# OpenMendel/MendelIHT.jl

Hardware: AMD Instinct MI355X
Metric: IHT iterations/sec + Xᵀr GB/s vs HBM roofline, n=500k p=1M k=200 (higher is better)
Workload: dtype f64 (residual as a 54-bit fixed-point number, exact accumulation on the matrix cores, f64 recombination); 1 GPU; iht on synthetic SnpArray n=500000 p=1000000 k=200 Normal/Identity (BASELINE configs[2]); n=500000, p=1000000, k=200, xtv_variant=-1

## Files before the change

### include/mendeliht_hip.h

```cpp
#ifndef MENDELIHT_HIP_H
#define MENDELIHT_HIP_H
#include <stddef.h>
#include <stdint.h>

#ifdef __cplusplus
extern "C" {
#endif

enum {
    MIH_OK = 0,
    MIH_BAD_DIM = 1,
    MIH_BAD_ARG = 2,
    MIH_NOT_CENTERED = 3,
    MIH_NAN_LOGL = 4,
    MIH_INF_LOGL = 5,
    MIH_HIP_ERROR = 6,
    MIH_OOM = 7,
    MIH_NO_DEVICE = 8
};

enum { MIH_NORMAL = 0, MIH_BERNOULLI = 1, MIH_POISSON = 2, MIH_NEGBIN = 3,
       MIH_GAMMA = 4, MIH_INVGAUSS = 5 };
enum { MIH_IDENTITY = 0, MIH_LOGIT = 1, MIH_LOG = 2, MIH_PROBIT = 3, MIH_CLOGLOG = 4, MIH_CAUCHIT = 5,
       MIH_INVERSE = 6, MIH_INVSQUARE = 7, MIH_SQRT = 8 };
enum { MIH_ESTR_NONE = 0, MIH_ESTR_MM = 1, MIH_ESTR_NEWTON = 2 };

typedef struct mih_mat mih_mat;

int mih_device_count(int *count);
int mih_last_error(char *buf, size_t len);
int mih_version(int *major, int *minor);
int mih_abi_sizes(int64_t *sizes, int32_t n);

int mih_snp_create(const uint8_t *bed_cols, int64_t n, int64_t p, int64_t col_stride_bytes,
                   int center, int scale, int impute, int dtype, int device, mih_mat **out);
int mih_snp_create_synthetic(int64_t n, int64_t p, uint64_t seed, double missing_rate,
                             int center, int scale, int impute, int device, mih_mat **out);
int mih_snp_create_synthetic_shard(int64_t n, int64_t p, int64_t col_offset, uint64_t seed,
                                   double missing_rate, int center, int scale, int impute,
                                   int device, mih_mat **out);
int mih_dense_create(const double *x, int64_t n, int64_t p, int device, mih_mat **out);
int mih_dense_create_f32(const float *x, int64_t n, int64_t p, int device, mih_mat **out);
int mih_dense_create_synthetic(int64_t n, int64_t p, uint64_t seed, int device, mih_mat **out);
int mih_dosage_create(const uint16_t *num, int64_t n, int64_t p, int64_t col_stride, int32_t denom, int device, mih_mat **out);
int mih_dosage_create_synthetic(int64_t n, int64_t p, uint64_t seed, int32_t denom, double missing_rate, int device, mih_mat **out);
enum {
    MIH_BGEN_CORRUPT = 1,
    MIH_BGEN_HEADER = 2,
    MIH_BGEN_PLOIDY = 3,
    MIH_BGEN_PHASED = 4,
    MIH_BGEN_BITS = 5,
    MIH_BGEN_SUM = 6,
    MIH_BGEN_DEEP = 10,
    MIH_BGEN_MIXED = 11,
    MIH_BGEN_FINE = 12,
    MIH_BGEN_MALFORMED = 13
};
int mih_dosage_create_bgen(const char *path, int64_t n, int64_t ncols, const int64_t *block_offset, int compression,
                           int threads, int device, mih_mat **out, int32_t *denom_out, int64_t *bad_block, int32_t *bad_what);
int mih_dosage_regrid(mih_mat *h, int32_t denom);
int mih_dosage_export(const mih_mat *h, int64_t col0, int64_t ncols, uint16_t *out);
int mih_mat_destroy(mih_mat *h);
int mih_mat_reserve(mih_mat *h, int64_t bytes);
int mih_mat_dims(const mih_mat *h, int64_t *n, int64_t *p);
int mih_snp_mu_sigma(const mih_mat *h, double *mu, double *sinv);
int mih_snp_export_bed(const mih_mat *h, uint8_t *bed_cols_out);
int mih_snp_naive_impute(const mih_mat *h, uint8_t *bed_cols_out);

int mih_xtv(const mih_mat *h, const double *r, double *out);
int mih_xtv_batched(const mih_mat *h, const double *R, int m, double *OUT);
int mih_xtv_batched_fmt(const mih_mat *h, const double *R, int m, int digits, double *OUT);
int mih_xv_sparse(const mih_mat *h, const int64_t *idx, const double *val, int64_t nnz, double *out);

int mih_project_topk(double *x, int64_t len, int64_t k, int64_t *n_kept);
int mih_project_group_sparse(double *y, const int64_t *group, int64_t len, int64_t J,
                             const int64_t *k, int k_is_vector);

typedef struct mih_comm {
    int32_t rank, world;
    int64_t col_offset;
    int64_t p_global;
    int (*allreduce)(void *user, double *buf, int64_t count, int32_t op, int32_t on_device);
    int (*allgather)(void *user, const double *send, int64_t count, double *recv);
    void *user;
} mih_comm;

int mih_rccl_unique_id(void *id128);
int mih_comm_create_rccl(const void *id128, int32_t rank, int32_t world, int32_t device, int64_t col_offset,
                         int64_t p_global, mih_comm **out);
int mih_comm_info(const mih_comm *c, int32_t *ranks_seen, char *librccl_path, int64_t cap);
int mih_comm_destroy_rccl(mih_comm *c);
int mih_cv_allgather(const mih_comm *c, double *mses_raw, int64_t count);

typedef struct mih_fit_params {
    int64_t  k;
    int64_t  J;
    int32_t  dist, link;
    double   nb_r;
    double   tol;
    int32_t  max_iter, min_iter, max_step;
    int32_t  est_r;
    const uint8_t *zkeep;
    const double  *weight;
    const int64_t *group;
    const int64_t *ks;
    int64_t  nks;
    void (*progress)(void *user, int iter, double logl, int backtracks, double tol);
    void    *progress_user;
    int32_t  init_beta;
    const mih_comm *comm;
    int32_t  debias;
    int32_t  xtv_digits;
    int (*choose)(void *user, int32_t kind, const int64_t *list, int64_t n, int64_t excess, int64_t *out);
    void    *choose_user;
    int32_t  cv_threads;
    int32_t  step_mode;
} mih_fit_params;
enum { MIH_CHOOSE_SAMPLE = 0, MIH_CHOOSE_SHUFFLE_B = 1, MIH_CHOOSE_SHUFFLE_C = 2 };

typedef struct mih_fit_result {
    double   time;
    double   logl;
    int64_t  iter;
    double   pve;
    double   nb_r;
    int32_t  choose_fired;
    int32_t  n_trace;
    double  *beta;
    double  *c;
    double  *logl_trace;
    double  *tol_trace;
    int32_t *bt_trace;
    double  *mu;
} mih_fit_result;

int mih_fit_iht(const mih_mat *h, const mih_fit_params *prm, const double *y,
                const double *z, int64_t q, const uint8_t *train, mih_fit_result *res);

int mih_cv_iht(const mih_mat *h, const mih_fit_params *prm, const double *y,
               const double *z, int64_t q, const int32_t *folds, int32_t nfolds,
               const int64_t *path, int64_t npath, int32_t rank, int32_t world,
               double *mses_raw);
int mih_cv_assignment(const int64_t *path, int64_t npath, int32_t nfolds, int32_t world, int32_t *rank_of);
int mih_cv_meanloss(const double *mses_raw, const int32_t *folds, int64_t n, int32_t nfolds,
                    int64_t npath, double *mse_out);
int mih_fit_iht_path(const mih_mat *h, const mih_fit_params *prm, const double *y, const double *z,
                     int64_t q, const int64_t *path, int64_t npath, int32_t rank, int32_t world,
                     double *logl_out, int64_t *iter_out, double *beta_out, double *c_out);
int mih_cv_iht_multi(const mih_mat *const *hs, int32_t nrep, const mih_fit_params *prm, const double *y,
                     const double *z, int64_t q, const int32_t *folds, int32_t nfolds,
                     const int64_t *path, int64_t npath, double *mses_raw);

typedef struct mih_mv_result {
    double   time, logl;
    int64_t  iter;
    int32_t  choose_fired, n_trace;
    double  *B;
    double  *C;
    double  *Sigma;
    double  *pve;
    double  *logl_trace, *tol_trace;
    int32_t *bt_trace;
} mih_mv_result;
int mih_fit_mv(const mih_mat *h, const mih_fit_params *prm, const double *Y, int64_t r,
               const double *Z, int64_t q, const uint8_t *train, mih_mv_result *res);
int mih_cv_mv(const mih_mat *h, const mih_fit_params *prm, const double *Y, int64_t r,
              const double *Z, int64_t q, const int32_t *folds, int32_t nfolds,
              const int64_t *path, int64_t npath, int32_t rank, int32_t world, double *mses_raw);

typedef struct mih_session mih_session;
int mih_session_create(const mih_mat *h, const mih_fit_params *prm, const double *y,
                       const double *z, int64_t q, const uint8_t *train, mih_session **out);
int mih_session_step(mih_session *s, double *logl, int32_t *backtracks, double *tol);
int mih_session_run(mih_session *s, int64_t nsteps, double *logl, int64_t *backtracks, double *tol);
int mih_session_model(mih_session *s, double *beta, double *c);
int mih_session_destroy(mih_session *s);

typedef struct mih_pass_record {
    double  start_ms;
    double  ms;
    int32_t residuals;
    int32_t operands;
    int32_t stream_tag;
    int32_t reserved;
    char    kernel[48];
} mih_pass_record;
enum { MIH_CNT_LANES = 0,
       MIH_CNT_MAX_IN_FLIGHT = 1,
       MIH_CNT_HANDOVERS = 2,
       MIH_CNT_SHARED_INIT = 3,
       MIH_CNT_ROUNDS = 4,
       MIH_CNT_FITS = 5,
       MIH_CNT_SCORES = 6,
       MIH_CNT_MAX_LANE_SLOTS = 7,
       MIH_CNT_INIT_SCORES = 8,
       MIH_CNT_RESIDENT_STEPS = 9,
       MIH_CNT_RESIDENT_ATTEMPTS = 10,
       MIH_CNT_RESIDENT_HANDBACKS = 11,
       MIH_CNT_RESIDENT_DIRECT = 12,
       MIH_CNT_RESIDENT_REDOS = 13,
       MIH_CNT_SKIPPED_LAST_SCORES = 14,
       MIH_CNT_RESIDUALS_43BIT = 15,
       MIH_CNT_PEELED_RESIDUALS = 16,
       MIH_PROFILE_NCOUNTERS = 17 };
int mih_profile_enable(const mih_mat *h, int on);
int mih_profile_read(const mih_mat *h, double *xtv_kernel_ms, int64_t *xtv_launches, int reset);
int mih_profile_passes(const mih_mat *h, mih_pass_record *out, int64_t cap, int64_t *n, int reset);
int mih_profile_exchange(const mih_mat *h, double *ms4, int64_t *count4, int reset);
int mih_profile_counters(const mih_mat *h, int64_t *out , int reset);
int mih_bench_xtv(const mih_mat *h, int digits, int m, int iters, int warmup, uint64_t seed,
                  float *ms_per_pass, double *checksum);
int mih_xtv_algorithmic_bytes(const mih_mat *h, int m, double *bytes);

#ifdef __cplusplus
}
#endif
// ... 2 lines not shown
```

### mendeliht.jl_amd/api.py

```python
import ctypes as C
import os
import sys
import time

import numpy as np

_HERE = os.path.dirname(os.path.abspath(__file__))
_LIBNAME = "libmendeliht_hip.so"
_PROBES_LIBNAME = "libmendeliht_hip_probes.so"


class MendelIHTError(RuntimeError):
    """Base class for errors reported by the HIP library."""


class DimensionMismatch(MendelIHTError, ValueError):
    pass


class ArgumentError(MendelIHTError, ValueError):
    pass


_STATUS = {1: DimensionMismatch, 2: ArgumentError, 3: ArgumentError, 4: MendelIHTError, 5: MendelIHTError,
           6: MendelIHTError, 7: MemoryError, 8: MendelIHTError}


def library_path():
    return os.path.join(_HERE, _LIBNAME)


def probes_library_path():
    return os.path.join(_HERE, _PROBES_LIBNAME)


def using_probes():
    e = os.environ.get("MENDELIHT_HIP_PROBES", "")
    return e not in ("", "0")


class _FitParams(C.Structure):
    _fields_ = [("k", C.c_int64), ("J", C.c_int64), ("dist", C.c_int32), ("link", C.c_int32),
                ("nb_r", C.c_double), ("tol", C.c_double),
                ("max_iter", C.c_int32), ("min_iter", C.c_int32), ("max_step", C.c_int32), ("est_r", C.c_int32),
                ("zkeep", C.c_void_p), ("weight", C.c_void_p), ("group", C.c_void_p), ("ks", C.c_void_p),
                ("nks", C.c_int64), ("progress", C.c_void_p), ("progress_user", C.c_void_p),
                ("init_beta", C.c_int32), ("comm", C.c_void_p), ("debias", C.c_int32), ("xtv_digits", C.c_int32),
                ("choose", C.c_void_p), ("choose_user", C.c_void_p), ("cv_threads", C.c_int32), ("step_mode", C.c_int32)]


class _Comm(C.Structure):
    _fields_ = [("rank", C.c_int32), ("world", C.c_int32), ("col_offset", C.c_int64), ("p_global", C.c_int64),
                ("allreduce", C.c_void_p), ("allgather", C.c_void_p), ("user", C.c_void_p)]


_CHOOSE = C.CFUNCTYPE(C.c_int, C.c_void_p, C.c_int32, C.POINTER(C.c_int64), C.c_int64, C.c_int64, C.POINTER(C.c_int64))
CHOOSE_SAMPLE, CHOOSE_SHUFFLE_B, CHOOSE_SHUFFLE_C = 0, 1, 2


def _choose_callback(fn):
    def cb(_user, kind, lst, n, excess, out):
        try:
            got = np.asarray(fn(int(kind), np.array(lst[:n], dtype=np.int64), int(excess)), dtype=np.int64).ravel()
            want = excess if kind == CHOOSE_SAMPLE else n
            if got.size != want:
                return 1
            for t in range(want):
                out[t] = int(got[t])
            return 0
        except Exception:
            return 1
    return _CHOOSE(cb)


_ALLREDUCE = C.CFUNCTYPE(C.c_int, C.c_void_p, C.c_void_p, C.c_int64, C.c_int32, C.c_int32)
_ALLGATHER = C.CFUNCTYPE(C.c_int, C.c_void_p, C.c_void_p, C.c_int64, C.c_void_p)


class _FitResult(C.Structure):
    _fields_ = [("time", C.c_double), ("logl", C.c_double), ("iter", C.c_int64), ("pve", C.c_double),
                ("nb_r", C.c_double), ("choose_fired", C.c_int32), ("n_trace", C.c_int32),
                ("beta", C.c_void_p), ("c", C.c_void_p), ("logl_trace", C.c_void_p), ("tol_trace", C.c_void_p),
                ("bt_trace", C.c_void_p), ("mu", C.c_void_p)]


class _MvResult(C.Structure):
    _fields_ = [("time", C.c_double), ("logl", C.c_double), ("iter", C.c_int64),
                ("choose_fired", C.c_int32), ("n_trace", C.c_int32),
                ("B", C.c_void_p), ("C", C.c_void_p), ("Sigma", C.c_void_p), ("pve", C.c_void_p),
                ("logl_trace", C.c_void_p), ("tol_trace", C.c_void_p), ("bt_trace", C.c_void_p)]


class _PassRecord(C.Structure):
    _fields_ = [("start_ms", C.c_double), ("ms", C.c_double), ("residuals", C.c_int32), ("operands", C.c_int32),
                ("stream_tag", C.c_int32), ("reserved", C.c_int32), ("kernel", C.c_char * 48)]


PROFILE_COUNTERS = ("lanes", "max_in_flight", "handovers", "shared_init", "rounds", "fits", "scores", "max_lane_slots", "init_scores",
                    "resident_steps", "resident_attempts", "resident_handbacks", "resident_direct", "resident_redos", "skipped_last_scores", "residuals_43bit",
                    "peeled_residuals")

_PROGRESS = C.CFUNCTYPE(None, C.c_void_p, C.c_int, C.c_double, C.c_int, C.c_double)

_lib = None


def lib():
    global _lib
    if _lib is not None:
        return _lib
    path = probes_library_path() if using_probes() else library_path()
    path = os.environ.get("MENDELIHT_HIP_LIB", path)
    if not os.path.exists(path):
        raise MendelIHTError(
            f"{path} is missing: build it with `python -c 'import __graft_entry__ as g; g.build()'` "
            "(hipcc --offload-arch=gfx950). There is no CPU fallback for this path.")
    L = C.CDLL(path)
    vp, i64, i32, dbl = C.c_void_p, C.c_int64, C.c_int32, C.c_double
    sig = {
        "mih_device_count": [C.POINTER(C.c_int)],
        "mih_last_error": [C.c_char_p, C.c_size_t],
        "mih_version": [C.POINTER(C.c_int), C.POINTER(C.c_int)],
        "mih_snp_create": [vp, i64, i64, i64, C.c_int, C.c_int, C.c_int, C.c_int, C.c_int, C.POINTER(vp)],
        "mih_snp_create_synthetic": [i64, i64, C.c_uint64, dbl, C.c_int, C.c_int, C.c_int, C.c_int, C.POINTER(vp)],
        "mih_snp_create_synthetic_shard": [i64, i64, i64, C.c_uint64, dbl, C.c_int, C.c_int, C.c_int, C.c_int, C.POINTER(vp)],
        "mih_dense_create": [vp, i64, i64, C.c_int, C.POINTER(vp)],
        "mih_dense_create_synthetic": [i64, i64, C.c_uint64, C.c_int, C.POINTER(vp)],
        "mih_dense_create_f32": [vp, i64, i64, C.c_int, C.POINTER(vp)],
        "mih_dosage_create": [vp, i64, i64, i64, i32, C.c_int, C.POINTER(vp)],
        "mih_dosage_create_synthetic": [i64, i64, C.c_uint64, i32, dbl, C.c_int, C.POINTER(vp)],
        "mih_dosage_export": [vp, i64, i64, vp],
        "mih_dosage_create_bgen": [C.c_char_p, i64, i64, vp, C.c_int, C.c_int, C.c_int, C.POINTER(vp), C.POINTER(i32), C.POINTER(i64),
                                   C.POINTER(i32)],
        "mih_dosage_regrid": [vp, i32],
        "mih_mat_destroy": [vp],
        "mih_mat_dims": [vp, C.POINTER(i64), C.POINTER(i64)],
        "mih_mat_reserve": [vp, i64],
        "mih_snp_mu_sigma": [vp, vp, vp],
        "mih_snp_export_bed": [vp, vp],
        "mih_snp_naive_impute": [vp, vp],
        "mih_xtv": [vp, vp, vp],
        "mih_xtv_batched": [vp, vp, C.c_int, vp],
        "mih_xtv_batched_fmt": [vp, vp, C.c_int, C.c_int, vp],
        "mih_xv_sparse": [vp, vp, vp, i64, vp],
        "mih_project_topk": [vp, i64, i64, C.POINTER(i64)],
        "mih_project_group_sparse": [vp, vp, i64, i64, vp, C.c_int],
        "mih_fit_iht": [vp, C.POINTER(_FitParams), vp, vp, i64, vp, C.POINTER(_FitResult)],
        "mih_cv_iht": [vp, C.POINTER(_FitParams), vp, vp, i64, vp, i32, vp, i64, i32, i32, vp],
        "mih_cv_meanloss": [vp, vp, i64, i32, i64, vp],
        "mih_cv_assignment": [vp, i64, i32, i32, vp],
        "mih_fit_iht_path": [vp, C.POINTER(_FitParams), vp, vp, i64, vp, i64, i32, i32, vp, vp, vp, vp],
        "mih_cv_iht_multi": [vp, i32, C.POINTER(_FitParams), vp, vp, i64, vp, i32, vp, i64, vp],
        "mih_fit_mv": [vp, C.POINTER(_FitParams), vp, i64, vp, i64, vp, C.POINTER(_MvResult)],
        "mih_cv_mv": [vp, C.POINTER(_FitParams), vp, i64, vp, i64, vp, i32, vp, i64, i32, i32, vp],
        "mih_bench_xtv": [vp, C.c_int, C.c_int, C.c_int, C.c_int, C.c_uint64, C.POINTER(C.c_float), C.POINTER(dbl)],
        "mih_xtv_algorithmic_bytes": [vp, C.c_int, C.POINTER(dbl)],
        "mih_abi_sizes": [vp, i32],
        "mih_session_create": [vp, C.POINTER(_FitParams), vp, vp, i64, vp, C.POINTER(vp)],
        "mih_session_step": [vp, C.POINTER(dbl), C.POINTER(i32), C.POINTER(dbl)],
        "mih_session_run": [vp, i64, C.POINTER(dbl), C.POINTER(i64), C.POINTER(dbl)],
        "mih_session_model": [vp, vp, vp],
        "mih_session_destroy": [vp],
        "mih_rccl_unique_id": [vp],
        "mih_comm_create_rccl": [vp, i32, i32, i32, i64, i64, C.POINTER(vp)],
        "mih_comm_destroy_rccl": [vp],
        "mih_comm_info": [vp, C.POINTER(i32), vp, i64],
        "mih_cv_allgather": [vp, vp, i64],
        "mih_profile_enable": [vp, C.c_int],
        "mih_profile_read": [vp, C.POINTER(dbl), C.POINTER(i64), C.c_int],
        "mih_profile_passes": [vp, C.POINTER(_PassRecord), i64, C.POINTER(i64), C.c_int],
        "mih_profile_counters": [vp, C.POINTER(i64), C.c_int],
        "mih_profile_exchange": [vp, C.POINTER(dbl), C.POINTER(i64), C.c_int],
    }
    if using_probes():
        sig.update({"mih_probe_set_xtv_variant": [C.c_int], "mih_probe_set_xtv_multi_variant": [C.c_int],
                    "mih_probe_set_max_fused": [C.c_int],
                    "mih_probe_xtv_sequence": [C.c_void_p, C.c_void_p, C.c_int, C.c_void_p, C.c_int, C.c_int, C.c_void_p],
                    "mih_probe_xv_sequence": [vp, i64, i64, C.c_int, vp, vp, vp, vp, vp, vp, vp]})
    for name, args in sig.items():
        f = getattr(L, name)
        f.argtypes = args
        f.restype = C.c_int
    _lib = L
    return L


def exported_symbols():
    return ["mih_device_count", "mih_last_error", "mih_version", "mih_snp_create", "mih_snp_create_synthetic",
            "mih_snp_create_synthetic_shard",
            "mih_dense_create", "mih_dense_create_synthetic", "mih_dense_create_f32",
            "mih_dosage_create", "mih_dosage_create_synthetic", "mih_dosage_export",
            "mih_dosage_create_bgen", "mih_dosage_regrid", "mih_mat_destroy", "mih_mat_dims", "mih_mat_reserve",
            "mih_snp_mu_sigma", "mih_snp_export_bed", "mih_snp_naive_impute", "mih_xtv", "mih_xtv_batched", "mih_xv_sparse",
            "mih_project_topk", "mih_project_group_sparse", "mih_fit_iht", "mih_cv_iht", "mih_cv_meanloss", "mih_cv_assignment", "mih_cv_iht_multi", "mih_fit_iht_path",
            "mih_fit_mv", "mih_cv_mv", "mih_bench_xtv", "mih_xtv_algorithmic_bytes", "mih_xtv_batched_fmt", "mih_abi_sizes",
            "mih_session_create", "mih_session_step", "mih_session_run", "mih_session_model", "mih_session_destroy",
            "mih_rccl_unique_id", "mih_comm_create_rccl", "mih_comm_info", "mih_comm_destroy_rccl", "mih_cv_allgather",
            "mih_profile_enable", "mih_profile_read", "mih_profile_passes", "mih_profile_counters", "mih_profile_exchange"]


def probe_symbols():
    return ["mih_probe_set_xtv_variant", "mih_probe_set_xtv_multi_variant", "mih_probe_set_max_fused", "mih_probe_xtv_sequence",
            "mih_probe_xv_sequence"]


def _check(rc):
    if rc == 0:
        return
    buf = C.create_string_buffer(512)
    lib().mih_last_error(buf, 512)
    raise _STATUS.get(rc, MendelIHTError)(f"[mih status {rc}] {buf.value.decode(errors='replace')}")


def _p(a):
    return None if a is None else a.ctypes.data_as(C.c_void_p)


def device_count():
    n = C.c_int(0)
    _check(lib().mih_device_count(C.byref(n)))
    return n.value


class _Dist:
    code = 0
    name = "Normal"

    def __repr__(self):
        return f"{self.name}()"


class Normal(_Dist):
    code, name = 0, "Normal"


class Bernoulli(_Dist):
    code, name = 1, "Bernoulli"


class Poisson(_Dist):
    code, name = 2, "Poisson"


class NegativeBinomial(_Dist):
    code, name = 3, "NegativeBinomial"

    def __init__(self, r=1.0, p=0.5):
        self.r, self.p = float(r), float(p)

    def __repr__(self):
        return f"NegativeBinomial(r={self.r}, p={self.p})"


class Gamma(_Dist):
    code, name = 4, "Gamma"


class InverseGaussian(_Dist):
    code, name = 5, "InverseGaussian"


class MvNormal(_Dist):
    code, name = -1, "MvNormal"


class IdentityLink:
    code = 0

    def __repr__(self):
        return "IdentityLink()"


class LogitLink:
    code = 1

    def __repr__(self):
        return "LogitLink()"


class LogLink:
    code = 2

    def __repr__(self):
        return "LogLink()"


def _link(name, code):
    return type(name, (), {"code": code, "__repr__": lambda self: f"{name}()"})


ProbitLink = _link("ProbitLink", 3)
CloglogLink = _link("CloglogLink", 4)
CauchitLink = _link("CauchitLink", 5)
InverseLink = _link("InverseLink", 6)
InverseSquareLink = _link("InverseSquareLink", 7)
SqrtLink = _link("SqrtLink", 8)


def canonicallink(d):
    d = _inst(d)
    return {0: IdentityLink, 1: LogitLink, 2: LogLink, 3: LogLink, 4: InverseLink, 5: InverseSquareLink}[max(d.code, 0)]()


def _inst(x):
    return x() if isinstance(x, type) else x


def read_bed(path, n):
    size = os.path.getsize(path)
    with open(path, "rb") as f:
        magic = f.read(3)
    if size < 3 or magic != b"\x6c\x1b\x01":
        raise ArgumentError(f"{path} is not a SNP-major PLINK .bed file")
    stride = (n + 3) // 4
    if (size - 3) % stride:
        raise DimensionMismatch(f"{path}: size does not match n={n}")
    if size == 3:
        return np.zeros((0, stride), dtype=np.uint8)
    return np.memmap(path, dtype=np.uint8, mode="r", offset=3, shape=((size - 3) // stride, stride))


class _Mat:
    def __init__(self):
        self._h = C.c_void_p(None)
        self.n = self.p = 0

    def __del__(self):
        try:
            if self._h:
                lib().mih_mat_destroy(self._h)
                self._h = C.c_void_p(None)
        except Exception:
            pass

    @property
    def shape(self):
        return (self.n, self.p)

    def _dims(self):
        n, p = C.c_int64(0), C.c_int64(0)
        _check(lib().mih_mat_dims(self._h, C.byref(n), C.byref(p)))
        self.n, self.p = n.value, p.value

    def xtv(self, r, xtv_digits=None):
        r = np.asarray(r, dtype=np.float64)
        dg = _digits(xtv_digits)
        if r.ndim == 1:
            if r.size != self.n:
                raise DimensionMismatch(f"r has length {r.size}, expected {self.n}")
            r = np.ascontiguousarray(r)
            out = np.empty(self.p)
            if dg == 0:
                _check(lib().mih_xtv(self._h, _p(r), _p(out)))
            else:
                _check(lib().mih_xtv_batched_fmt(self._h, _p(r), 1, dg, _p(out)))
            return out
        if r.shape[0] != self.n:
            raise DimensionMismatch(f"R has {r.shape[0]} rows, expected {self.n}")
        R = np.asfortranarray(r)
        out = np.empty((self.p, R.shape[1]), order="F")
        _check(lib().mih_xtv_batched_fmt(self._h, _p(R), R.shape[1], dg, _p(out)))
        return out

    def xv_sparse(self, idx, val):
        idx = np.ascontiguousarray(idx, dtype=np.int64)
        val = np.ascontiguousarray(val, dtype=np.float64)
        out = np.empty(self.n)
        _check(lib().mih_xv_sparse(self._h, _p(idx), _p(val), idx.size, _p(out)))
        return out

    def bench_xtv(self, variant=-1, iters=10, warmup=2, seed=1, xtv_digits=None):
        return self.bench_xtv_batched(1, variant=variant, iters=iters, warmup=warmup, seed=seed, xtv_digits=xtv_digits)

    def bench_xtv_batched(self, m, max_fused=4, variant=-1, iters=5, warmup=1, seed=1, xtv_digits=None):
        if variant != -1 or max_fused != 4 or using_probes():
            probe_set(variant=variant, max_fused=max_fused)
        ms, cs = C.c_float(0), C.c_double(0)
        try:
            _check(lib().mih_bench_xtv(self._h, _digits(xtv_digits), m, iters, warmup, seed, C.byref(ms), C.byref(cs)))
        finally:
            if using_probes():
                probe_set(variant=-1, max_fused=4)
        return ms.value, cs.value

    def algorithmic_bytes(self, m=1):
        b = C.c_double(0)
        _check(lib().mih_xtv_algorithmic_bytes(self._h, m, C.byref(b)))
        return b.value


RESERVE_BY_DEFAULT = False


class SnpLinAlg(_Mat):

    def _reserve(self, reserve):
        if reserve:
            _check(lib().mih_mat_reserve(self._h, 0))
        elif reserve is None and RESERVE_BY_DEFAULT:
            lib().mih_mat_reserve(self._h, 0)

    def __init__(self, bed, n=None, center=False, scale=False, impute=True, device=0, _handle=None, dtype=np.float64, reserve=None):
        super().__init__()
        self.center, self.scale, self.impute = bool(center), bool(scale), bool(impute)
        self.device = device
        self.dtype = np.dtype(dtype).type
        if self.dtype not in (np.float64, np.float32):
            raise ArgumentError("SnpLinAlg{T}: T must be Float64 or Float32")
        if _handle is not None:
            self._h = _handle
            self._dims()
            return
        if isinstance(bed, (str, os.PathLike)):
            if n is None:
                raise ArgumentError("n (number of samples) is required with a .bed path")
            bed = read_bed(bed, n)
        cols = np.ascontiguousarray(bed, dtype=np.uint8)
        if cols.ndim != 2:
            raise DimensionMismatch("bed columns must be a (p, stride) uint8 array")
        if n is None:
            raise ArgumentError("n (number of samples) is required")
        h = C.c_void_p(None)
        _check(lib().mih_snp_create(_p(cols), n, cols.shape[0], cols.shape[1], int(center), int(scale),
                                    int(impute), 32 if self.dtype is np.float32 else 64, device, C.byref(h)))
        self._h = h
        self._dims()
        self._reserve(reserve)

    @classmethod
    def synthetic(cls, n, p, seed=2024, missing_rate=0.0, center=True, scale=True, impute=True, device=0,
                  col_offset=0, reserve=None):
        h = C.c_void_p(None)
        _check(lib().mih_snp_create_synthetic_shard(n, p, int(col_offset), seed, float(missing_rate), int(center),
                                                    int(scale), int(impute), device, C.byref(h)))
        x = cls(None, center=center, scale=scale, impute=impute, device=device, _handle=h)
        x._reserve(reserve)
        return x

    def mu_sigma(self):
        mu, s = np.empty(self.p), np.empty(self.p)
        _check(lib().mih_snp_mu_sigma(self._h, _p(mu), _p(s)))
        return mu, s

    def export_bed(self):
        out = np.empty((self.p, (self.n + 3) // 4), dtype=np.uint8)
        _check(lib().mih_snp_export_bed(self._h, _p(out)))
        return out


def naive_impute(x, destination, n=None):
    if isinstance(x, SnpLinAlg):
        mat = x
    else:
        if n is None:
            raise ArgumentError("naive_impute needs the number of samples n with a .bed path or raw columns")
        cols = read_bed(x, n) if isinstance(x, (str, os.PathLike)) else x
        mat = SnpLinAlg(cols, n)
    out = np.empty((mat.p, (mat.n + 3) // 4), dtype=np.uint8)
    _check(lib().mih_snp_naive_impute(mat._h, _p(out)))
    if not str(destination).endswith(".bed"):
        destination = str(destination) + ".bed"
    with open(destination, "wb") as f:
        f.write(b"\x6c\x1b\x01")
        f.write(out.tobytes())
    return None


class DenseMatrix(_Mat):

    def __init__(self, x, device=0, _handle=None):
        super().__init__()
        self.device = device
        self.dtype = np.float64
        if _handle is not None:
            self._h = _handle
            self._dims()
            return
        x = np.asarray(x)
        if x.ndim != 2:
            raise DimensionMismatch("x must be a matrix")
        h = C.c_void_p(None)
        if x.dtype == np.float32:
            x = np.asfortranarray(x)
            self.dtype = np.float32
            _check(lib().mih_dense_create_f32(_p(x), x.shape[0], x.shape[1], device, C.byref(h)))
        else:
            x = np.asfortranarray(x, dtype=np.float64)
            _check(lib().mih_dense_create(_p(x), x.shape[0], x.shape[1], device, C.byref(h)))
        self._h = h
        self._dims()

    @classmethod
    def synthetic(cls, n, p, seed=2024, device=0):
        h = C.c_void_p(None)
        _check(lib().mih_dense_create_synthetic(n, p, seed, device, C.byref(h)))
        return cls(None, device=device, _handle=h)


class DosageMatrix(_Mat):

    def __init__(self, num, denom, device=0, _handle=None):
        super().__init__()
        self.device = device
        self.denom = int(denom)
        self.dtype = np.float64
        if _handle is not None:
            self._h = _handle
            self._dims()
            return
        num = np.asarray(num)
        if num.ndim != 2:
            raise DimensionMismatch("num must be a matrix")
        if num.dtype != np.uint16:
            raise ArgumentError(f"num must be uint16 (0xFFFF = missing), got {num.dtype}")
        num = np.asfortranarray(num)
        h = C.c_void_p(None)
        _check(lib().mih_dosage_create(_p(num), num.shape[0], num.shape[1], num.shape[0], self.denom, device, C.byref(h)))
        self._h = h
        self._dims()

    @classmethod
    def from_dosages(cls, d, device=0):
        from .genotypes import dosage_grid
        num, denom = dosage_grid(np.asarray(d, dtype=np.float64))
        return cls(num, denom, device=device)

    @classmethod
    def synthetic(cls, n, p, seed=2024, denom=255, missing_rate=0.0, device=0):
        h = C.c_void_p(None)
        _check(lib().mih_dosage_create_synthetic(n, p, seed, int(denom), float(missing_rate), device, C.byref(h)))
        return cls(None, denom, device=device, _handle=h)

    def mu_sigma(self):
        mu, s = np.empty(self.p), np.empty(self.p)
        _check(lib().mih_snp_mu_sigma(self._h, _p(mu), _p(s)))
        return mu, s

    def regrid(self, denom):
        _check(lib().mih_dosage_regrid(self._h, int(denom)))
        self.denom = int(denom)
        return self

    def export(self, col0=0, ncols=None):
        ncols = self.p - col0 if ncols is None else ncols
        out = np.empty((ncols, self.n), dtype=np.uint16)
        _check(lib().mih_dosage_export(self._h, int(col0), int(ncols), _p(out)))
        return out.T


def _as_mat(x):
    if isinstance(x, _Mat):
        return x
    if isinstance(x, np.ndarray):
        if x.dtype == np.uint8:
            raise ArgumentError("x is a SnpArray! Please convert it to a SnpLinAlg first!")
        return DenseMatrix(x)
    raise ArgumentError(f"unsupported design matrix type {type(x)}")


def project_k(x, k):
    if k < 0:
        raise ArgumentError(f"DomainError: Attempted to project to sparsity level {k}")
    x = np.array(x, dtype=np.float64).ravel()
    kept = C.c_int64(0)
    _check(lib().mih_project_topk(_p(x), x.size, int(k), C.byref(kept)))
    return x


def project_group_sparse(y, group, J, k):
    y = np.array(y, dtype=np.float64).ravel()
    group = np.ascontiguousarray(group, dtype=np.int64)
    if group.size != y.size:
        raise DimensionMismatch("group must have the length of y")
    kv = np.ascontiguousarray(np.atleast_1d(k), dtype=np.int64)
    _check(lib().mih_project_group_sparse(_p(y), _p(group), y.size, int(J), _p(kv), int(np.ndim(k) > 0)))
    return y


def standardize(z):
    z = np.array(z, dtype=np.float64)
    mu = z.mean(axis=0)
    sd = np.sqrt(((z - mu) ** 2).sum(axis=0) / (z.shape[0] - 1))
    return (z - mu) / sd


class IHTResult:

    def __init__(self, time, logl, iter, beta, c, J, k, group, d, sigma_g, trace=None, choose_fired=False, mu=None):
        self.time, self.logl, self.iter = time, logl, iter
        self.beta, self.c, self.J, self.k, self.group, self.d = beta, c, J, k, group, d
# ... 713 lines not shown
```

### mendeliht.jl_amd/csrc/common.h

```cpp
#pragma once
#include <hip/hip_runtime.h>
#include <atomic>
#include <chrono>
#include <map>
#include <mutex>
#include <iterator>
#include <memory>
#include <cstdint>
#include <cstdlib>
#include <cstdio>
#include <cstring>
#include <string>
#include <unordered_map>
#include <functional>
#include <vector>
#include "../../include/mendeliht_hip.h"

namespace mih {

void set_error(const char *fmt, ...);
int  hip_fail(hipError_t e, const char *what, const char *file, int line);

inline const char *probe_env(const char *name)
{
#ifdef MIH_PROBES
    return getenv(name);
#else
    (void)name;
    return nullptr;
#endif
}

#define MIH_HIP(expr)                                                         \
    do {                                                                      \
        hipError_t e_ = (expr);                                               \
        if (e_ != hipSuccess) return ::mih::hip_fail(e_, #expr, __FILE__, __LINE__); \
    } while (0)

#define MIH_TRY(expr)                      \
    do {                                   \
        int rc_ = (expr);                  \
        if (rc_ != MIH_OK) return rc_;     \
    } while (0)

constexpr int kChunkRows = 1024;

inline int64_t round_up(int64_t a, int64_t b) { return (a + b - 1) / b * b; }

struct DevPool {
    char *base = nullptr; size_t bytes = 0;
    std::mutex mu;
    std::map<size_t, size_t> free_blocks;
    std::map<size_t, size_t> used;
    static constexpr size_t kGran = 2ull << 20;
    ~DevPool() { if (base) (void)hipFree(base); }
    bool init(size_t total)
    {
        total = (total + kGran - 1) / kGran * kGran;
        if (hipMalloc((void **)&base, total) != hipSuccess) { (void)hipGetLastError(); base = nullptr; return false; }
        bytes = total; free_blocks[0] = total;
        return true;
    }
    void *take(size_t want)
    {
        want = (want + kGran - 1) / kGran * kGran;
        std::lock_guard<std::mutex> g(mu);
        for (auto it = free_blocks.begin(); it != free_blocks.end(); ++it) {
            if (it->second < want) continue;
            const size_t off = it->first, sz = it->second;
            free_blocks.erase(it);
            if (sz > want) free_blocks[off + want] = sz - want;
            used[off] = want;
            return base + off;
        }
        return nullptr;
    }
    bool owns(const void *q) const { return base && (const char *)q >= base && (const char *)q < base + bytes; }
    void give_back(void *q)
    {
        std::lock_guard<std::mutex> g(mu);
        const size_t off = (size_t)((char *)q - base);
        auto u = used.find(off);
        if (u == used.end()) return;
        size_t o = off, sz = u->second;
        used.erase(u);
        auto nx = free_blocks.lower_bound(o);
        if (nx != free_blocks.end() && o + sz == nx->first) { sz += nx->second; nx = free_blocks.erase(nx); }
        if (nx != free_blocks.begin()) { auto pv = std::prev(nx); if (pv->first + pv->second == o) { o = pv->first; sz += pv->second; free_blocks.erase(pv); } }
        free_blocks[o] = sz;
    }
};
inline DevPool *&current_pool() { static thread_local DevPool *q = nullptr; return q; }
struct PoolScope {
    DevPool *prev;
    explicit PoolScope(DevPool *q) : prev(current_pool()) { current_pool() = q; }
    ~PoolScope() { current_pool() = prev; }
};
inline hipError_t dev_malloc(void **q, size_t bytes, DevPool **from)
{
    *from = nullptr;
    if (DevPool *pl = current_pool()) {
        if (bytes >= (1ull << 20)) { if (void *r = pl->take(bytes)) { *q = r; *from = pl; return hipSuccess; } }
    }
    return hipMalloc(q, bytes);
}

struct Arena {
    char *dev = nullptr, *pin = nullptr;
    DevPool *dev_pool = nullptr;
    size_t dev_bytes = 0, pin_bytes = 0, dev_off = 0, pin_off = 0;
    Arena() = default;
    Arena(const Arena &) = delete;
    Arena &operator=(const Arena &) = delete;
    ~Arena() { release_dev(); if (pin) (void)hipHostFree(pin); }
    void release_dev() { if (dev) { if (dev_pool) dev_pool->give_back(dev); else (void)hipFree(dev); dev = nullptr; } }
    int reserve(size_t device_bytes, size_t pinned_bytes)
    {
        static const bool off = probe_env("MENDELIHT_NO_ARENA") != nullptr;
        if (off) return MIH_OK;
        if (dev_malloc((void **)&dev, device_bytes, &dev_pool) != hipSuccess) { (void)hipGetLastError(); dev = nullptr; device_bytes = 0; }
        if (hipHostMalloc((void **)&pin, pinned_bytes, hipHostMallocCoherent) != hipSuccess) { (void)hipGetLastError(); pin = nullptr; pinned_bytes = 0; }
        dev_bytes = device_bytes; pin_bytes = pinned_bytes; dev_off = pin_off = 0;
        return MIH_OK;
    }
    void *take_dev(size_t bytes)
    {
        const size_t o = (dev_off + 255) & ~(size_t)255;
        if (!dev || o + bytes > dev_bytes) return nullptr;
        dev_off = o + bytes;
        return dev + o;
    }
    void *take_pin(size_t bytes)
    {
        const size_t o = (pin_off + 255) & ~(size_t)255;
        if (!pin || o + bytes > pin_bytes) return nullptr;
        pin_off = o + bytes;
        return pin + o;
    }
};
inline Arena *&current_arena() { static thread_local Arena *a = nullptr; return a; }
struct CoopSched { virtual void yield() = 0; virtual ~CoopSched() {} };
inline CoopSched *&current_coop() { static thread_local CoopSched *c = nullptr; return c; }
inline int &coop_blocked() { static thread_local int d = 0; return d; }
inline bool coop_can_yield() { return current_coop() != nullptr && coop_blocked() == 0; }
int stream_sync_coop(hipStream_t s);
struct ArenaScope {
    Arena *prev;
    explicit ArenaScope(Arena *a) : prev(current_arena()) { current_arena() = a; ++coop_blocked(); }
    ~ArenaScope() { current_arena() = prev; --coop_blocked(); }
};

template <typename T>
struct DevBuf {
    T *p = nullptr;
    size_t n = 0;
    bool own = true;
    DevPool *pool = nullptr;
    DevBuf() = default;
    DevBuf(const DevBuf &) = delete;
    DevBuf &operator=(const DevBuf &) = delete;
    ~DevBuf() { release(); }
    void release() { if (p && own) { if (pool) pool->give_back(p); else (void)hipFree(p); } p = nullptr; n = 0; own = true; pool = nullptr; }
    void attach(T *ptr, size_t count) { release(); p = ptr; n = count; own = false; }
    int alloc(size_t count) {
        release();
        if (count == 0) count = 1;
        if (Arena *a = current_arena()) {
            if (void *q = a->take_dev(count * sizeof(T))) { p = static_cast<T *>(q); n = count; own = false; return MIH_OK; }
        }
        hipError_t e = dev_malloc((void **)&p, count * sizeof(T), &pool);
        if (e != hipSuccess) { set_error("hipMalloc(%zu bytes) failed: %s", count * sizeof(T), hipGetErrorString(e)); p = nullptr; return e == hipErrorOutOfMemory ? MIH_OOM : MIH_HIP_ERROR; }
        n = count;
        return MIH_OK;
    }
};

template <typename T>
struct PinBuf {
    T *p = nullptr;
    size_t n = 0;
    bool own = true;
    PinBuf() = default;
    PinBuf(const PinBuf &) = delete;
    PinBuf &operator=(const PinBuf &) = delete;
    ~PinBuf() { if (p && own) (void)hipHostFree(p); }
    int alloc(size_t count, bool coherent = false) {
        if (p && own) (void)hipHostFree(p);
        p = nullptr; n = 0; own = true;
        if (count == 0) count = 1;
        if (Arena *a = current_arena()) {
            if (void *q = a->take_pin(count * sizeof(T))) { p = static_cast<T *>(q); n = count; own = false; return MIH_OK; }
        }
        if (hipHostMalloc((void **)&p, count * sizeof(T), coherent ? hipHostMallocCoherent : hipHostMallocDefault) != hipSuccess) { set_error("hipHostMalloc(%zu bytes) failed", count * sizeof(T)); (void)hipGetLastError(); p = nullptr; return MIH_OOM; }
        n = count;
        return MIH_OK;
    }
};

struct SpinFlag {
    PinBuf<uint64_t> word;
    uint64_t seq = 0;
};
int readback_words(hipStream_t s, SpinFlag &f, const uint64_t *src_dev, uint64_t *dst_host, size_t words, int64_t pairs_first = -1);
uint64_t spin_begin(SpinFlag &f);
int spin_wait(hipStream_t s, SpinFlag &f, uint64_t seq);
#if defined(__HIPCC__)
__device__ __forceinline__ void publish_block(const uint64_t *src, uint64_t *dst_host, uint64_t words, uint64_t *flag_host, uint64_t seq)
{
    for (uint64_t i = threadIdx.x; i < words; i += blockDim.x)
        dst_host[i] = __hip_atomic_load(&src[i], __ATOMIC_RELAXED, __HIP_MEMORY_SCOPE_AGENT);
    __threadfence_system();
    __syncthreads();
    if (threadIdx.x == 0) __hip_atomic_store(flag_host, seq, __ATOMIC_RELEASE, __HIP_MEMORY_SCOPE_SYSTEM);
}
#endif

struct HostStage {
    static constexpr int kSlots = 8;
    PinBuf<uint64_t> ring;
    size_t slot_words = 0;
    int next = 0, since_sync = 0;
    int init(size_t words_per_slot) { slot_words = words_per_slot; next = 0; since_sync = 0; return ring.alloc(words_per_slot * kSlots, true); }
    int put(hipStream_t s, const void *a, size_t bytes_a, const void *b, size_t bytes_b, const uint64_t **out);
    void synced() { since_sync = 0; }
};
void stage_to_device(hipStream_t s, const uint64_t *src_pinned, uint64_t *dst_a, size_t words_a, uint64_t *dst_b, size_t words_b);

}

namespace mih {
struct PassRecord { hipEvent_t e0 = nullptr, e1 = nullptr; int residuals = 0, operands = 0, stream_tag = 0; char kernel[48] = {0}; };
struct ExchRecord { hipEvent_t e0 = nullptr, e1 = nullptr; int kind = 0; };
struct Profile {
    std::mutex mu;
    std::atomic<bool> on{false};
    hipEvent_t origin = nullptr;
    std::vector<PassRecord> open;
    std::vector<mih_pass_record> done;
    int64_t counters[MIH_PROFILE_NCOUNTERS] = {0};
    std::vector<ExchRecord> xopen;
    double xms[4] = {0.0, 0.0, 0.0, 0.0}; int64_t xcount[4] = {0, 0, 0, 0};
    void exch_host(int kind, double ms) { if (!on) return; std::lock_guard<std::mutex> g(mu); xms[kind] += ms; ++xcount[kind]; }
    void count(int which, int64_t add) { if (!on) return; std::lock_guard<std::mutex> g(mu); counters[which] += add; }
    void count_max(int which, int64_t v) { if (!on) return; std::lock_guard<std::mutex> g(mu); if (v > counters[which]) counters[which] = v; }
    void drain();
    ~Profile();
};
}

struct mih_mat {
    int       kind = 0;
    int       device = 0;
    int64_t   n = 0, p = 0;
    int       center = 1, scale = 1, impute = 1;
    int64_t   ncg = 0;
    int64_t   nbp = 0;
    int64_t   n_pad = 0;
    uint32_t *X = nullptr;
    double   *mu = nullptr, *sinv = nullptr;
    int64_t  *miss_ptr = nullptr;
    int32_t  *miss_row = nullptr;
    int64_t   total_missing = 0;
    double   *D = nullptr;
    float    *Df = nullptr;
    uint16_t *Du = nullptr;
    int64_t   du_ld = 0;
    int32_t   denom = 0;
    double   *du_mun = nullptr;
    double   *du_sc = nullptr;
    hipStream_t stream = nullptr;
    mih::DevPool *pool = nullptr;
    std::shared_ptr<mih::DevPool> pool_owner;
    std::shared_ptr<mih::Profile> prof = std::make_shared<mih::Profile>();
    mutable std::mutex ws_mu;
    mutable std::vector<hipStream_t> worker_streams;
};
namespace mih {
int select_device(int device);

struct DosageView { const uint16_t *X; int64_t ld; const double *mun, *sc; };
int dosage_alloc(mih_mat *h, int64_t n, int64_t p, int32_t denom, int device);
int dosage_stats(mih_mat *h);
void dosage_rescale(mih_mat *h, const uint32_t *gcol, uint32_t g, uint32_t mult);
inline DosageView dosage_view(const mih_mat *h) { return {h->Du, h->du_ld, h->du_mun, h->du_sc}; }
__device__ __forceinline__ double dosage_c(uint32_t num, double mun) { return num == 0xFFFFu ? 0.0 : (double)num - mun; }
__device__ __forceinline__ double dosage_x(const DosageView &v, int64_t j, int64_t i)
{
    return dosage_c(v.X[j * v.ld + i], v.mun[j]) * v.sc[j];
}
constexpr int kWorkerStreamsPerLane = 4;
hipStream_t worker_stream(const mih_mat *h, int i);
}

namespace mih {

__host__ __device__ inline int64_t xword(int64_t nbp, int64_t j, int64_t t)
{
    int64_t cg = j >> 5, blk = t >> 2, bp = blk >> 1;
    int m = (int)(j & 31), h = (int)((t >> 1) & 1), u = (int)(t & 1), e = (int)(blk & 1);
    return (((cg * nbp + bp) * 64 + (h * 32 + m)) << 2) + (e << 1) + u;
}

struct DigitMode {
    int base;
    int ndig;
    int per_op;
    int slots;
    int ebits;
    int rows_log2;
    int lay16 = 0;
    int flat = 0;
    int nres = 0;
    const int32_t *gate = nullptr; int32_t gate_val = 0;
};
constexpr int kMaxFlatPasses = 16;
struct FlatPasses { int npass; int u0[kMaxFlatPasses + 1]; int t0[kMaxFlatPasses + 1]; };
struct XtvTune {
    int digits = 0;
    int variant = -1;
    int multi_variant = 0;
    int max_nr = 4;
    int max_ops = 6;
    int slices = 0;
    bool half = true;
};
XtvTune xtv_tune(int digits);
inline XtvTune xtv_tune(const mih_fit_params *prm) { return xtv_tune(prm ? prm->xtv_digits : 0); }
bool xtv_digits_valid(int digits);

struct XtvSupportHook {
    const int32_t *cur = nullptr;
    const int64_t *idx[2] = {nullptr, nullptr};
    const int64_t *cnt[2] = {nullptr, nullptr};
    double *gval = nullptr, *A = nullptr, *B = nullptr;
    int blocks = 0;
};
struct XtvStatsHook {
    const double *spart = nullptr;
    const double *zpart = nullptr; double *df2 = nullptr; int q = 0, zblocks = 0;
    int ebits = 0;
};
constexpr int kStatBlocks = 64;
struct XtvWork {
    DevBuf<uint32_t> digits;
    DevBuf<double>   partial;
    DevBuf<double>   scal;
    DevBuf<unsigned> stat_done;
    double peels_counted = 0.0;
    DevBuf<double>   peel;
    int m_cap = 0, splits_cap = 0;
    DigitMode dm = {13, 16, 2, 16, 56, 20};
    int ops_cap = 0;
    size_t rhs_cap = 0;
    XtvTune tune;
    int stream_tag = 0;
    const int32_t *gate = nullptr; int32_t gate_val = 0;
    bool stats_done = false;
    DigitMode dm_alt = {49, 8, 4, 8, 42, 18}; bool has_alt = false, use_alt = false;
    XtvSupportHook hook;
    XtvStatsHook shook;
};
int  xtv_work_init(const mih_mat *h, XtvWork &w, int m, const XtvTune &tune, bool batched = true);
int  xtv_device(const mih_mat *h, XtvWork &w, const double *r_dev, int m, double *out_dev, hipStream_t s);
void xtv_count_peels(const mih_mat *h, XtvWork &w, hipStream_t s);
int  xtv_lockstep_width(const mih_mat *h, const XtvTune &tune);

struct XvWork {
    DevBuf<double> partial;
    DevBuf<double> coefA, coefB;
    DevBuf<double> coefG;
    int64_t cap = 0; int groups = 0;
    DevBuf<uint32_t> cache;
    DevBuf<int32_t>  slot_dev;
    DevBuf<int64_t>  fill_dev;
    DevBuf<int64_t>  off_dev;
    int64_t slots = 0;
    std::unordered_map<int64_t, int32_t> slot_of;
    std::vector<int64_t> col_of;
    std::vector<uint64_t> stamp;
    uint64_t tick = 0;
    std::vector<int64_t> h_offs;
    std::vector<int32_t> h_slots; std::vector<int64_t> h_fills;
};
int  xv_work_init(const mih_mat *h, XvWork &w, int64_t max_nnz, int64_t cache_nnz = 0);
size_t xv_work_bytes(const mih_mat *h, int64_t max_nnz, int64_t cache_nnz = 0);
int  xv_sparse_device(const mih_mat *h, XvWork &w, const int64_t *idx_dev, const double *val_dev,
                      int64_t nnz, double *out_dev, int clamp20, hipStream_t s, const int64_t *idx_host = nullptr,
                      HostStage *st = nullptr, const double *gather_src = nullptr, double *gather_out = nullptr);

int  xv_sparse_multi_device(const mih_mat *h, XvWork &w, const int64_t *idx_dev, const double *vals_dev, int64_t nnz, int m,
                            double *out_dev, hipStream_t s, const int64_t *idx_host);

struct TopkWork {
    DevBuf<uint32_t> hist;
    DevBuf<uint64_t> state;
    PinBuf<uint64_t> hsel;
    DevBuf<uint64_t> sel;
    DevBuf<uint64_t> fin;
    int64_t cap = 0;
    int64_t expect = 0;
    bool radix8 = false;
    SpinFlag flag;
};
int  topk_work_init(TopkWork &w, int64_t max_keep);
int  topk_project_device(double *x_dev, int64_t len, int64_t k, TopkWork &w, hipStream_t s,
                         std::vector<int64_t> &idx_out, std::vector<double> &val_out, bool zero_in_place = true);
int  collect_nonzero_device(double *x_dev, int64_t len, TopkWork &w, hipStream_t s,
                            std::vector<int64_t> &idx_out, std::vector<double> &val_out);
int  group_project_device(double *y_dev, const int64_t *group_dev, int64_t len, int64_t G, int64_t J,
                          const int64_t *k_dev, int k_is_vector, hipStream_t s);
struct DebiasShard { int64_t k_total = 0, k_off = 0; std::function<int(double *, int64_t)> reduce; };
int  debias_glm_device(const mih_mat *h, const int64_t *idx_host, int64_t k, const double *y_dev, int dist, int link,
                       double nb_r, double *beta_out, hipStream_t s, const DebiasShard *shard = nullptr);
int  comm_native_allreduce_on_stream(const mih_comm *c, double *buf_dev, int64_t count, int32_t op, hipStream_t s, int device);
int  comm_native_allgather_on_stream(const mih_comm *c, const double *send_dev, double *recv_dev, int64_t count, hipStream_t s, int device);
bool comm_is_native(const mih_comm *c, int device);
void cv_assign(const int64_t *path, int64_t npath, int32_t nfolds, int32_t world, std::vector<int32_t> &rank_of);
int  init_beta_regress_device(const mih_mat *h, const double *w_dev, const double *Y_dev, int m, double N,
                              const double *Sy_host, double *beta_dev, double *icpt_sum_host,
                              DevBuf<double> &red, DevBuf<double> &scal, hipStream_t s, const XtvTune &tune);

}
```

### mendeliht.jl_amd/csrc/dosage.hip

```cpp
#include "common.h"
#include <cmath>

namespace mih {

__global__ void __launch_bounds__(256)
k_dosage_stats(const uint16_t *__restrict__ X, int64_t ld, int32_t denom, double *__restrict__ mu, double *__restrict__ sinv,
               double *__restrict__ mun, double *__restrict__ sc, unsigned long long *__restrict__ bad)
{
    __shared__ unsigned long long s_sum[256], s_cnt[256], s_bad[256];
    const int64_t j = blockIdx.x;
    const uint4 *cx = reinterpret_cast<const uint4 *>(X + j * ld);
    const uint32_t top = 2u * (uint32_t)denom;
    unsigned long long sum = 0, cnt = 0, nbad = 0;
    for (int64_t i = threadIdx.x; i < ld / 8; i += 256) {
        const uint4 q = cx[i];
        const uint32_t w[4] = {q.x, q.y, q.z, q.w};
        #pragma unroll
        for (int k = 0; k < 8; ++k) {
            const uint32_t v = (w[k >> 1] >> (16 * (k & 1))) & 0xFFFFu;
            if (v != 0xFFFFu) {
                if (v > top) ++nbad;
                else { sum += v; ++cnt; }
            }
        }
    }
    s_sum[threadIdx.x] = sum; s_cnt[threadIdx.x] = cnt; s_bad[threadIdx.x] = nbad;
    __syncthreads();
    for (int w = 128; w > 0; w >>= 1) {
        if ((int)threadIdx.x < w) {
            s_sum[threadIdx.x] += s_sum[threadIdx.x + w]; s_cnt[threadIdx.x] += s_cnt[threadIdx.x + w];
            s_bad[threadIdx.x] += s_bad[threadIdx.x + w];
        }
        __syncthreads();
    }
    if (threadIdx.x == 0) {
        const double S = (double)s_sum[0], N = (double)s_cnt[0];
        const double m = N > 0.0 ? S / (N * (double)denom) : 0.0;
        const double s = sqrt(m * (1.0 - m / 2.0));
        mu[j] = m;
        sinv[j] = s > 0.0 ? 1.0 / s : 1.0;
        mun[j] = N > 0.0 ? S / N : 0.0;
        sc[j] = sinv[j] / (double)denom;
        if (s_bad[0]) atomicAdd(bad, s_bad[0]);
    }
}

__device__ __forceinline__ uint32_t dsg_mix(uint32_t x)
{
    x ^= x >> 16; x *= 0x7feb352du; x ^= x >> 15; x *= 0x846ca68bu; x ^= x >> 16;
    return x;
}

__global__ void __launch_bounds__(256)
k_dosage_synth(uint16_t *__restrict__ X, int64_t ld, int64_t n, int64_t p, uint64_t seed, int32_t denom, uint32_t miss_thr)
{
    const int64_t nv = ld / 8, total = nv * p;
    const uint32_t s0 = dsg_mix((uint32_t)seed ^ 0x3C6EF372u) ^ dsg_mix((uint32_t)(seed >> 32) + 0x1B873593u);
    const int32_t blur = denom / 10;
    for (int64_t q = blockIdx.x * 256ll + threadIdx.x; q < total; q += 256ll * gridDim.x) {
        const int64_t j = q / nv, i0 = (q - j * nv) * 8;
        const uint32_t key = dsg_mix(s0 ^ dsg_mix((uint32_t)j) ^ dsg_mix((uint32_t)(j >> 32) + 0x85EBCA6Bu));
        const uint32_t thr = (uint32_t)(((dsg_mix(key ^ 0xB5297A4Du) >> 8) + 0.5) / 16777216.0 * 0.5 * 65536.0);
        uint32_t w[4] = {0u, 0u, 0u, 0u};
        #pragma unroll
        for (int k = 0; k < 8; ++k) {
            const int64_t i = i0 + k;
            uint32_t v = 0xFFFFu;
            if (i < n) {
                const uint32_t e = dsg_mix(key ^ dsg_mix((uint32_t)i ^ 0x68E31DA4u) ^ (uint32_t)(i >> 32));
                const uint32_t f = dsg_mix(e ^ 0x1B56C4E9u), g = dsg_mix(f ^ 0x2C1B3C6Du);
                const int32_t calls = (int32_t)((e & 0xFFFFu) < thr) + (int32_t)((e >> 16) < thr);
                const int32_t d = blur > 0 ? (int32_t)(f % (uint32_t)(2 * blur + 1)) - blur : 0;
                int32_t num = calls * denom + d;
                num = num < 0 ? 0 : (num > 2 * denom ? 2 * denom : num);
                v = g < miss_thr ? 0xFFFFu : (uint32_t)num;
            }
            w[k >> 1] |= v << (16 * (k & 1));
        }
        reinterpret_cast<uint4 *>(X + j * ld)[i0 / 8] = make_uint4(w[0], w[1], w[2], w[3]);
    }
}

int dosage_alloc(mih_mat *h, int64_t n, int64_t p, int32_t denom, int device)
{
    h->kind = 1; h->device = device; h->n = n; h->p = p; h->center = h->scale = h->impute = 0;
    h->denom = denom;
    h->du_ld = (n + 7) / 8 * 8;
    if (hipMalloc((void **)&h->Du, sizeof(uint16_t) * (size_t)h->du_ld * (size_t)p) != hipSuccess) {
        set_error("hipMalloc for the dosage matrix (%lld x %lld u16) failed", (long long)n, (long long)p); (void)hipGetLastError(); return MIH_OOM;
    }
    for (double **a : {&h->mu, &h->sinv, &h->du_mun, &h->du_sc})
        if (hipMalloc((void **)a, sizeof(double) * (size_t)p) != hipSuccess) { set_error("hipMalloc failed"); (void)hipGetLastError(); return MIH_OOM; }
    if (hipStreamCreate(&h->stream) != hipSuccess) return MIH_HIP_ERROR;
    return MIH_OK;
}

int dosage_stats(mih_mat *h)
{
    DevBuf<unsigned long long> bad;
    MIH_TRY(bad.alloc(1));
    MIH_HIP(hipMemsetAsync(bad.p, 0, sizeof(unsigned long long), h->stream));
    hipLaunchKernelGGL(k_dosage_stats, dim3((unsigned)h->p), dim3(256), 0, h->stream, h->Du, h->du_ld, h->denom, h->mu, h->sinv,
                       h->du_mun, h->du_sc, bad.p);
    unsigned long long nbad = 0;
    MIH_HIP(hipMemcpyAsync(&nbad, bad.p, sizeof(nbad), hipMemcpyDeviceToHost, h->stream));
    MIH_HIP(hipStreamSynchronize(h->stream));
    if (nbad) { set_error("%llu dosage numerators exceed 2 * denom = %d (0xFFFF marks a missing entry)", nbad, 2 * h->denom); return MIH_BAD_ARG; }
    return MIH_OK;
}

__global__ void __launch_bounds__(256)
k_dosage_scale(uint16_t *__restrict__ X, int64_t ld, const uint32_t *__restrict__ gcol, uint32_t g, uint32_t mult)
{
    const int64_t j = blockIdx.x;
    const uint32_t m = gcol ? gcol[j] / g : mult;
    if (m == 1u) return;
    uint4 *cx = reinterpret_cast<uint4 *>(X + j * ld);
    for (int64_t i = threadIdx.x; i < ld / 8; i += 256) {
        const uint4 q = cx[i];
        uint32_t w[4] = {q.x, q.y, q.z, q.w};
        #pragma unroll
        for (int k = 0; k < 4; ++k) {
            const uint32_t lo = w[k] & 0xFFFFu, hi = w[k] >> 16;
            w[k] = (lo == 0xFFFFu ? lo : lo * m) | ((hi == 0xFFFFu ? hi : hi * m) << 16);
        }
        cx[i] = make_uint4(w[0], w[1], w[2], w[3]);
    }
}

void dosage_rescale(mih_mat *h, const uint32_t *gcol, uint32_t g, uint32_t mult)
{
    hipLaunchKernelGGL(k_dosage_scale, dim3((unsigned)h->p), dim3(256), 0, h->stream, h->Du, h->du_ld, gcol, g, mult);
}

}

using namespace mih;

extern "C" {

int mih_dosage_create(const uint16_t *num, int64_t n, int64_t p, int64_t col_stride, int32_t denom, int device, mih_mat **out)
{
    if (!num || !out) { set_error("null argument"); return MIH_BAD_ARG; }
    if (n <= 0 || p <= 0 || col_stride < n) { set_error("bad dimensions"); return MIH_BAD_DIM; }
    if (denom < 1 || denom > 32767) { set_error("denom must be in [1, 32767], got %d", denom); return MIH_BAD_ARG; }
    MIH_TRY(select_device(device));
    mih_mat *h = new mih_mat();
    auto fail = [&](int code) { mih_mat_destroy(h); return code; };
    int rc = dosage_alloc(h, n, p, denom, device);
    if (rc) return fail(rc);
    const size_t ld_b = sizeof(uint16_t) * (size_t)h->du_ld;
    if (h->du_ld > n && hipMemset2DAsync(h->Du + n, ld_b, 0xFF, sizeof(uint16_t) * (size_t)(h->du_ld - n), (size_t)p, h->stream) != hipSuccess)
        return fail(MIH_HIP_ERROR);
    if (hipMemcpy2DAsync(h->Du, ld_b, num, sizeof(uint16_t) * (size_t)col_stride, sizeof(uint16_t) * (size_t)n, (size_t)p,
                         hipMemcpyHostToDevice, h->stream) != hipSuccess) { set_error("dosage upload failed"); return fail(MIH_HIP_ERROR); }
    if ((rc = dosage_stats(h))) return fail(rc);
    *out = h;
    return MIH_OK;
}

int mih_dosage_create_synthetic(int64_t n, int64_t p, uint64_t seed, int32_t denom, double missing_rate, int device, mih_mat **out)
{
    if (!out) { set_error("null argument"); return MIH_BAD_ARG; }
    if (n <= 0 || p <= 0) { set_error("bad dimensions"); return MIH_BAD_DIM; }
    if (denom < 1 || denom > 32767) { set_error("denom must be in [1, 32767], got %d", denom); return MIH_BAD_ARG; }
    if (!(missing_rate >= 0.0 && missing_rate < 1.0)) { set_error("missing_rate must be in [0,1)"); return MIH_BAD_ARG; }
    MIH_TRY(select_device(device));
    mih_mat *h = new mih_mat();
    auto fail = [&](int code) { mih_mat_destroy(h); return code; };
    int rc = dosage_alloc(h, n, p, denom, device);
    if (rc) return fail(rc);
    const uint32_t miss_thr = (uint32_t)(missing_rate * 4294967296.0);
    hipLaunchKernelGGL(k_dosage_synth, dim3(8192), dim3(256), 0, h->stream, h->Du, h->du_ld, n, p, seed, denom, miss_thr);
    if ((rc = dosage_stats(h))) return fail(rc);
    *out = h;
    return MIH_OK;
}

int mih_dosage_regrid(mih_mat *h, int32_t denom)
{
    if (!h || !h->Du) { set_error("not a dosage handle"); return MIH_BAD_ARG; }
    if (denom < 1 || denom > 32767 || denom % h->denom != 0) {
        set_error("denom must be a multiple of the handle's denominator %d and at most 32767, got %d", h->denom, denom); return MIH_BAD_ARG;
    }
    if (denom == h->denom) return MIH_OK;
    MIH_HIP(hipSetDevice(h->device));
    dosage_rescale(h, nullptr, 1u, (uint32_t)(denom / h->denom));
    h->denom = denom;
    return dosage_stats(h);
}

int mih_dosage_export(const mih_mat *h, int64_t col0, int64_t ncols, uint16_t *out)
{
    if (!h || !h->Du || !out) { set_error("not a dosage handle"); return MIH_BAD_ARG; }
    if (col0 < 0 || ncols < 0 || col0 + ncols > h->p) { set_error("columns [%lld, %lld) out of range", (long long)col0, (long long)(col0 + ncols)); return MIH_BAD_DIM; }
    if (ncols == 0) return MIH_OK;
    MIH_HIP(hipSetDevice(h->device));
    MIH_HIP(hipMemcpy2D(out, sizeof(uint16_t) * (size_t)h->n, h->Du + col0 * h->du_ld, sizeof(uint16_t) * (size_t)h->du_ld,
                        sizeof(uint16_t) * (size_t)h->n, (size_t)ncols, hipMemcpyDeviceToHost));
    return MIH_OK;
}

}
```

### mendeliht.jl_amd/csrc/snp.hip

```cpp
#include "common.h"
#include <memory>
#include <cstdarg>
#include <cmath>
#include <cstdlib>
#include <cstring>
#include <atomic>
#include <thread>

namespace mih {

static thread_local char g_err[512] = "";

void set_error(const char *fmt, ...)
{
    va_list ap;
    va_start(ap, fmt);
    vsnprintf(g_err, sizeof(g_err), fmt, ap);
    va_end(ap);
}

int hip_fail(hipError_t e, const char *what, const char *file, int line)
{
    set_error("HIP error %d (%s) at %s:%d: %s", (int)e, hipGetErrorString(e), file, line, what);
    (void)hipGetLastError();
    return e == hipErrorOutOfMemory ? MIH_OOM : MIH_HIP_ERROR;
}

__device__ __forceinline__ uint32_t plink_to_dosage(uint32_t w)
{
    uint32_t hi = w & 0xAAAAAAAAu;
    uint32_t both = (w << 1) & hi;
    return (hi >> 1) + (both >> 1);
}
__device__ __forceinline__ uint32_t plink_missing_mask(uint32_t w)
{
    return (~w >> 1) & w & 0x55555555u;
}

__device__ __forceinline__ uint32_t lowbias32(uint32_t x)
{
    x ^= x >> 16; x *= 0x7feb352du; x ^= x >> 15; x *= 0x846ca68bu; x ^= x >> 16;
    return x;
}

__device__ __forceinline__ void flush_counts(int32_t c1, int32_t c2, int32_t cm, int64_t cg, int64_t p,
                                             int32_t *__restrict__ cnt)
{
    __shared__ int32_t red[3][32];
    if (threadIdx.x < 96) red[threadIdx.x / 32][threadIdx.x % 32] = 0;
    __syncthreads();
    int m = threadIdx.x & 31;
    atomicAdd(&red[0][m], c1); atomicAdd(&red[1][m], c2); atomicAdd(&red[2][m], cm);
    __syncthreads();
    if (threadIdx.x < 96) {
        int k = threadIdx.x / 32, mm = threadIdx.x % 32;
        int64_t j = cg * 32 + mm;
        if (j < p && red[k][mm]) atomicAdd(&cnt[3 * j + k], red[k][mm]);
    }
}

constexpr int kBpPerBlock = 64;
__global__ void __launch_bounds__(256)
k_transcode(const uint8_t *__restrict__ raw, int64_t raw_stride, int64_t n, int64_t p, int64_t col0,
            int64_t ncols, uint4 *__restrict__ X, int64_t nbp, int32_t *__restrict__ cnt)
{
    const int lane = threadIdx.x & 63, w = threadIdx.x >> 6, m = lane & 31, h = lane >> 5;
    const int64_t cg = col0 / 32 + blockIdx.y;
    const int64_t j = cg * 32 + m, jl = j - col0;
    const bool live = j < p && jl < ncols;
    const uint8_t *src = raw + (live ? jl : 0) * raw_stride;
    const int64_t nbytes = (n + 3) >> 2;
    int32_t c1 = 0, c2 = 0, cm = 0;
    int64_t bp0 = (int64_t)blockIdx.x * kBpPerBlock;
    for (int64_t bp = bp0 + w; bp < bp0 + kBpPerBlock && bp < nbp; bp += 4) {
        uint32_t d[4];
        #pragma unroll
        for (int q = 0; q < 4; ++q) {
            int64_t t = bp * 8 + (q >> 1) * 4 + h * 2 + (q & 1);
            uint32_t wv = 0;
            if (live) {
                int64_t b0 = t * 4;
                #pragma unroll
                for (int b = 0; b < 4; ++b) if (b0 + b < nbytes) wv |= (uint32_t)src[b0 + b] << (8 * b);
                int64_t rows_left = n - t * 16;
                uint32_t valid = rows_left >= 16 ? 0xFFFFFFFFu : rows_left <= 0 ? 0u : ((1u << (2 * rows_left)) - 1u);
                wv &= valid;
            }
            const uint32_t dd = plink_to_dosage(wv), mm = plink_missing_mask(wv);
            d[q] = dd | mm | (mm << 1);
            c1 += __popc(dd & 0x55555555u); c2 += __popc(dd & 0xAAAAAAAAu); cm += __popc(mm);
        }
        X[(cg * nbp + bp) * 64 + lane] = make_uint4(d[0], d[1], d[2], d[3]);
    }
    flush_counts(c1, c2, cm, cg, p, cnt);
}

__global__ void k_col_stats(const int32_t *__restrict__ cnt, int64_t n, int64_t p,
                            double *__restrict__ mu, double *__restrict__ sinv)
{
    int64_t j = blockIdx.x * (int64_t)blockDim.x + threadIdx.x;
    if (j >= p) return;
    double n1 = cnt[3 * j], n2 = cnt[3 * j + 1], nm = cnt[3 * j + 2];
    double m = (n1 + 2.0 * n2) / ((double)n - nm);
    double s = sqrt(m * (1.0 - m / 2.0));
    mu[j] = m;
    sinv[j] = (s > 0.0) ? 1.0 / s : 1.0;
}

__global__ void __launch_bounds__(64)
k_missing_from_tiles(uint4 *__restrict__ X, int64_t nbp, int64_t p, const int64_t *__restrict__ miss_ptr,
                     int32_t *__restrict__ miss_row)
{
    const int64_t cg = blockIdx.x;
    const int lane = threadIdx.x, m = lane & 31, h = lane >> 5;
    const int64_t j = cg * 32 + m;
    int64_t base = (j < p) ? miss_ptr[j] : 0;
    const int64_t end = (j < p) ? miss_ptr[j + 1] : 0;
    if (__ballot(end > base) == 0ull) return;
    for (int64_t bp = 0; bp < nbp; ++bp) {
        uint4 v = X[(cg * nbp + bp) * 64 + lane];
        uint32_t d[4] = {v.x, v.y, v.z, v.w}, mk[4];
        int c[2] = {0, 0};
        #pragma unroll
        for (int q = 0; q < 4; ++q) { mk[q] = d[q] & (d[q] >> 1) & 0x55555555u; c[q >> 1] += __popc(mk[q]); }
        const int o0 = __shfl_xor(c[0], 32, 64), o1 = __shfl_xor(c[1], 32, 64);
        if (__ballot((c[0] | c[1]) != 0) == 0ull) continue;
        int64_t w0 = base + (h ? o0 : 0);
        int64_t w1 = base + c[0] + o0 + (h ? o1 : 0);
        #pragma unroll
        for (int q = 0; q < 4; ++q) {
            int64_t &w = (q >> 1) ? w1 : w0;
            uint32_t bits = mk[q];
            const int32_t row0 = (int32_t)(bp * 128 + (q >> 1) * 64 + h * 32 + (q & 1) * 16);
            while (bits) {
                int sft = __ffs((int)bits) - 1;
                miss_row[w++] = row0 + (sft >> 1);
                bits &= bits - 1;
            }
            d[q] &= ~(mk[q] | (mk[q] << 1));
        }
        if (c[0] | c[1]) X[(cg * nbp + bp) * 64 + lane] = make_uint4(d[0], d[1], d[2], d[3]);
        base += c[0] + c[1] + o0 + o1;
    }
}

__device__ __forceinline__ void synth_entry(uint32_t key_g, uint32_t key_m, uint32_t thr16,
                                            uint32_t miss_thr, int64_t i, uint32_t &dos, bool &miss)
{
    uint32_t h = lowbias32((uint32_t)i * 0x9E3779B1u ^ key_g);
    dos = ((h & 0xFFFFu) < thr16) + ((h >> 16) < thr16);
    miss = miss_thr != 0 && lowbias32((uint32_t)i * 0x85EBCA77u ^ key_m) < miss_thr;
}

__device__ __forceinline__ void synth_col_keys(uint64_t seed, int64_t j, uint32_t &key_g,
                                               uint32_t &key_m, uint32_t &thr16)
{
    uint32_t s0 = (uint32_t)seed, s1 = (uint32_t)(seed >> 32);
    key_g = lowbias32((uint32_t)j ^ lowbias32(s0 ^ 0xA511E9B3u)) ^ lowbias32((uint32_t)(j >> 32) + s1);
    key_m = lowbias32(key_g ^ 0x68E31DA4u);
    uint32_t u = lowbias32(key_g ^ 0xB5297A4Du) >> 8;
    double maf = 0.5 * ((double)u + 0.5) / 16777216.0;
    thr16 = (uint32_t)(maf * 65536.0);
}

__global__ void __launch_bounds__(256)
k_synth(uint4 *__restrict__ X, int64_t nbp, int64_t n, int64_t p, int64_t col0, uint64_t seed,
        uint32_t miss_thr, int32_t *__restrict__ cnt)
{
    const int lane = threadIdx.x & 63, w = threadIdx.x >> 6, m = lane & 31, h = lane >> 5;
    const int64_t cg = blockIdx.y;
    const int64_t j = cg * 32 + m;
    const bool live = j < p;
    uint32_t key_g = 0, key_m = 0, thr16 = 0;
    if (live) synth_col_keys(seed, col0 + j, key_g, key_m, thr16);
    int32_t c1 = 0, c2 = 0, cm = 0;
    int64_t bp0 = (int64_t)blockIdx.x * kBpPerBlock;
    for (int64_t bp = bp0 + w; bp < bp0 + kBpPerBlock && bp < nbp; bp += 4) {
        uint32_t d[4];
        #pragma unroll
        for (int q = 0; q < 4; ++q) {
            int64_t t = bp * 8 + (q >> 1) * 4 + h * 2 + (q & 1);
            uint32_t dd = 0;
            if (live) {
                #pragma unroll
                for (int s = 0; s < 16; ++s) {
                    int64_t i = t * 16 + s;
                    uint32_t dos; bool miss;
                    synth_entry(key_g, key_m, thr16, miss_thr, i, dos, miss);
                    if (i < n) {
                        if (miss) cm++;
                        else { dd |= dos << (2 * s); c1 += (dos == 1); c2 += (dos == 2); }
                    }
                }
            }
            d[q] = dd;
        }
        X[(cg * nbp + bp) * 64 + lane] = make_uint4(d[0], d[1], d[2], d[3]);
    }
    flush_counts(c1, c2, cm, cg, p, cnt);
}

__global__ void __launch_bounds__(64)
k_fill_missing_synth(int64_t n, int64_t p, int64_t col0, uint64_t seed, uint32_t miss_thr,
                     const int64_t *__restrict__ miss_ptr, int32_t *__restrict__ miss_row)
{
    int64_t j = blockIdx.x;
    if (j >= p) return;
    uint32_t key_g, key_m, thr16;
    synth_col_keys(seed, col0 + j, key_g, key_m, thr16);
    int64_t base = miss_ptr[j];
    int lane = threadIdx.x;
    for (int64_t i0 = 0; i0 < n; i0 += 64) {
        int64_t i = i0 + lane;
        uint32_t dos; bool miss = false;
        if (i < n) synth_entry(key_g, key_m, thr16, miss_thr, i, dos, miss);
        unsigned long long bal = __ballot(miss);
        if (miss) miss_row[base + __popcll(bal & ((1ull << lane) - 1ull))] = (int32_t)i;
        base += __popcll(bal);
    }
}

__global__ void k_synth_dense(double *__restrict__ D, int64_t total, uint64_t seed)
{
    int64_t i = blockIdx.x * (int64_t)blockDim.x + threadIdx.x;
    int64_t stride = (int64_t)gridDim.x * blockDim.x;
    uint32_t s0 = lowbias32((uint32_t)seed ^ 0x3C6EF372u), s1 = lowbias32((uint32_t)(seed >> 32) ^ 0xDAA66D2Bu);
    for (; i < total; i += stride) {
        uint32_t a = lowbias32((uint32_t)i ^ s0) ^ lowbias32((uint32_t)(i >> 32) + s1);
        uint32_t b = lowbias32(a ^ 0x9E3779B9u);
        double u = ((a & 0xFFFF) + (a >> 16) + (b & 0xFFFF) + (b >> 16)) * (1.0 / 65536.0) - 2.0;
        D[i] = u * 1.7320508075688772;
    }
}

__global__ void k_export(const uint4 *__restrict__ X, int64_t nbp, int64_t ncg, int64_t p, int64_t ndw,
                         uint32_t *__restrict__ out)
{
    int64_t total = ncg * nbp * 64;
    int64_t i = blockIdx.x * (int64_t)blockDim.x + threadIdx.x;
    int64_t stride = (int64_t)gridDim.x * blockDim.x;
    for (; i < total; i += stride) {
        int lane = (int)(i & 63), m = lane & 31, h = lane >> 5;
        int64_t tile = i >> 6, cg = tile / nbp, bp = tile - cg * nbp, j = cg * 32 + m;
        if (j >= p) continue;
        uint4 v = X[i];
        uint32_t d[4] = {v.x, v.y, v.z, v.w};
        #pragma unroll
        for (int q = 0; q < 4; ++q) {
            int64_t t = bp * 8 + (q >> 1) * 4 + h * 2 + (q & 1);
            uint32_t nz = (d[q] | (d[q] >> 1)) & 0x55555555u;
            uint32_t two = (d[q] >> 1) & 0x55555555u;
            out[j * ndw + t] = (nz << 1) | two;
        }
    }
}

__global__ void k_export_missing(uint32_t *__restrict__ out, int64_t ndw, int64_t p,
                                 const int64_t *__restrict__ miss_ptr, const int32_t *__restrict__ miss_row)
{
    int64_t j = blockIdx.x;
    if (j >= p) return;
    for (int64_t t = miss_ptr[j] + threadIdx.x; t < miss_ptr[j + 1]; t += blockDim.x) {
        int32_t i = miss_row[t];
        atomicOr(&out[j * ndw + (i >> 4)], 1u << (2 * (i & 15)));
    }
}

__global__ void __launch_bounds__(64)
k_impute_mode(uint32_t *__restrict__ out, int64_t ndw, int64_t p, int64_t n,
              const int64_t *__restrict__ miss_ptr, const int32_t *__restrict__ miss_row)
{
    const int64_t j = blockIdx.x;
    if (j >= p) return;
    const int64_t a = miss_ptr[j], b = miss_ptr[j + 1];
    if (b == a) return;
    long long c1 = 0, c2 = 0;
    for (int64_t t = threadIdx.x; t < ndw; t += 64) {
        const uint32_t d = out[j * ndw + t], hi = (d >> 1) & 0x55555555u, lo = d & 0x55555555u;
        c1 += __popc(hi & ~lo);
        c2 += __popc(hi & lo);
    }
    #pragma unroll
    for (int off = 32; off > 0; off >>= 1) { c1 += __shfl_xor(c1, off, 64); c2 += __shfl_xor(c2, off, 64); }
    const long long c0 = n - (b - a) - c1 - c2;
    const long long most = c0 > c1 ? (c0 > c2 ? c0 : c2) : (c1 > c2 ? c1 : c2);
    const uint32_t code = most == c1 ? 2u : most == c2 ? 3u : 0u;
    if (code == 0u) return;
    for (int64_t t = a + threadIdx.x; t < b; t += 64) {
        const int32_t i = miss_row[t];
        atomicOr(&out[j * ndw + (i >> 4)], code << (2 * (i & 15)));
    }
}

static int finish_missing_ptr(mih_mat *h, const std::vector<int32_t> &cnt, std::vector<int64_t> &ptr)
{
    ptr.assign((size_t)h->p + 1, 0);
    for (int64_t j = 0; j < h->p; ++j) ptr[j + 1] = ptr[j] + cnt[3 * j + 2];
    h->total_missing = ptr[h->p];
    MIH_HIP(hipMalloc((void **)&h->miss_ptr, sizeof(int64_t) * (size_t)(h->p + 1)));
    MIH_HIP(hipMemcpy(h->miss_ptr, ptr.data(), sizeof(int64_t) * (size_t)(h->p + 1), hipMemcpyHostToDevice));
    MIH_HIP(hipMalloc((void **)&h->miss_row, sizeof(int32_t) * (size_t)(h->total_missing > 0 ? h->total_missing : 1)));
    return MIH_OK;
}

static int alloc_snp(mih_mat *h)
{
    h->ncg = (h->p + 31) / 32;
    h->nbp = (h->n + 127) / 128;
    h->n_pad = h->nbp * 128;
    size_t bytes = sizeof(uint4) * (size_t)h->ncg * (size_t)h->nbp * 64;
    hipError_t e = hipMalloc((void **)&h->X, bytes);
    if (e != hipSuccess) { set_error("hipMalloc of %zu bytes for the genotype matrix failed: %s", bytes, hipGetErrorString(e)); return MIH_OOM; }
    MIH_HIP(hipMalloc((void **)&h->mu, sizeof(double) * (size_t)h->p));
    MIH_HIP(hipMalloc((void **)&h->sinv, sizeof(double) * (size_t)h->p));
    return MIH_OK;
}

hipStream_t worker_stream(const mih_mat *h, int i)
{
    std::lock_guard<std::mutex> g(h->ws_mu);
    if (i < 0 || i >= 2 * kWorkerStreamsPerLane) return nullptr;
    if ((int)h->worker_streams.size() <= i) h->worker_streams.resize((size_t)i + 1, nullptr);
    if (!h->worker_streams[(size_t)i]) {
        hipStream_t st = nullptr;
        if (hipStreamCreate(&st) != hipSuccess) { (void)hipGetLastError(); return nullptr; }
        h->worker_streams[(size_t)i] = st;
    }
    return h->worker_streams[(size_t)i];
}

int select_device(int device)
{
    int c = 0;
    if (hipGetDeviceCount(&c) != hipSuccess || c == 0) {
        (void)hipGetLastError();
        set_error("no HIP device available (the MI355X path has no CPU fallback)");
        return MIH_NO_DEVICE;
    }
    if (device < 0 || device >= c) { set_error("device %d out of range (count %d)", device, c); return MIH_BAD_ARG; }
    MIH_HIP(hipSetDevice(device));
    return MIH_OK;
}

}

using namespace mih;

extern "C" {

int mih_device_count(int *count)
{
    if (!count) { set_error("count is NULL"); return MIH_BAD_ARG; }
    int c = 0;
    hipError_t e = hipGetDeviceCount(&c);
    if (e != hipSuccess) { *count = 0; (void)hipGetLastError(); return MIH_OK; }
    *count = c;
    return MIH_OK;
}

int mih_last_error(char *buf, size_t len)
{
    if (!buf || len == 0) return MIH_BAD_ARG;
    snprintf(buf, len, "%s", g_err);
    return MIH_OK;
}

int mih_version(int *major, int *minor)
{
    if (major) *major = 0;
    if (minor) *minor = 6;
    return MIH_OK;
}

int mih_abi_sizes(int64_t *sizes, int32_t n)
{
    const int64_t v[4] = {(int64_t)sizeof(mih_fit_params), (int64_t)sizeof(mih_fit_result), (int64_t)sizeof(mih_mv_result),
                          (int64_t)sizeof(mih_comm)};
    if (!sizes) return MIH_BAD_ARG;
    for (int i = 0; i < n && i < 4; ++i) sizes[i] = v[i];
    return MIH_OK;
}

static void reserve_fit_memory(mih_mat *h, bool asked = false, size_t asked_bytes = 0)
{
    static const bool off = probe_env("MENDELIHT_NO_RESERVE") != nullptr;
    const size_t min_bytes = (size_t)(4ull << 30);
    const size_t x_bytes = (size_t)h->ncg * (size_t)h->nbp * 1024;
    if (h->kind != 0 || (!asked && (off || x_bytes < min_bytes))) return;
    size_t big = (size_t)2432 * (size_t)h->p;
    size_t var = 128ull << 20;
    if (x_bytes >= (4ull << 30)) big = std::min<size_t>(std::max<size_t>(big, 256ull << 20), 4ull << 30);
    else {
        big = std::max<size_t>(big + (size_t)30 * 8 * (size_t)h->n_pad, 4ull << 20);
        var = std::min<size_t>(var, std::max<size_t>((size_t)8 * (40 * (size_t)h->n_pad + 6 * (size_t)h->p) + (2ull << 20), 4ull << 20));
    }
    const size_t want = asked_bytes ? asked_bytes : 4 * big + 64 * var;
    size_t free_b = 0, total_b = 0;
    if (hipMemGetInfo(&free_b, &total_b) != hipSuccess) { (void)hipGetLastError(); return; }
    if (free_b < 4 * want) return;
    std::shared_ptr<DevPool> pool(new DevPool());
    if (pool->init(want)) { h->pool_owner = pool; h->pool = pool.get(); }
}

int mih_snp_create(const uint8_t *bed_cols, int64_t n, int64_t p, int64_t col_stride_bytes,
                   int center, int scale, int impute, int dtype, int device, mih_mat **out)
{
    if (!bed_cols || !out) { set_error("null argument"); return MIH_BAD_ARG; }
    if (n <= 0 || p <= 0 || col_stride_bytes < (n + 3) / 4) { set_error("bad dimensions n=%lld p=%lld stride=%lld", (long long)n, (long long)p, (long long)col_stride_bytes); return MIH_BAD_DIM; }
    if (n >= (1ll << 31)) { set_error("n must be < 2^31"); return MIH_BAD_DIM; }
    if (dtype != 64 && dtype != 32) { set_error("dtype must be 64 (SnpLinAlg{Float64}) or 32 (SnpLinAlg{Float32})"); return MIH_BAD_ARG; }
    MIH_TRY(select_device(device));
    const bool trace = probe_env("MENDELIHT_INGEST_TRACE") != nullptr;
    auto tnow = [] { return std::chrono::duration<double, std::milli>(std::chrono::steady_clock::now().time_since_epoch()).count(); };
    double t_mark = tnow();
    auto lap = [&](const char *what) { if (trace) { const double t = tnow(); fprintf(stderr, "ingest: %-28s %8.2f ms\n", what, t - t_mark); t_mark = t; } };
    mih_mat *h = new mih_mat();
    h->kind = 0; h->device = device; h->n = n; h->p = p;
    h->center = center; h->scale = scale; h->impute = impute;
    int rc = alloc_snp(h);
    if (rc) { mih_mat_destroy(h); return rc; }
    if (hipStreamCreate(&h->stream) != hipSuccess) { mih_mat_destroy(h); return MIH_HIP_ERROR; }
    lap("matrix allocation");

    auto fail = [&](int code) { mih_mat_destroy(h); return code; };
    const int64_t chunk_bytes = 16ll << 20;
    int64_t cols_per_chunk = chunk_bytes / col_stride_bytes / 32 * 32;
    if (cols_per_chunk < 32) cols_per_chunk = 32;
    if (cols_per_chunk > round_up(p, 32)) cols_per_chunk = round_up(p, 32);
    const size_t buf_bytes = (size_t)(cols_per_chunk * col_stride_bytes);
    const int64_t nchunks = (p + cols_per_chunk - 1) / cols_per_chunk;
    DevBuf<int32_t> cnt;
    if ((rc = cnt.alloc((size_t)(3 * p)))) return fail(rc);
    if (hipMemsetAsync(cnt.p, 0, sizeof(int32_t) * 3 * (size_t)p, h->stream) != hipSuccess) return fail(MIH_HIP_ERROR);
    if (hipStreamSynchronize(h->stream) != hipSuccess) return fail(MIH_HIP_ERROR);
    unsigned nth = std::thread::hardware_concurrency();
    nth = nth >= 16 ? 8 : (nth >= 4 ? nth / 2 : 1);
    if (const char *e = probe_env("MENDELIHT_INGEST_THREADS")) { int v = atoi(e); if (v >= 1 && v <= 64) nth = (unsigned)v; }
    if ((int64_t)nth > nchunks) nth = (unsigned)nchunks;
    const size_t staging_budget = 512ull << 20;
    if (buf_bytes * 2 * nth > staging_budget) nth = (unsigned)std::max<size_t>(1, staging_budget / (buf_bytes * 2));
    std::atomic<int64_t> next_chunk{0};
    std::atomic<int> failed{0};
    std::mutex err_mu; std::string err_msg;
    struct Staging {
        uint8_t *pin = nullptr, *raw = nullptr;
        ~Staging() { if (pin) (void)hipHostFree(pin); if (raw) (void)hipFree(raw); }
    } stg;
    for (;;) {
        const bool ok = hipHostMalloc((void **)&stg.pin, buf_bytes * 2 * nth, hipHostMallocDefault) == hipSuccess &&
                        hipMalloc((void **)&stg.raw, buf_bytes * 2 * nth) == hipSuccess;
        if (ok) break;
        (void)hipGetLastError();
        if (stg.pin) { (void)hipHostFree(stg.pin); stg.pin = nullptr; }
        if (stg.raw) { (void)hipFree(stg.raw); stg.raw = nullptr; }
        if (nth == 1) { set_error("allocation of the upload staging buffers (2 x %zu bytes pinned + device) failed", buf_bytes); return fail(MIH_OOM); }
        nth = 1;
    }
    lap("staging buffers");
    std::atomic<unsigned> worker_no{0};
    auto worker = [&]() {
        const unsigned me = worker_no.fetch_add(1);
        struct Res {
            uint8_t *pin[2] = {nullptr, nullptr}, *raw[2] = {nullptr, nullptr}; hipStream_t st = nullptr; hipEvent_t done[2] = {nullptr, nullptr};
            ~Res() {
                if (st) (void)hipStreamSynchronize(st);
                for (int i = 0; i < 2; ++i) if (done[i]) (void)hipEventDestroy(done[i]);
                if (st) (void)hipStreamDestroy(st);
            }
        } r;
        auto bad = [&](const char *what) { std::lock_guard<std::mutex> g(err_mu); if (err_msg.empty()) err_msg = what; failed.store(1); };
        if (hipSetDevice(device) != hipSuccess || hipStreamCreate(&r.st) != hipSuccess) return bad("ingest worker: stream");
        for (int i = 0; i < 2; ++i) {
            r.pin[i] = stg.pin + buf_bytes * (2 * me + i);
            r.raw[i] = stg.raw + buf_bytes * (2 * me + i);
            if (hipEventCreateWithFlags(&r.done[i], hipEventDisableTiming) != hipSuccess) return bad("ingest worker: event");
        }
        for (int64_t it = 0; !failed.load(); ++it) {
            const int64_t c = next_chunk.fetch_add(1);
            if (c >= nchunks) break;
            const int b = (int)(it & 1);
            if (it >= 2 && hipEventSynchronize(r.done[b]) != hipSuccess) return bad("ingest worker: wait");
            const int64_t c0 = c * cols_per_chunk, nc = std::min<int64_t>(cols_per_chunk, p - c0);
            const size_t bytes = (size_t)(nc * col_stride_bytes);
            std::memcpy(r.pin[b], bed_cols + c0 * col_stride_bytes, bytes);
            if (hipMemcpyAsync(r.raw[b], r.pin[b], bytes, hipMemcpyHostToDevice, r.st) != hipSuccess) return bad("ingest worker: H2D copy");
            dim3 grid((unsigned)((h->nbp + kBpPerBlock - 1) / kBpPerBlock), (unsigned)((nc + 31) / 32));
            hipLaunchKernelGGL(k_transcode, grid, dim3(256), 0, r.st, r.raw[b], col_stride_bytes, n, p, c0, nc,
                               reinterpret_cast<uint4 *>(h->X), h->nbp, cnt.p);
            if (hipEventRecord(r.done[b], r.st) != hipSuccess) return bad("ingest worker: event record");
        }
        if (hipStreamSynchronize(r.st) != hipSuccess) return bad("transcode kernel failed");
    };
    if (nth <= 1) worker();
    else {
        std::vector<std::thread> th;
        for (unsigned t = 0; t < nth; ++t) th.emplace_back(worker);
        for (auto &t : th) t.join();
    }
    if (failed.load()) { set_error("%s", err_msg.c_str()); (void)hipGetLastError(); return fail(MIH_HIP_ERROR); }
    lap("copy + DMA + transcode");
    if (hipStreamSynchronize(h->stream) != hipSuccess) { set_error("transcode kernel failed"); return fail(MIH_HIP_ERROR); }
    hipLaunchKernelGGL(k_col_stats, dim3((unsigned)((p + 255) / 256)), dim3(256), 0, h->stream, cnt.p, n, p, h->mu, h->sinv);
    std::vector<int32_t> hcnt((size_t)(3 * p));
    if (hipMemcpy(hcnt.data(), cnt.p, sizeof(int32_t) * hcnt.size(), hipMemcpyDeviceToHost) != hipSuccess) return fail(MIH_HIP_ERROR);
    std::vector<int64_t> ptr;
    if ((rc = finish_missing_ptr(h, hcnt, ptr))) return fail(rc);
    if (h->total_missing > 0)
        hipLaunchKernelGGL(k_missing_from_tiles, dim3((unsigned)h->ncg), dim3(64), 0, h->stream, reinterpret_cast<uint4 *>(h->X), h->nbp, p,
                           h->miss_ptr, h->miss_row);
    if (hipStreamSynchronize(h->stream) != hipSuccess) return fail(MIH_HIP_ERROR);
    lap("statistics + missing lists");
    reserve_fit_memory(h);
    lap("reserve for the fits");
    *out = h;
    return MIH_OK;
}

int mih_snp_create_synthetic(int64_t n, int64_t p, uint64_t seed, double missing_rate,
                             int center, int scale, int impute, int device, mih_mat **out)
{
    return mih_snp_create_synthetic_shard(n, p, 0, seed, missing_rate, center, scale, impute, device, out);
}

int mih_snp_create_synthetic_shard(int64_t n, int64_t p, int64_t col_offset, uint64_t seed, double missing_rate,
                                   int center, int scale, int impute, int device, mih_mat **out)
{
    if (!out) return MIH_BAD_ARG;
    if (n <= 0 || p <= 0 || n >= (1ll << 31)) { set_error("bad dimensions"); return MIH_BAD_DIM; }
    if (!(missing_rate >= 0.0 && missing_rate < 1.0)) { set_error("missing_rate must be in [0,1)"); return MIH_BAD_ARG; }
    MIH_TRY(select_device(device));
    mih_mat *h = new mih_mat();
    h->kind = 0; h->device = device; h->n = n; h->p = p;
    h->center = center; h->scale = scale; h->impute = impute;
    int rc = alloc_snp(h);
    if (rc) { mih_mat_destroy(h); return rc; }
    auto fail = [&](int code) { mih_mat_destroy(h); return code; };
    if (hipStreamCreate(&h->stream) != hipSuccess) return fail(MIH_HIP_ERROR);
    DevBuf<int32_t> cnt;
    if ((rc = cnt.alloc((size_t)(3 * p)))) return fail(rc);
    uint32_t miss_thr = (uint32_t)(missing_rate * 4294967296.0);
    if (hipMemsetAsync(cnt.p, 0, sizeof(int32_t) * 3 * (size_t)p, h->stream) != hipSuccess) return fail(MIH_HIP_ERROR);
    dim3 grid((unsigned)((h->nbp + kBpPerBlock - 1) / kBpPerBlock), (unsigned)h->ncg);
    hipLaunchKernelGGL(k_synth, grid, dim3(256), 0, h->stream, reinterpret_cast<uint4 *>(h->X), h->nbp, n, p, col_offset, seed, miss_thr, cnt.p);
    hipLaunchKernelGGL(k_col_stats, dim3((unsigned)((p + 255) / 256)), dim3(256), 0, h->stream, cnt.p, n, p, h->mu, h->sinv);
    if (hipStreamSynchronize(h->stream) != hipSuccess) { set_error("synthetic generator failed: %s", hipGetErrorString(hipGetLastError())); return fail(MIH_HIP_ERROR); }
    std::vector<int32_t> hcnt((size_t)(3 * p));
    if (hipMemcpy(hcnt.data(), cnt.p, sizeof(int32_t) * hcnt.size(), hipMemcpyDeviceToHost) != hipSuccess) return fail(MIH_HIP_ERROR);
    std::vector<int64_t> ptr;
    if ((rc = finish_missing_ptr(h, hcnt, ptr))) return fail(rc);
    if (h->total_missing > 0) {
        hipLaunchKernelGGL(k_fill_missing_synth, dim3((unsigned)p), dim3(64), 0, h->stream, n, p, col_offset, seed, miss_thr, h->miss_ptr, h->miss_row);
        if (hipStreamSynchronize(h->stream) != hipSuccess) return fail(MIH_HIP_ERROR);
    }
    reserve_fit_memory(h);
    *out = h;
    return MIH_OK;
}

int mih_dense_create(const double *x, int64_t n, int64_t p, int device, mih_mat **out)
{
    if (!x || !out) return MIH_BAD_ARG;
    if (n <= 0 || p <= 0) return MIH_BAD_DIM;
    MIH_TRY(select_device(device));
    mih_mat *h = new mih_mat();
    h->kind = 1; h->device = device; h->n = n; h->p = p; h->center = h->scale = h->impute = 0;
    auto fail = [&](int code) { mih_mat_destroy(h); return code; };
    if (hipMalloc((void **)&h->D, sizeof(double) * (size_t)n * (size_t)p) != hipSuccess) { set_error("hipMalloc for dense matrix failed"); (void)hipGetLastError(); return fail(MIH_OOM); }
    if (hipMemcpy(h->D, x, sizeof(double) * (size_t)n * (size_t)p, hipMemcpyHostToDevice) != hipSuccess) return fail(MIH_HIP_ERROR);
    if (hipStreamCreate(&h->stream) != hipSuccess) return fail(MIH_HIP_ERROR);
    *out = h;
    return MIH_OK;
}

int mih_dense_create_f32(const float *x, int64_t n, int64_t p, int device, mih_mat **out)
{
    if (!x || !out) return MIH_BAD_ARG;
    if (n <= 0 || p <= 0) return MIH_BAD_DIM;
    MIH_TRY(select_device(device));
    mih_mat *h = new mih_mat();
    h->kind = 1; h->device = device; h->n = n; h->p = p; h->center = h->scale = h->impute = 0;
    auto fail = [&](int code) { mih_mat_destroy(h); return code; };
    if (hipMalloc((void **)&h->Df, sizeof(float) * (size_t)n * (size_t)p) != hipSuccess) { set_error("hipMalloc for dense matrix failed"); (void)hipGetLastError(); return fail(MIH_OOM); }
    if (hipMemcpy(h->Df, x, sizeof(float) * (size_t)n * (size_t)p, hipMemcpyHostToDevice) != hipSuccess) return fail(MIH_HIP_ERROR);
    if (hipStreamCreate(&h->stream) != hipSuccess) return fail(MIH_HIP_ERROR);
    *out = h;
    return MIH_OK;
}

int mih_dense_create_synthetic(int64_t n, int64_t p, uint64_t seed, int device, mih_mat **out)
{
    if (!out) return MIH_BAD_ARG;
    if (n <= 0 || p <= 0) return MIH_BAD_DIM;
    MIH_TRY(select_device(device));
    mih_mat *h = new mih_mat();
    h->kind = 1; h->device = device; h->n = n; h->p = p; h->center = h->scale = h->impute = 0;
    auto fail = [&](int code) { mih_mat_destroy(h); return code; };
    if (hipMalloc((void **)&h->D, sizeof(double) * (size_t)n * (size_t)p) != hipSuccess) { set_error("hipMalloc for dense matrix failed"); (void)hipGetLastError(); return fail(MIH_OOM); }
    if (hipStreamCreate(&h->stream) != hipSuccess) return fail(MIH_HIP_ERROR);
    hipLaunchKernelGGL(k_synth_dense, dim3(8192), dim3(256), 0, h->stream, h->D, n * p, seed);
    if (hipStreamSynchronize(h->stream) != hipSuccess) return fail(MIH_HIP_ERROR);
    *out = h;
    return MIH_OK;
}

int mih_mat_destroy(mih_mat *h)
{
    if (!h) return MIH_OK;
    (void)hipSetDevice(h->device);
    for (hipStream_t ws : h->worker_streams) if (ws) { (void)hipStreamSynchronize(ws); (void)hipStreamDestroy(ws); }
    h->worker_streams.clear();
    if (h->X) (void)hipFree(h->X);
    if (h->mu) (void)hipFree(h->mu);
    if (h->sinv) (void)hipFree(h->sinv);
    if (h->miss_ptr) (void)hipFree(h->miss_ptr);
    if (h->miss_row) (void)hipFree(h->miss_row);
    if (h->D) (void)hipFree(h->D);
    if (h->Df) (void)hipFree(h->Df);
    if (h->Du) (void)hipFree(h->Du);
    if (h->du_mun) (void)hipFree(h->du_mun);
    if (h->du_sc) (void)hipFree(h->du_sc);
    if (h->stream) (void)hipStreamDestroy(h->stream);
    delete h;
    return MIH_OK;
}

int mih_mat_reserve(mih_mat *h, int64_t bytes)
{
    if (!h) { set_error("null handle"); return MIH_BAD_ARG; }
    if (h->kind != 0) return MIH_OK;
    MIH_HIP(hipSetDevice(h->device));
    if (bytes < 0) { h->pool = nullptr; h->pool_owner.reset(); return MIH_OK; }
    if (h->pool) return MIH_OK;
    reserve_fit_memory(h, true, (size_t)bytes);
    if (!h->pool) { set_error("the device has no room for a reserve of the asked size beside this matrix"); return MIH_OOM; }
    return MIH_OK;
}

int mih_mat_dims(const mih_mat *h, int64_t *n, int64_t *p)
{
    if (!h) return MIH_BAD_ARG;
    if (n) *n = h->n;
    if (p) *p = h->p;
    return MIH_OK;
}

int mih_snp_mu_sigma(const mih_mat *h, double *mu, double *sinv)
{
    if (!h || (h->kind != 0 && !h->Du)) { set_error("not a SnpLinAlg or dosage handle"); return MIH_BAD_ARG; }
    MIH_HIP(hipSetDevice(h->device));
    if (mu) MIH_HIP(hipMemcpy(mu, h->mu, sizeof(double) * (size_t)h->p, hipMemcpyDeviceToHost));
    if (sinv) MIH_HIP(hipMemcpy(sinv, h->sinv, sizeof(double) * (size_t)h->p, hipMemcpyDeviceToHost));
    return MIH_OK;
}

static int export_codes(const mih_mat *h, uint8_t *bed_cols_out, bool impute_mode);
int mih_snp_export_bed(const mih_mat *h, uint8_t *bed_cols_out) { return export_codes(h, bed_cols_out, false); }
int mih_snp_naive_impute(const mih_mat *h, uint8_t *bed_cols_out) { return export_codes(h, bed_cols_out, true); }
static int export_codes(const mih_mat *h, uint8_t *bed_cols_out, bool impute_mode)
{
    if (!h || h->kind != 0 || !bed_cols_out) return MIH_BAD_ARG;
    MIH_HIP(hipSetDevice(h->device));
    DevBuf<uint32_t> tmp;
    int64_t ndw = h->n_pad / 16;
    MIH_TRY(tmp.alloc((size_t)h->p * (size_t)ndw));
    hipLaunchKernelGGL(k_export, dim3(4096), dim3(256), 0, h->stream, reinterpret_cast<const uint4 *>(h->X), h->nbp, h->ncg, h->p, ndw, tmp.p);
    if (h->total_missing > 0 && impute_mode)
        hipLaunchKernelGGL(k_impute_mode, dim3((unsigned)h->p), dim3(64), 0, h->stream, tmp.p, ndw, h->p, h->n, h->miss_ptr, h->miss_row);
    else if (h->total_missing > 0)
        hipLaunchKernelGGL(k_export_missing, dim3((unsigned)h->p), dim3(64), 0, h->stream, tmp.p, ndw, h->p, h->miss_ptr, h->miss_row);
    MIH_HIP(hipStreamSynchronize(h->stream));
    size_t width = (size_t)((h->n + 3) / 4);
    MIH_HIP(hipMemcpy2D(bed_cols_out, width, tmp.p, (size_t)ndw * 4, width, (size_t)h->p, hipMemcpyDeviceToHost));
    return MIH_OK;
}

}
```

### mendeliht.jl_amd/csrc/xtv.hip

```cpp
#include "common.h"
#include "peel.h"
#include <algorithm>
#include <mutex>
#include <utility>

namespace mih {

static bool prof_begin(const mih_mat *h, hipStream_t s, PassRecord &rec)
{
    Profile &pf = *h->prof;
    if (!pf.on) return false;
    if (hipEventCreate(&rec.e0) != hipSuccess || hipEventCreate(&rec.e1) != hipSuccess) { rec.e0 = rec.e1 = nullptr; (void)hipGetLastError(); return false; }
    (void)hipEventRecord(rec.e0, s);
    return true;
}
static void prof_end(const mih_mat *h, hipStream_t s, PassRecord &rec)
{
    (void)hipEventRecord(rec.e1, s);
    Profile &pf = *h->prof;
    std::lock_guard<std::mutex> g(pf.mu);
    pf.open.push_back(rec);
}
void Profile::drain()
{
    for (auto &r : open) {
        float ms = 0.f, st = 0.f;
        mih_pass_record out;
        memset(&out, 0, sizeof(out));
        if (hipEventSynchronize(r.e1) == hipSuccess && hipEventElapsedTime(&ms, r.e0, r.e1) == hipSuccess) {
            if (origin && hipEventElapsedTime(&st, origin, r.e0) != hipSuccess) { st = 0.f; (void)hipGetLastError(); }
            out.start_ms = st; out.ms = ms; out.residuals = r.residuals; out.operands = r.operands; out.stream_tag = r.stream_tag;
            memcpy(out.kernel, r.kernel, sizeof(out.kernel));
            done.push_back(out);
        } else (void)hipGetLastError();
        (void)hipEventDestroy(r.e0); (void)hipEventDestroy(r.e1);
    }
    open.clear();
}
Profile::~Profile()
{
    for (auto &r : open) { (void)hipEventDestroy(r.e0); (void)hipEventDestroy(r.e1); }
    for (auto &r : xopen) { (void)hipEventDestroy(r.e0); (void)hipEventDestroy(r.e1); }
    if (origin) (void)hipEventDestroy(origin);
}

typedef float f32x16 __attribute__((ext_vector_type(16)));
typedef int i32x8 __attribute__((ext_vector_type(8)));

__global__ void __launch_bounds__(256)
k_r_stats(const double *__restrict__ r, int64_t n, int m, double *__restrict__ part ,
          unsigned *__restrict__ done , int ebits, double *__restrict__ scal,
          const int32_t *__restrict__ gate, int32_t gate_val, double *__restrict__ peel )
{
    if (gate && *gate != gate_val) return;
    __shared__ double smax[256], ssum[256];
    __shared__ bool last;
    const int v = blockIdx.y;
    double mx = 0.0, sm = 0.0;
    const int64_t stride = (int64_t)gridDim.x * 256;
    for (int64_t i = blockIdx.x * 256ll + threadIdx.x; i < n; i += 8 * stride) {
        double x8[8];
        #pragma unroll
        for (int u = 0; u < 8; ++u) x8[u] = (i + u * stride < n) ? r[(int64_t)v * n + i + u * stride] : 0.0;
        #pragma unroll
        for (int u = 0; u < 8; ++u) if (i + u * stride < n) { mx = fmax(mx, fabs(x8[u])); sm += x8[u]; }
    }
    smax[threadIdx.x] = mx; ssum[threadIdx.x] = sm;
    __syncthreads();
    for (int k = 128; k > 0; k >>= 1) {
        if ((int)threadIdx.x < k) { smax[threadIdx.x] = fmax(smax[threadIdx.x], smax[threadIdx.x + k]); ssum[threadIdx.x] += ssum[threadIdx.x + k]; }
        __syncthreads();
    }
    const int nblocks = (int)gridDim.x;
    if (threadIdx.x == 0) {
        part[((int64_t)v * nblocks + blockIdx.x) * 2] = smax[0]; part[((int64_t)v * nblocks + blockIdx.x) * 2 + 1] = ssum[0];
        __threadfence();
        last = atomicAdd(&done[v], 1u) == (unsigned)nblocks - 1;
    }
    __syncthreads();
    if (!last) return;
    __threadfence();
    double top = -1.0;
    if (peel) {
        const int64_t nb64 = (n + 255) / 256;
        top = peel_decide(r + (int64_t)v * n, n, part + (int64_t)v * nblocks * 2, (int)(nb64 < nblocks ? nb64 : nblocks), peel + (int64_t)v * kPeelStride);
    }
    if (threadIdx.x == 0) {
        double fmx = 0.0, fsm = 0.0;
        for (int b = 0; b < nblocks; ++b) {
            fmx = fmax(fmx, __hip_atomic_load(&part[((int64_t)v * nblocks + b) * 2], __ATOMIC_RELAXED, __HIP_MEMORY_SCOPE_AGENT));
            fsm += __hip_atomic_load(&part[((int64_t)v * nblocks + b) * 2 + 1], __ATOMIC_RELAXED, __HIP_MEMORY_SCOPE_AGENT);
        }
        if (top < 0.0) top = fmx;
        int e = 0;
        if (top > 0.0 && top < 1.0e300) e = ebits - ilogb(top);
        if (e > 1000) e = 1000;
        scal[4 * v + 0] = fmx;
        scal[4 * v + 1] = ldexp(1.0, -e);
        scal[4 * v + 2] = fsm;
        scal[4 * v + 3] = ldexp(1.0, e);
        done[v] = 0;
    }
}

__device__ __forceinline__ int digit13(int m)
{
    return m <= 4 ? m : m >= 9 ? m - 13 : m == 5 ? -8 : m == 6 ? 6 : m == 7 ? -6 : 8;
}
__device__ __forceinline__ int digit49(int m)
{
    return m <= 16 ? m : m >= 33 ? m - 49 : (m & 1) ? m - 49 : m;
}

__global__ void __launch_bounds__(256)
k_digits(const double *__restrict__ r, int64_t n, int64_t nblk, int m, DigitMode dm,
         double *scal, uint4 *__restrict__ dig , uint2 *__restrict__ dig2, FlatPasses fp, XtvStatsHook sh,
         const double *__restrict__ peel )
{
    if (dm.gate && *dm.gate != dm.gate_val) return;
    __shared__ uint32_t img[4][2][32][6];
    __shared__ double s_scale;
    if (sh.spart) {
        if (threadIdx.x == 0) {
            double fmx = 0.0, fsm = 0.0;
            for (int b = 0; b < 64; ++b) { fmx = fmax(fmx, sh.spart[2 * b]); fsm += sh.spart[2 * b + 1]; }
            const double top = (peel && peel[0] > 0.0) ? peel[2] : fmx;
            int e = 0;
            if (top > 0.0 && top < 1.0e300) e = sh.ebits - ilogb(top);
            if (e > 1000) e = 1000;
            s_scale = ldexp(1.0, e);
            if (blockIdx.x == 0) { scal[0] = fmx; scal[1] = ldexp(1.0, -e); scal[2] = fsm; scal[3] = ldexp(1.0, e); }
        }
        if (blockIdx.x == 0 && (int)threadIdx.x >= 64 && (int)threadIdx.x < 64 + sh.q) {
            const int l = threadIdx.x - 64;
            double a = 0.0;
            for (int b = 0; b < sh.zblocks; ++b) a += sh.zpart[(int64_t)l * sh.zblocks + b];
            sh.df2[l] = a;
        }
        __syncthreads();
    }
    const int w = threadIdx.x >> 6, lane = threadIdx.x & 63;
    const int64_t blk = blockIdx.x * 4ll + w;
    const int vs = blockIdx.y;
    const int slots = dm.slots, op = vs / dm.per_op, sub = vs % dm.per_op;
    const bool fp6 = dm.base == 49;
    {
        uint32_t *z = &img[w][0][0][0];
        #pragma unroll
        for (int e = 0; e < 6; ++e) z[e * 64 + lane] = 0u;
    }
    __syncthreads();
    if (vs < m && blk < nblk) {
        const int64_t i = blk * 64 + lane;
        double x = (i < n) ? r[(int64_t)vs * n + i] : 0.0;
        if (peel) {
            const double *pl = peel + (int64_t)vs * kPeelStride;
            if (pl[0] > 0.0 && fabs(x) > pl[1]) x = 0.0;
        }
        long long R = __double2ll_rn(x * (sh.spart ? s_scale : scal[4 * vs + 3]));
        const int hh = lane >> 5, uu = (lane >> 4) & 1, ss = lane & 15;
        const int el = 8 * (2 * uu + (ss & 1)) + (ss >> 1);
        const int bit = (fp6 ? 6 : 4) * el, dwd = bit >> 5, sh = bit & 31;
        uint32_t *mine = &img[w][hh][0][0];
        const bool neg = R < 0;
        const unsigned long long aR = neg ? 0ull - (unsigned long long)R : (unsigned long long)R;
        uint32_t limb_hi = (uint32_t)(aR / 282475249ull), limb_lo = (uint32_t)(aR - (unsigned long long)limb_hi * 282475249ull);
        int carry = 0;
        if (dm.base == 4) {
            const unsigned long long U = (unsigned long long)R + 0x00AAAAAAAAAAAAAAull;
            for (int t = 0; t < dm.ndig; ++t) {
                const uint32_t u = (uint32_t)(U >> (2 * t)) & 3u;
                const uint32_t code = (0x109Au >> (4u * u)) & 15u;
                if (code) atomicOr(mine + t * 6 + dwd, code << sh);
            }
        } else
        for (int t = 0; t < dm.ndig; ++t) {
            int d;
            if (dm.base == 49) {
                const uint32_t L = t < 5 ? limb_lo : limb_hi, qd = L / 49u;
                const int v = (int)(L - qd * 49u) + carry;
                if (t < 5) limb_lo = qd; else limb_hi = qd;
                if (v == 49) { d = 0; carry = 1; }
                else { d = digit49(v); carry = d < 0; }
                if (neg) d = -d;
            } else if (dm.base == 4) {
                const int mm = (int)(R & 3);
                d = mm < 2 ? mm : mm - 4;
                R = (R - d) >> 2;
            } else {
                int mm = (int)(R % 13);
                if (mm < 0) mm += 13;
                d = digit13(mm);
                R = (R - d) / 13;
            }
            const unsigned a = (unsigned)(d < 0 ? -d : d);
            uint32_t code;
            if (fp6) code = (a < 8 ? a : a < 16 ? a : a <= 30 ? 8u + (a >> 1) : 16u + (a >> 2)) | (d < 0 ? 32u : 0u);
            else code = (a <= 4 ? a : a == 6 ? 5u : 6u) | (d < 0 ? 8u : 0u);
            if (code) {
                atomicOr(mine + t * 6 + dwd, code << sh);
                if (sh > 26) atomicOr(mine + t * 6 + dwd + 1, code >> (32 - sh));
            }
        }
    }
    __syncthreads();
    if (blk < nblk && lane < 2 * slots) {
        const int h = lane / slots, dg = lane % slots;
        int64_t o = ((int64_t)op * nblk + blk) * 64 + h * 32 + sub * slots + dg;
        if (dm.lay16) {
            int col = sub * slots + dg, opc = op;
            if (dm.flat) {
                int q = 0;
                while (q + 1 < fp.npass && vs >= fp.u0[q + 1]) ++q;
                const int cg = (vs - fp.u0[q]) * slots + dg;
                opc = fp.t0[q] + (cg >> 5); col = cg & 31;
            }
            const int e = (int)(blk & 1);
            o = ((int64_t)opc * nblk + (blk - e) + (col >> 4)) * 64 + 16 * (e + 2 * h) + (col & 15);
        }
        const uint32_t *q = &img[w][h][dg][0];
        dig[o] = make_uint4(q[0], q[1], q[2], q[3]);
        if (fp6) dig2[o] = make_uint2(q[4], q[5]);
    }
}

typedef unsigned int u32x4 __attribute__((ext_vector_type(4)));
typedef unsigned int u32x2 __attribute__((ext_vector_type(2)));
__device__ __forceinline__ uint4 ld_stream(const uint4 *p)
{
    u32x4 v = __builtin_nontemporal_load(reinterpret_cast<const u32x4 *>(p));
    return make_uint4(v.x, v.y, v.z, v.w);
}

__device__ __forceinline__ f32x16 mfma_fp6(uint32_t u0, uint32_t u1, const uint4 &b, const uint2 &b2, f32x16 acc)
{
    const uint32_t M = 0x33333333u;
    i32x8 a = {(int)(u0 & M), (int)((u0 >> 2) & M), (int)(u1 & M), (int)((u1 >> 2) & M), 0, 0, 0, 0};
    i32x8 bb = {(int)b.x, (int)b.y, (int)b.z, (int)b.w, (int)b2.x, (int)b2.y, 0, 0};
    return __builtin_amdgcn_mfma_scale_f32_32x32x64_f8f6f4(a, bb, acc, 4, 2, 0, 0, 0, 0);
}

__device__ __forceinline__ f32x16 mfma_fp4(uint32_t u0, uint32_t u1, const uint4 &b, f32x16 acc)
{
    const uint32_t M = 0x33333333u;
    i32x8 a = {(int)(u0 & M), (int)((u0 >> 2) & M), (int)(u1 & M), (int)((u1 >> 2) & M), 0, 0, 0, 0};
    i32x8 bb = {(int)b.x, (int)b.y, (int)b.z, (int)b.w, 0, 0, 0, 0};
    return __builtin_amdgcn_mfma_scale_f32_32x32x64_f8f6f4(a, bb, acc, 4, 4, 0, 0, 0, 0);
}

template <int CT, int NR>
__device__ __forceinline__ void xtv_epilogue(const f32x16 (&acc)[CT][NR], int lane, int64_t cg0, int64_t ncg, int split,
                                             int splits, DigitMode dm, const double *__restrict__ scal,
                                             double *__restrict__ partial)
{
    const int slots = dm.slots, col = lane & 31;
    const int sub = col / slots, dgt = col - sub * slots;
    const bool live = sub < dm.per_op;
    double wgt = 0.0;
    if (live && dgt < dm.ndig) {
        unsigned long long w = dm.base == 49 ? 16 : 4;
        for (int t = 0; t < dgt; ++t) w *= (unsigned)dm.base;
        wgt = (double)w;
    }
    const bool tree = (slots & (slots - 1)) == 0;
    const int src0 = (lane & 32) + sub * slots;
    #pragma unroll
    for (int v = 0; v < NR; ++v) {
        const int rhs = v * dm.per_op + (live ? sub : 0);
        const double inv = scal[4 * rhs + 1];
        #pragma unroll
        for (int c = 0; c < CT; ++c) {
            #pragma unroll
            for (int g = 0; g < 16; ++g) {
                double x = (double)acc[c][v][g] * wgt;
                if (tree) {
                    if (slots > 16) x += __shfl_xor(x, 16, 64);
                    if (slots > 8) x += __shfl_xor(x, 8, 64);
                    #pragma unroll
                    for (int off = 4; off > 0; off >>= 1) x += __shfl_xor(x, off, 64);
                } else {
                    double sum = 0.0;
                    #pragma unroll
                    for (int t = 0; t < 10; ++t) sum += __shfl(x, src0 + t, 64);
                    x = sum;
                }
                int row = (g & 3) + 8 * (g >> 2) + 4 * (lane >> 5);
                if (dgt == 0 && live && cg0 + c < ncg)
                    partial[((int64_t)rhs * splits + split) * (ncg * 32) + (cg0 + c) * 32 + row] = x * inv;
            }
        }
    }
}

template <int WAVES, int CT, int NR>
__global__ void __launch_bounds__(WAVES * 64)
k_xtv_mfma(const uint4 *__restrict__ X, int64_t nbp, int64_t ncg, const uint4 *__restrict__ dig, int64_t dig_stride,
           int splits, DigitMode dm, const double *__restrict__ scal, double *__restrict__ partial )
{
    const int lane = threadIdx.x & 63;
    const int wave = __builtin_amdgcn_readfirstlane(threadIdx.x >> 6);
    const int split = blockIdx.x % splits;
    const int64_t grp = blockIdx.x / splits;
    const int64_t cg0 = (grp * WAVES + wave) * CT;
    if (cg0 >= ncg) return;
    const int64_t bps = (nbp + splits - 1) / splits;
    const int64_t b0 = split * bps;
    const int64_t b1 = (b0 + bps < nbp) ? b0 + bps : nbp;

    f32x16 acc[CT][NR];
    #pragma unroll
    for (int c = 0; c < CT; ++c)
        #pragma unroll
        for (int v = 0; v < NR; ++v)
            #pragma unroll
// ... 264 lines not shown
    }
}
template <int CT, int NR>
__device__ __forceinline__ void xtv_epilogue_lds(const f32x16 (&acc)[CT][NR], float *buf, int lane, int64_t cg0, int64_t ncg,
                                                 int split, int splits, DigitMode dm, const double *__restrict__ scal,
                                                 double *__restrict__ partial)
{
    if (dm.slots == 10) xtv_epilogue_lds_s<CT, NR, 10>(acc, buf, lane, cg0, ncg, split, splits, dm, scal, partial);
    else if (dm.slots == 8) xtv_epilogue_lds_s<CT, NR, 8>(acc, buf, lane, cg0, ncg, split, splits, dm, scal, partial);
    else if (dm.slots == 16) xtv_epilogue_lds_s<CT, NR, 16>(acc, buf, lane, cg0, ncg, split, splits, dm, scal, partial);
    else xtv_epilogue_lds_s<CT, NR, 32>(acc, buf, lane, cg0, ncg, split, splits, dm, scal, partial);
}

template <int NR, int CT, int WAVES, int D, bool FP6, int MODE = 0>
__global__ void __launch_bounds__(WAVES * 64, 1)
k_xtv_dma(const uint4 *__restrict__ X, int64_t nbp, int64_t ncg, const uint4 *__restrict__ dig, const uint2 *__restrict__ dig2,
          int64_t dig_stride, int splits, DigitMode dm, const double *__restrict__ scal,
          double *__restrict__ partial )
{
    constexpr int S = D + 1;
    constexpr int DOS = WAVES * CT * 1024;
    constexpr int OPB = FP6 ? 3072 : 2048;
    constexpr int DGT = NR * OPB;
    constexpr int STAGE = DOS + DGT;
    constexpr int PPO = FP6 ? 3 : 2;
    constexpr int NP = NR * PPO;
    constexpr int PW = (NP + WAVES - 1) / WAVES;
    constexpr int L = CT + PW;
    constexpr int NI = 2 * NR;
    static_assert(S * STAGE <= 160 * 1024, "LDS ring too large");
    static_assert(D * L <= 63, "vmcnt range");
    static_assert(S * STAGE >= WAVES * 32 * 36 * 4, "the epilogue buffers overlay the ring");
    if (dm.gate && *dm.gate != dm.gate_val) return;
    __shared__ uint4 lds[S * STAGE / 16];
    const int lane = threadIdx.x & 63;
    const int wave = __builtin_amdgcn_readfirstlane(threadIdx.x >> 6);
    const int split = blockIdx.x % splits;
    const int64_t grp = blockIdx.x / splits;
    const int64_t cg0 = (grp * WAVES + wave) * CT;
    const int64_t bps = (nbp + splits - 1) / splits;
    const int64_t b0 = split * bps;
    const int64_t b1 = (b0 + bps < nbp) ? b0 + bps : nbp;

    f32x16 acc[CT][NR];
    #pragma unroll
    for (int c = 0; c < CT; ++c)
        #pragma unroll
        for (int v = 0; v < NR; ++v)
            #pragma unroll
            for (int g = 0; g < 16; ++g) acc[c][v][g] = 0.f;

    {
        const bool empty = b0 >= b1;
        const int64_t bb0 = empty ? nbp - 1 : b0;
        const int nb = empty ? 1 : (int)(b1 - b0);
        const int amask = empty ? 0 : -1;
        const char *xs[CT];
        #pragma unroll
        for (int c = 0; c < CT; ++c) {
            const int64_t cg = cg0 + c < ncg ? cg0 + c : ncg - 1;
            xs[c] = reinterpret_cast<const char *>(X) + (cg * nbp + bb0) * 1024;
        }
        const char *dsrc[PW]; int dstep[PW]; int doff[PW];
        #pragma unroll
        for (int u = 0; u < PW; ++u) {
            const int jj = wave + u * WAVES, j = jj < NP ? jj : NP - 1;
            const int op = j / PPO, part = j - PPO * op;
            if (part < 2) {
                dsrc[u] = reinterpret_cast<const char *>(dig) + (op * dig_stride + (2 * bb0 + part) * 64) * 16;
                dstep[u] = 2048; doff[u] = DOS + op * OPB + part * 1024;
            } else {
                dsrc[u] = reinterpret_cast<const char *>(dig2) + (op * dig_stride + 2 * bb0 * 64) * 8;
                dstep[u] = 1024; doff[u] = DOS + op * OPB + 2048;
            }
        }
        const uint32_t voff = lane * 16;
        const uint32_t lds0 = (uint32_t)(uintptr_t)lds;
        const uint32_t mydos = wave * CT * 1024;
        const char *ldsb = reinterpret_cast<const char *>(lds);

        auto issue = [&](int ts, int st) {
            const int tb = ts < nb ? ts : nb - 1;
            const uint32_t base = lds0 + st * STAGE;
            #pragma unroll
            for (int c = 0; c < CT; ++c) glds16<true>(base + mydos + c * 1024, voff, xs[c] + (int64_t)tb * 1024);
            #pragma unroll
            for (int u = 0; u < PW; ++u) glds16<false>(base + doff[u], voff, dsrc[u] + (int64_t)tb * dstep[u]);
        };
        auto read_b = [&](int st, int item, i32x8 &b) {
            const int v = item >> 1, e = item & 1;
            const char *q = ldsb + st * STAGE + DOS + v * OPB;
            const i32x4v lo = *reinterpret_cast<const i32x4v *>(q + e * 1024 + lane * 16);
            if (FP6) {
                const i32x2v hi = lds_read_b64(q + 2048 + e * 512 + lane * 8);
                b = i32x8{lo[0], lo[1], lo[2], lo[3], hi[0], hi[1], 0, 0};
            } else b = i32x8{lo[0], lo[1], lo[2], lo[3], 0, 0, 0, 0};
        };
        auto read_dos = [&](int st, i32x4v (&raw)[CT]) {
            #pragma unroll
            for (int c = 0; c < CT; ++c) raw[c] = *reinterpret_cast<const i32x4v *>(ldsb + st * STAGE + mydos + c * 1024 + lane * 16);
        };
        auto expand = [&](const i32x4v (&raw)[CT], i32x4v (&a)[CT][2]) {
            const int M = 0x33333333 & amask;
            #pragma unroll
            for (int c = 0; c < CT; ++c) {
                const unsigned x = raw[c][0], y = raw[c][1], z = raw[c][2], w = raw[c][3];
                a[c][0] = i32x4v{(int)x & M, (int)(x >> 2) & M, (int)y & M, (int)(y >> 2) & M};
                a[c][1] = i32x4v{(int)z & M, (int)(z >> 2) & M, (int)w & M, (int)(w >> 2) & M};
            }
        };

        #pragma unroll
        for (int s = 0; s < D; ++s) issue(s, s);
        i32x4v araw[CT];
        i32x4v A[2][CT][2];
        i32x8 B[2];
        wait_vm_barrier<(D - 1) * L>();
        read_dos(0, araw);
        read_b(0, 0, B[0]);
        expand(araw, A[0]);
        int st = 0;
#define MIH_MM(a_, b_, c_) (MODE == 1 ? fake4x(a_, b_, c_) : mfma4x<FP6>(a_, b_, c_))
#define MIH_DMA_STEP(P, T)                                                                                         \
        {                                                                                                          \
            const int st_next = st + 1 == S ? 0 : st + 1, st_ld = st == 0 ? S - 1 : st - 1;                        \
            if (MODE != 2) issue((T) + D, st_ld);                                                                  \
            _Pragma("unroll")                                                                                      \
            for (int i = 0; i < NI - 1; ++i) {                                                                     \
                read_b(st, i + 1, B[(i + 1) & 1]);                                                                 \
                _Pragma("unroll")                                                                                  \
                for (int c = 0; c < CT; ++c) acc[c][i >> 1] = MIH_MM(A[P][c][i & 1], B[i & 1], acc[c][i >> 1]);    \
                if (i == (NI > 2 ? NI / 2 - 1 : 0)) { wait_vm<D * L - CT>(); read_dos(st_next, araw); }            \
                if (i == (NI > 2 ? NI / 2 : 0)) expand(araw, A[(P) ^ 1]);                                          \
            }                                                                                                      \
            wait_vm_barrier<(D - 1) * L>();                                                                        \
            read_b(st_next, 0, B[0]);                                                                              \
            __builtin_amdgcn_sched_barrier(0);                                                                     \
            _Pragma("unroll")                                                                                      \
            for (int c = 0; c < CT; ++c) acc[c][NR - 1] = MIH_MM(A[P][c][1], B[1], acc[c][NR - 1]);                \
            st = st_next;                                                                                          \
        }
        for (int t = 0; t < nb; t += 2) {
            MIH_DMA_STEP(0, t)
            if (t + 1 < nb) MIH_DMA_STEP(1, t + 1)
        }
#undef MIH_DMA_STEP
#undef MIH_MM
        asm volatile("s_waitcnt vmcnt(0) lgkmcnt(0)\n\ts_barrier" ::: "memory");
    }
    if (cg0 >= ncg) return;
    xtv_epilogue_lds<CT, NR>(acc, reinterpret_cast<float *>(lds) + wave * (32 * 36), lane, cg0, ncg, split, splits, dm, scal, partial);
}

typedef float f32x4a __attribute__((ext_vector_type(4)));
__device__ __forceinline__ f32x4a mfma16(i32x4v a, const i32x8 &b, f32x4a acc)
{
    i32x8 aa = {a[0], a[1], a[2], a[3], 0, 0, 0, 0};
    return __builtin_amdgcn_mfma_scale_f32_16x16x128_f8f6f4(aa, b, acc, 4, 2, 0, 0, 0, 0);
}

template <int CT, int NR, int SLOTS, int HALF>
__device__ __forceinline__ void xtv_epilogue16_s(const f32x4a (&acc)[CT][NR][2][2], float *buf, int lane, int64_t cg0, int64_t ncg,
                                                 int split, int splits, DigitMode dm, const double *__restrict__ scal,
                                                 double *__restrict__ partial)
{
#pragma clang fp contract(off)
    constexpr int RS = 36;
    const int n16 = lane & 15, rg = lane >> 4;
    const int per_op = dm.per_op;
    double wgt[SLOTS];
    {
        unsigned long long w = 16;
        #pragma unroll
        for (int t = 0; t < SLOTS; ++t) { wgt[t] = t < dm.ndig ? (double)w : 0.0; w *= 49u; }
    }
    #pragma unroll
    for (int v = 0; v < NR; ++v) {
        const bool cut = HALF && v == NR - 1;
        const int nsub = cut ? 16 / SLOTS : per_op;
        #pragma unroll
        for (int c = 0; c < CT; ++c) {
            __builtin_amdgcn_wave_barrier();
            #pragma unroll
            for (int a = 0; a < 2; ++a)
                #pragma unroll
                for (int b = 0; b < (cut ? 1 : 2); ++b)
                    *reinterpret_cast<f32x4v *>(buf + (16 * b + n16) * RS + 16 * a + 4 * rg) =
                        f32x4v{acc[c][v][a][b][0], acc[c][v][a][b][1], acc[c][v][a][b][2], acc[c][v][a][b][3]};
            __builtin_amdgcn_wave_barrier();
            #pragma unroll
            for (int k = 0; k < 2; ++k) {
                const int o = lane + 64 * k, row = o & 31, sub = o >> 5;
                if (sub < nsub) {
                    const float *src = buf + sub * SLOTS * RS + row;
                    double x[SLOTS];
                    #pragma unroll
                    for (int t = 0; t < SLOTS; ++t) x[t] = (double)src[t * RS] * wgt[t];
                    double sum;
                    if ((SLOTS & (SLOTS - 1)) == 0) {
                        #pragma unroll
                        for (int off = SLOTS / 2; off > 0; off >>= 1)
                            #pragma unroll
                            for (int t = 0; t < off; ++t) x[t] = x[t] + x[t + off];
                        sum = x[0];
                    } else {
                        sum = 0.0;
                        #pragma unroll
                        for (int t = 0; t < SLOTS; ++t) sum += x[t];
                    }
                    const int rhs = v * per_op + sub;
                    if (cg0 + c < ncg)
                        partial[((int64_t)rhs * splits + split) * (ncg * 32) + (cg0 + c) * 32 + row] = sum * scal[4 * rhs + 1];
                }
            }
        }
    }
}

template <int CT, int NR, int HALF>
__device__ __forceinline__ void xtv_epilogue16_flat(const f32x4a (&acc)[CT][NR][2][2], float *buf, int lane, int64_t cg0, int64_t ncg,
                                                    int split, int splits, DigitMode dm, const double *__restrict__ scal,
                                                    double *__restrict__ partial)
{
#pragma clang fp contract(off)
    constexpr int RS = 36, ND = 10;
    const int n16 = lane & 15, rg = lane >> 4;
    const int nres = dm.nres;
    double wgt[ND];
    {
        unsigned long long w = 16;
        #pragma unroll
        for (int t = 0; t < ND; ++t) { wgt[t] = (double)w; w *= 49u; }
    }
    double *carry = reinterpret_cast<double *>(buf + 32 * RS);
    #pragma unroll
    for (int c = 0; c < CT; ++c) {
        #pragma unroll
        for (int v = 0; v < NR; ++v) {
            const bool cut = HALF && v == NR - 1;
            __builtin_amdgcn_wave_barrier();
            #pragma unroll
            for (int a = 0; a < 2; ++a)
                #pragma unroll
                for (int b = 0; b < (cut ? 1 : 2); ++b)
                    *reinterpret_cast<f32x4v *>(buf + (16 * b + n16) * RS + 16 * a + 4 * rg) =
                        f32x4v{acc[c][v][a][b][0], acc[c][v][a][b][1], acc[c][v][a][b][2], acc[c][v][a][b][3]};
            __builtin_amdgcn_wave_barrier();
            const int jlo = (32 * v) / ND, jhi = (32 * v + 31) / ND;
            #pragma unroll
            for (int k = 0; k < 3; ++k) {
                const int o = lane + 64 * k, row = o & 31, j = jlo + (o >> 5);
                if (j <= jhi && j < nres) {
                    const int c0 = ND * j - 32 * v;
                    const int tf = c0 < 0 ? -c0 : 0, tl = c0 + ND - 1 > 31 ? 31 - c0 : ND - 1;
                    double sum = tf == 0 ? 0.0 : carry[row];
                    #pragma unroll
                    for (int t = 0; t < ND; ++t)
                        if (t >= tf && t <= tl) {
                            const double x = (double)buf[(c0 + t) * RS + row] * wgt[t];
                            sum += x;
                        }
                    if (tl == ND - 1) {
                        if (cg0 + c < ncg)
                            partial[((int64_t)j * splits + split) * (ncg * 32) + (cg0 + c) * 32 + row] = sum * scal[4 * j + 1];
                    } else carry[row] = sum;
                }
            }
        }
    }
}

template <int NR, int CT, int WAVES, int D, int MODE = 0, int HALF = 0>
__global__ void __launch_bounds__(WAVES * 64, 1)
k_xtv_dma16(const uint4 *__restrict__ X, int64_t nbp, int64_t ncg, const uint4 *__restrict__ dig, const uint2 *__restrict__ dig2,
            int64_t dig_stride, int splits, DigitMode dm, const double *__restrict__ scal,
            double *__restrict__ partial )
{
    constexpr int S = D + 1;
    constexpr int DOS = WAVES * CT * 1024;
    constexpr int OPB = 3072;
    constexpr int DGT = NR * OPB;
    constexpr int STAGE = DOS + DGT;
    constexpr int NP = NR * 3;
    constexpr int PW = (NP + WAVES - 1) / WAVES;
    constexpr int L = CT + PW;
    constexpr int NI = 2 * NR - HALF;
    constexpr int ODD = NI & 1;
    static_assert(S * STAGE <= 160 * 1024, "LDS ring too large");
    static_assert(D * L <= 63, "vmcnt range");
    static_assert(S * STAGE >= WAVES * (32 * 36 + 64) * 4, "the epilogue buffers overlay the ring");
    static_assert(HALF == 0 || MODE == 0, "probes run on full operands");
    __shared__ uint4 lds[S * STAGE / 16];
    const int lane = threadIdx.x & 63;
    const int wave = __builtin_amdgcn_readfirstlane(threadIdx.x >> 6);
    const int split = blockIdx.x % splits;
    const int64_t grp = blockIdx.x / splits;
    const int64_t cg0 = (grp * WAVES + wave) * CT;
    const int64_t bps = (nbp + splits - 1) / splits;
    const int64_t b0 = split * bps;
    const int64_t b1 = (b0 + bps < nbp) ? b0 + bps : nbp;

    f32x4a acc[CT][NR][2][2];
    #pragma unroll
    for (int c = 0; c < CT; ++c)
        #pragma unroll
        for (int v = 0; v < NR; ++v)
// ... 386 lines not shown
            for (int e = 0; e < 4; ++e) a[v][c][e] = 0.0;
    #pragma unroll
    for (int v = 0; v < NRHS; ++v) rt[0][v][slot] = stage(0, v);
    __syncthreads();
    u32x4 x[kDsgCols][kDsgU], xn[kDsgCols][kDsgU];
    #pragma unroll
    for (int c = 0; c < kDsgCols; ++c)
        #pragma unroll
        for (int u = 0; u < kDsgU; ++u) { const int64_t i = lane + 64 * u; x[c][u] = i < nv ? __builtin_nontemporal_load(cx[c] + i) : vmiss; }
    for (int64_t st = 0; st < steps; ++st) {
        const int buf = (int)(st & 1);
        f64x2 rn[NRHS];
        #pragma unroll
        for (int v = 0; v < NRHS; ++v) rn[v] = stage(st + 1, v);
        #pragma unroll
        for (int c = 0; c < kDsgCols; ++c)
            #pragma unroll
            for (int u = 0; u < kDsgU; ++u) {
                const int64_t i = (st + 1) * 64 * kDsgU + lane + 64 * u;
                xn[c][u] = i < nv ? __builtin_nontemporal_load(cx[c] + i) : vmiss;
            }
        #pragma unroll
        for (int u = 0; u < kDsgU; ++u) {
            double cv[kDsgCols][8];
            #pragma unroll
            for (int c = 0; c < kDsgCols; ++c) {
                const uint32_t w[4] = {x[c][u].x, x[c][u].y, x[c][u].z, x[c][u].w};
                #pragma unroll
                for (int k = 0; k < 4; ++k) {
                    cv[c][2 * k] = dosage_c(w[k] & 0xFFFFu, mun[c]);
                    cv[c][2 * k + 1] = dosage_c(w[k] >> 16, mun[c]);
                }
            }
            #pragma unroll
            for (int v = 0; v < NRHS; ++v)
                #pragma unroll
                for (int hh = 0; hh < 4; ++hh) {
                    const f64x2 rv = rt[buf][v][hh * (kDsgPairs / 4) + lane + 64 * u];
                    #pragma unroll
                    for (int c = 0; c < kDsgCols; ++c) {
                        a[v][c][2 * (hh & 1)] = fma(cv[c][2 * hh], rv.x, a[v][c][2 * (hh & 1)]);
                        a[v][c][2 * (hh & 1) + 1] = fma(cv[c][2 * hh + 1], rv.y, a[v][c][2 * (hh & 1) + 1]);
                    }
                }
        }
        #pragma unroll
        for (int v = 0; v < NRHS; ++v) rt[buf ^ 1][v][slot] = rn[v];
        __syncthreads();
        #pragma unroll
        for (int c = 0; c < kDsgCols; ++c)
            #pragma unroll
            for (int u = 0; u < kDsgU; ++u) x[c][u] = xn[c][u];
    }
    #pragma unroll
    for (int v = 0; v < NRHS; ++v)
        #pragma unroll
        for (int c = 0; c < kDsgCols; ++c) {
            const double sum = wave_sum((a[v][c][0] + a[v][c][1]) + (a[v][c][2] + a[v][c][3]));
            if (lane == 0 && jj[c] < p) out[(int64_t)v * p + j[c]] = sum * dv.sc[j[c]];
        }
}

static void launch_dosage_lds(const mih_mat *h, const double *r_dev, int m, double *out_dev, hipStream_t s)
{
    const dim3 grid((unsigned)((h->p + kDsgWaves * kDsgCols - 1) / (kDsgWaves * kDsgCols))), block(64 * kDsgWaves);
    const DosageView dv = dosage_view(h);
    int v = 0;
    for (; v + 4 <= m; v += 4)
        hipLaunchKernelGGL((k_xtv_dosage_lds<4>), grid, block, 0, s, dv, h->n, h->p, r_dev + (int64_t)v * h->n, out_dev + (int64_t)v * h->p);
    if (m - v >= 2) {
        hipLaunchKernelGGL((k_xtv_dosage_lds<2>), grid, block, 0, s, dv, h->n, h->p, r_dev + (int64_t)v * h->n, out_dev + (int64_t)v * h->p);
        v += 2;
    }
    if (m - v == 1)
        hipLaunchKernelGGL((k_xtv_dosage_lds<1>), grid, block, 0, s, dv, h->n, h->p, r_dev + (int64_t)v * h->n, out_dev + (int64_t)v * h->p);
}

constexpr int kMaxSplits = 16;

static bool digit_mode(int id, DigitMode &dm)
{
    switch (id) {
    case -1:
    case 0:
    case 4910: dm = {49, 10, 3, 10, 53, 18}; return true;
    case 4908: dm = {49, 8, 4, 8, 42, 18}; return true;
    case 1316: dm = {13, 16, 2, 16, 56, 20}; return true;
    case 1308: dm = {13, 8, 4, 8, 26, 20}; return true;
    case 428:  dm = {4, 28, 1, 32, 53, 22}; return true;
    }
    return false;
}
bool xtv_digits_valid(int digits) { DigitMode dm; return digit_mode(digits, dm); }

#ifdef MIH_PROBES
#include "xtv_probes.inc"
#else
XtvTune xtv_tune(int digits) { XtvTune t; t.digits = digits; return t; }
static int dispatch_probe(const XtvTune &, int, bool, const mih_mat *, const uint4 *, const uint2 *, int64_t, int, DigitMode,
                          const double *, double *, hipStream_t, char *) { return -1; }
static int probe_splits(const XtvTune &) { return 0; }
#endif

static int dispatch_xtv(const XtvTune &tn, int nr, bool half, const mih_mat *h, const uint4 *dig, const uint2 *dig2, int64_t dig_stride,
                        int splits, DigitMode dm, const double *scal, double *partial, hipStream_t s, char *name)
{
    {
        const int rc = dispatch_probe(tn, nr, half, h, dig, dig2, dig_stride, splits, dm, scal, partial, s, name);
        if (rc >= 0) return rc;
    }
#define MIH_DMA16(NRV, C, W, DD, HF) if (nr == NRV && (int)half == HF) { \
        int64_t groups = (h->ncg + W * C - 1) / (W * C); \
        hipLaunchKernelGGL((k_xtv_dma16<NRV, C, W, DD, 0, HF>), dim3((unsigned)(groups * splits)), dim3(W * 64), 0, s, \
                           reinterpret_cast<const uint4 *>(h->X), h->nbp, h->ncg, dig, dig2, dig_stride, splits, dm, scal, partial); \
        snprintf(name, 48, "k_xtv_dma16<%d,%d,%d,%d%s>", NRV, C, W, DD, HF ? ",half" : ""); \
        return MIH_OK; }
    if (dm.base == 49) {
        if (!dm.lay16) { set_error("FP6 digit planes need the 16-column layout"); return MIH_BAD_ARG; }
        MIH_DMA16(6, 2, 8, 3, 1) MIH_DMA16(5, 2, 8, 4, 1) MIH_DMA16(4, 2, 8, 4, 1) MIH_DMA16(3, 2, 8, 4, 1) MIH_DMA16(2, 2, 8, 4, 1) MIH_DMA16(1, 2, 8, 4, 1)
        MIH_DMA16(6, 2, 8, 3, 0) MIH_DMA16(5, 2, 8, 4, 0) MIH_DMA16(4, 2, 8, 4, 0) MIH_DMA16(3, 2, 8, 4, 0) MIH_DMA16(2, 2, 8, 4, 0) MIH_DMA16(1, 2, 8, 4, 0)
        set_error("unsupported operand count %d", nr);
        return MIH_BAD_ARG;
    }
#undef MIH_DMA16
    if (nr == 1) {
        int64_t groups = (h->ncg + 4 * 2 - 1) / (4 * 2);
        hipLaunchKernelGGL((k_xtv_dma<1, 2, 4, 8, false, 0>), dim3((unsigned)(groups * splits)), dim3(4 * 64), 0, s,
                           reinterpret_cast<const uint4 *>(h->X), h->nbp, h->ncg, dig, dig2, dig_stride, splits, dm, scal, partial);
        snprintf(name, 48, "k_xtv_dma<1,2,4,8,fp4>");
        return MIH_OK;
    }
#define MIH_LDS(NRV, C, RB, W) if (nr == NRV) { \
        int64_t groups = (h->ncg + W * C - 1) / (W * C); \
        hipLaunchKernelGGL((k_xtv_mfma_lds<NRV, C, RB, 0, W>), dim3((unsigned)(groups * splits)), dim3(W * 64), 0, s, \
                           reinterpret_cast<const uint4 *>(h->X), h->nbp, h->ncg, dig, dig2, dig_stride, splits, dm, scal, partial); \
        snprintf(name, 48, "k_xtv_mfma_lds<%d,%d,%d,%d,fp4>", NRV, C, RB, W); \
        return MIH_OK; }
    MIH_LDS(4, 2, 2, 8) MIH_LDS(3, 2, 2, 8) MIH_LDS(2, 4, 1, 4)
#undef MIH_LDS
    set_error("unsupported operand count %d", nr);
    return MIH_BAD_ARG;
}

static int auto_splits(const mih_mat *h, const XtvTune &tn)
{
    if (tn.slices >= 1 && tn.slices <= kMaxSplits) return tn.slices;
    int s = 1;
    while (s < 4 && h->n >= 100000ll * s) s *= 2;
    const int64_t groups = (h->ncg + 15) / 16;
    while (s < 16 && groups * s < 2048 && h->nbp / (2 * s) >= 8) s *= 2;
    return s;
}

static bool xtv_lay16(const DigitMode &dm, const XtvTune &tn)
{
    return dm.base == 49 && tn.variant < 0 && (tn.multi_variant == 0 || (tn.multi_variant >= 40 && tn.multi_variant < 50));
}

static bool xtv_flat(const DigitMode &dm, const XtvTune &tn)
{
    return xtv_lay16(dm, tn) && tn.multi_variant == 0 && dm.slots * dm.per_op < 32 && tn.max_nr >= 4;
}
static int xtv_pass_residuals(const DigitMode &dm, const XtvTune &tn)
{
    return xtv_flat(dm, tn) ? (tn.max_ops * 32) / dm.slots : tn.max_ops * dm.per_op;
}

static void choose_mode(const mih_mat *h, const XtvTune &tn, bool batched, DigitMode &dm)
{
    digit_mode(tn.digits, dm);
    if (tn.digits == 0 || tn.digits == -1) {
        if (!batched) digit_mode(428, dm);
        else if (tn.variant >= 0 || h->n_pad > ((int64_t)kMaxSplits << dm.rows_log2)) digit_mode(1316, dm);
        if (h->n_pad > ((int64_t)kMaxSplits << dm.rows_log2)) digit_mode(428, dm);
    }
}

int xtv_lockstep_width(const mih_mat *h, const XtvTune &tn)
{
    if (h->kind != 0) return 16;
    DigitMode dm;
    choose_mode(h, tn, true, dm);
    if (xtv_lay16(dm, tn)) return 2 * xtv_pass_residuals(dm, tn);
    return 8 * dm.per_op;
}

int xtv_work_init(const mih_mat *h, XtvWork &w, int m, const XtvTune &tune, bool batched)
{
    w.tune = tune;
    if (h->kind != 0) return MIH_OK;
    if (!xtv_digits_valid(tune.digits)) { set_error("residual format must be 0 (default), -1 (auto in lock-step drivers), 4910, 4908, 1316, 1308 or 428"); return MIH_BAD_ARG; }
    int64_t nblk = h->nbp * 2;
    choose_mode(h, tune, batched, w.dm);
    w.has_alt = tune.digits == -1 && batched && w.dm.base == 49 && w.dm.ndig == 10;
    w.use_alt = false;
    if (w.dm.base == 49 && tune.variant >= 0) {
        set_error("the FP6 residual formats need the default kernel (variant -1)");
        return MIH_BAD_ARG;
    }
    int ops = (m + w.dm.per_op - 1) / w.dm.per_op;
    size_t rhs_cap = (size_t)ops * w.dm.per_op;
    if (xtv_flat(w.dm, tune)) {
        const int cap = xtv_pass_residuals(w.dm, tune), npass = (m + cap - 1) / cap;
        if (npass <= kMaxFlatPasses) { ops = (m * w.dm.slots + 31) / 32 + npass; rhs_cap = (size_t)m; }
    }
    w.ops_cap = ops; w.rhs_cap = rhs_cap;
    const size_t lanes = (size_t)w.ops_cap * (size_t)nblk * 64;
    const size_t dwords = lanes * (w.dm.base == 49 ? 6 : 4);
    MIH_TRY(w.digits.alloc(dwords));
    MIH_TRY(w.partial.alloc((size_t)kMaxSplits * rhs_cap * (size_t)h->ncg * 32));
    MIH_TRY(w.scal.alloc(rhs_cap * 4 + (size_t)m * kStatBlocks * 2));
    MIH_TRY(w.stat_done.alloc(rhs_cap));
    MIH_TRY(w.peel.alloc(rhs_cap * kPeelStride));
    MIH_HIP(hipMemsetAsync(w.peel.p, 0, sizeof(double) * rhs_cap * kPeelStride, h->stream));
    MIH_HIP(hipMemset(w.stat_done.p, 0, sizeof(unsigned) * rhs_cap));
    MIH_HIP(hipMemsetAsync(w.digits.p, 0, sizeof(*w.digits.p) * dwords, h->stream));
    MIH_HIP(hipMemsetAsync(w.scal.p, 0, sizeof(double) * rhs_cap * 4, h->stream));
    MIH_HIP(hipStreamSynchronize(h->stream));
    w.m_cap = m; w.splits_cap = kMaxSplits;
    return MIH_OK;
}

void xtv_count_peels(const mih_mat *h, XtvWork &w, hipStream_t s)
{
    if (!h->prof->on || !w.peel.p || w.rhs_cap == 0) return;
    std::vector<double> c(w.rhs_cap * kPeelStride, 0.0);
    if (hipMemcpyAsync(c.data(), w.peel.p, sizeof(double) * c.size(), hipMemcpyDeviceToHost, s) != hipSuccess ||
        hipStreamSynchronize(s) != hipSuccess) { (void)hipGetLastError(); return; }
    double total = 0.0;
    for (size_t v = 0; v < w.rhs_cap; ++v) total += c[v * kPeelStride + 3];
    h->prof->count(MIH_CNT_PEELED_RESIDUALS, (int64_t)(total - w.peels_counted));
    w.peels_counted = total;
}

int xtv_device(const mih_mat *h, XtvWork &w, const double *r_dev, int m, double *out_dev, hipStream_t s)
{
    const XtvTune &tn = w.tune;
    if (h->kind == 1 && h->Du) {
        PassRecord rec;
        const bool prof = prof_begin(h, s, rec);
        launch_dosage_lds(h, r_dev, m, out_dev, s);
        if (prof) {
            rec.residuals = m; rec.operands = m; rec.stream_tag = w.stream_tag;
            snprintf(rec.kernel, sizeof(rec.kernel), "k_xtv_dosage_lds<u16>");
            prof_end(h, s, rec);
        }
        MIH_HIP(hipGetLastError());
        return MIH_OK;
    }
    if (h->kind == 1) {
        const bool lds_ok = tn.variant < 0 && (((uintptr_t)(h->Df ? (const void *)h->Df : (const void *)h->D)) & 15) == 0
                            && h->n % (h->Df ? 4 : 2) == 0;
        PassRecord rec;
        const bool prof = prof_begin(h, s, rec);
        if (lds_ok) {
            if (h->Df) launch_dense_lds<float>(h->Df, h, r_dev, m, out_dev, s);
            else launch_dense_lds<double>(h->D, h, r_dev, m, out_dev, s);
        } else {
            for (int v = 0; v < m; ++v) {
                if (h->Df) hipLaunchKernelGGL(k_xtv_dense_f32, dim3((unsigned)((h->p + 3) / 4)), dim3(256), 0, s, h->Df, h->n, h->p,
                                              r_dev + (int64_t)v * h->n, out_dev + (int64_t)v * h->p);
                else hipLaunchKernelGGL(k_xtv_dense, dim3((unsigned)((h->p + 3) / 4)), dim3(256), 0, s, h->D, h->n, h->p,
                                        r_dev + (int64_t)v * h->n, out_dev + (int64_t)v * h->p);
            }
        }
        if (prof) {
            rec.residuals = m; rec.operands = m; rec.stream_tag = w.stream_tag;
            snprintf(rec.kernel, sizeof(rec.kernel), "%s<%s>", lds_ok ? "k_xtv_dense_lds" : "k_xtv_dense", h->Df ? "f32" : "f64");
            prof_end(h, s, rec);
        }
        MIH_HIP(hipGetLastError());
        return MIH_OK;
    }
    if (m > w.m_cap) { set_error("X'r workspace too small"); return MIH_BAD_ARG; }
    int splits = probe_splits(tn);
    if (splits <= 0) splits = auto_splits(h, tn);
    DigitMode dm = (w.use_alt && w.has_alt) ? w.dm_alt : w.dm;
    dm.lay16 = xtv_lay16(dm, tn);
    const int64_t need = (h->n_pad + (1ll << dm.rows_log2) - 1) >> dm.rows_log2;
    if (need > w.splits_cap) { set_error("n = %lld rows needs more than %d row slices for exact accumulation", (long long)h->n, w.splits_cap); return MIH_BAD_DIM; }
    if (splits < need) splits = (int)need;
    if (splits > h->nbp) splits = (int)h->nbp;
    if (splits > w.splits_cap) splits = w.splits_cap;
    const int64_t nblk = h->nbp * 2, pstride = h->ncg * 32;
    const int per_op = dm.per_op;
    const int nops = (m + per_op - 1) / per_op;
    double *part = w.scal.p + w.rhs_cap * 4;
    dm.gate = w.gate; dm.gate_val = w.gate_val;
    if (!w.stats_done)
        hipLaunchKernelGGL(k_r_stats, dim3(kStatBlocks, (unsigned)m), dim3(256), 0, s, r_dev, h->n, m, part, w.stat_done.p, dm.ebits, w.scal.p, w.gate, w.gate_val, w.peel.p);
    uint4 *dig_all = reinterpret_cast<uint4 *>(w.digits.p);
    uint2 *dig2_all = reinterpret_cast<uint2 *>(w.digits.p + (size_t)w.ops_cap * (size_t)nblk * 64 * 4);
    FlatPasses fp{};
    if (xtv_flat(dm, tn)) {
        const int cap = xtv_pass_residuals(dm, tn), npass = (m + cap - 1) / cap;
        if (npass <= kMaxFlatPasses) {
            dm.flat = 1;
            fp.npass = npass;
            int u = 0, t = 0;
            for (int q = 0; q < npass; ++q) {
                const int cnt = m / npass + (q < m % npass ? 1 : 0);
                fp.u0[q] = u; fp.t0[q] = t;
                u += cnt; t += (cnt * dm.slots + 31) / 32;
            }
            fp.u0[npass] = u; fp.t0[npass] = t;
        }
    }
    hipLaunchKernelGGL(k_digits, dim3((unsigned)((nblk + 3) / 4), (unsigned)(dm.flat ? m : nops * per_op)), dim3(256), 0, s, r_dev, h->n, nblk, m, dm,
                       w.scal.p, dig_all, dig2_all, fp, (w.stats_done && m == 1) ? w.shook : XtvStatsHook(), w.peel.p);
    for (int q = 0; dm.flat && q < fp.npass; ++q) {
        const int u0 = fp.u0[q], u1 = fp.u0[q + 1], t = fp.t0[q], nr = fp.t0[q + 1] - t;
        DigitMode dq = dm;
        dq.nres = u1 - u0;
        double *partial = w.partial.p + (int64_t)u0 * splits * pstride;
        PassRecord rec;
        const bool prof = prof_begin(h, s, rec);
        const bool half = tn.half && (u1 - u0) * dm.slots - 32 * (nr - 1) <= 16;
        char name[48] = {0};
        const int rc = dispatch_xtv(tn, nr, half, h, dig_all + (int64_t)t * nblk * 64, dig2_all + (int64_t)t * nblk * 64, nblk * 64, splits, dq,
                                    w.scal.p + 4 * u0, partial, s, name);
        if (prof) {
            rec.residuals = u1 - u0; rec.operands = nr; rec.stream_tag = w.stream_tag;
            memcpy(rec.kernel, name, sizeof(rec.kernel));
            prof_end(h, s, rec);
        }
        if (rc) return rc;
        hipLaunchKernelGGL(k_xtv_finalize, dim3((unsigned)((h->p + 255) / 256)), dim3(256), 0, s,
                           partial, splits, pstride, h->p, u1 - u0, w.scal.p + 4 * u0, r_dev + (int64_t)u0 * h->n, h->n, h->mu, h->sinv,
                           h->miss_ptr, h->miss_row, h->center, h->scale, h->impute && h->total_missing > 0, out_dev + (int64_t)u0 * h->p, w.gate, w.gate_val, XtvSupportHook(),
                           w.peel.p + (int64_t)u0 * kPeelStride, h->X, h->nbp);
    }
    if (dm.flat) { MIH_HIP(hipGetLastError()); return MIH_OK; }
    for (int t = 0; t < nops;) {
        int nr = (nops - t >= 4 && nops - t != 5 && tn.max_nr >= 4) ? 4 : ((nops - t == 3 || nops - t == 5) && tn.max_nr >= 4) ? 3
                 : (nops - t >= 2 && tn.max_nr >= 2) ? 2 : 1;
        if (dm.lay16 && tn.max_nr >= 4) {
            const int rem = nops - t, mo = tn.max_ops, passes = (rem + mo - 1) / mo;
            nr = (rem + passes - 1) / passes;
        }
        const int u0 = t * per_op;
        double *partial = w.partial.p + (int64_t)u0 * splits * pstride;
        const uint4 *dig = dig_all + (int64_t)t * nblk * 64;
        const uint2 *dig2 = dig2_all + (int64_t)t * nblk * 64;
        PassRecord rec;
        const bool prof = prof_begin(h, s, rec);
        const int u1 = std::min((t + nr) * per_op, m);
        const bool half = dm.lay16 && tn.half && (u1 - (t + nr - 1) * per_op) * dm.slots <= 16;
        char name[48] = {0};
        const int rc = dispatch_xtv(tn, nr, half, h, dig, dig2, nblk * 64, splits, dm, w.scal.p + 4 * u0, partial, s, name);
        if (prof) {
            rec.residuals = u1 - u0; rec.operands = nr; rec.stream_tag = w.stream_tag;
            memcpy(rec.kernel, name, sizeof(rec.kernel));
            prof_end(h, s, rec);
        }
        if (rc) return rc;
        if (u1 > u0) {
            const bool hooked = w.hook.cur != nullptr && m == 1;
            hipLaunchKernelGGL(k_xtv_finalize, dim3((unsigned)((h->p + 255) / 256 + (hooked ? w.hook.blocks : 0))), dim3(256), 0, s,
                               w.partial.p + (int64_t)u0 * splits * pstride, splits, pstride, h->p, u1 - u0,
                               w.scal.p + 4 * u0, r_dev + (int64_t)u0 * h->n, h->n, h->mu, h->sinv, h->miss_ptr, h->miss_row,
                               h->center, h->scale, h->impute && h->total_missing > 0, out_dev + (int64_t)u0 * h->p, w.gate, w.gate_val,
                               hooked ? w.hook : XtvSupportHook(), w.peel.p + (int64_t)u0 * kPeelStride, h->X, h->nbp);
        }
        t += nr;
    }
    MIH_HIP(hipGetLastError());
    return MIH_OK;
}

}

using namespace mih;

extern "C" {

int mih_profile_enable(const mih_mat *h, int on)
{
    if (!h) { set_error("null matrix handle"); return MIH_BAD_ARG; }
    Profile &pf = *h->prof;
    std::lock_guard<std::mutex> g(pf.mu);
    if (on && !pf.on) {
        MIH_HIP(hipSetDevice(h->device));
        if (pf.origin) { (void)hipEventDestroy(pf.origin); pf.origin = nullptr; }
        MIH_HIP(hipEventCreate(&pf.origin));
        MIH_HIP(hipEventRecord(pf.origin, h->stream));
    }
    pf.on = on != 0;
    return MIH_OK;
}

int mih_profile_read(const mih_mat *h, double *xtv_kernel_ms, int64_t *xtv_launches, int reset)
{
    if (!h) { set_error("null matrix handle"); return MIH_BAD_ARG; }
    Profile &pf = *h->prof;
    std::lock_guard<std::mutex> g(pf.mu);
    pf.drain();
    double ms = 0.0;
    for (const auto &r : pf.done) ms += r.ms;
    if (xtv_kernel_ms) *xtv_kernel_ms = ms;
    if (xtv_launches) *xtv_launches = (int64_t)pf.done.size();
    if (reset) pf.done.clear();
    return MIH_OK;
}

int mih_profile_passes(const mih_mat *h, mih_pass_record *out, int64_t cap, int64_t *n, int reset)
{
    if (!h || !n) { set_error("null argument"); return MIH_BAD_ARG; }
    Profile &pf = *h->prof;
    std::lock_guard<std::mutex> g(pf.mu);
    pf.drain();
    *n = (int64_t)pf.done.size();
    if (out) for (int64_t i = 0; i < cap && i < *n; ++i) out[i] = pf.done[(size_t)i];
    if (reset) pf.done.clear();
    return MIH_OK;
}

int mih_profile_exchange(const mih_mat *h, double *ms4, int64_t *count4, int reset)
{
    if (!h || !ms4 || !count4) { set_error("null argument"); return MIH_BAD_ARG; }
    Profile &pf = *h->prof;
    std::lock_guard<std::mutex> g(pf.mu);
    for (auto &r : pf.xopen) {
        float ms = 0.f;
        if (hipEventSynchronize(r.e1) == hipSuccess && hipEventElapsedTime(&ms, r.e0, r.e1) == hipSuccess) { pf.xms[r.kind] += ms; ++pf.xcount[r.kind]; }
        else (void)hipGetLastError();
        (void)hipEventDestroy(r.e0); (void)hipEventDestroy(r.e1);
    }
    pf.xopen.clear();
    for (int i = 0; i < 4; ++i) { ms4[i] = pf.xms[i]; count4[i] = pf.xcount[i]; if (reset) { pf.xms[i] = 0.0; pf.xcount[i] = 0; } }
    return MIH_OK;
}

int mih_profile_counters(const mih_mat *h, int64_t *out, int reset)
{
    if (!h || !out) { set_error("null argument"); return MIH_BAD_ARG; }
    Profile &pf = *h->prof;
    std::lock_guard<std::mutex> g(pf.mu);
    for (int i = 0; i < MIH_PROFILE_NCOUNTERS; ++i) { out[i] = pf.counters[i]; if (reset) pf.counters[i] = 0; }
    return MIH_OK;
}

int mih_xtv_algorithmic_bytes(const mih_mat *h, int m, double *bytes)
{
    if (!h || !bytes || m < 1) return MIH_BAD_ARG;
    if (h->kind == 0)
        *bytes = (double)h->p * (double)((h->n + 3) / 4) + 8.0 * m * ((double)h->n + (double)h->p) + 16.0 * (double)h->p;
    else
        *bytes = (h->Du ? 2.0 : h->Df ? 4.0 : 8.0) * (double)h->n * (double)h->p + 8.0 * m * ((double)h->n + (double)h->p);
    return MIH_OK;
}

int mih_xtv_batched_fmt(const mih_mat *h, const double *R, int m, int digits, double *OUT)
{
    if (!h || !R || !OUT || m < 1) { set_error("null/invalid argument"); return MIH_BAD_ARG; }
    MIH_HIP(hipSetDevice(h->device));
    XtvWork w;
    MIH_TRY(xtv_work_init(h, w, m, xtv_tune(digits)));
    DevBuf<double> r, out;
    MIH_TRY(r.alloc((size_t)m * h->n));
    MIH_TRY(out.alloc((size_t)m * h->p));
    MIH_HIP(hipMemcpyAsync(r.p, R, sizeof(double) * (size_t)m * h->n, hipMemcpyHostToDevice, h->stream));
    MIH_TRY(xtv_device(h, w, r.p, m, out.p, h->stream));
    MIH_HIP(hipMemcpyAsync(OUT, out.p, sizeof(double) * (size_t)m * h->p, hipMemcpyDeviceToHost, h->stream));
    MIH_HIP(hipStreamSynchronize(h->stream));
    xtv_count_peels(h, w, h->stream);
    return MIH_OK;
}

int mih_xtv_batched(const mih_mat *h, const double *R, int m, double *OUT)
{
    return mih_xtv_batched_fmt(h, R, m, 0, OUT);
}

int mih_xtv(const mih_mat *h, const double *r, double *out)
{
    return mih_xtv_batched_fmt(h, r, 1, 0, out);
}

#ifdef MIH_PROBES
int mih_probe_xtv_sequence(const mih_mat *h, const double *R, int mcap, const int *ms, int nms, int digits, double *OUT)
{
    if (!h || !R || !ms || !OUT || mcap < 1 || nms < 1) { set_error("null/invalid argument"); return MIH_BAD_ARG; }
    for (int i = 0; i < nms; ++i) if (ms[i] < 1 || ms[i] > mcap) { set_error("ms[%d] = %d outside 1..%d", i, ms[i], mcap); return MIH_BAD_ARG; }
    MIH_HIP(hipSetDevice(h->device));
    XtvWork w;
    MIH_TRY(xtv_work_init(h, w, mcap, xtv_tune(digits)));
    DevBuf<double> r, out;
    MIH_TRY(r.alloc((size_t)mcap * h->n));
    MIH_TRY(out.alloc((size_t)mcap * h->p));
    MIH_HIP(hipMemcpyAsync(r.p, R, sizeof(double) * (size_t)mcap * h->n, hipMemcpyHostToDevice, h->stream));
    size_t off = 0;
    for (int i = 0; i < nms; ++i) {
        MIH_TRY(xtv_device(h, w, r.p, ms[i], out.p, h->stream));
        MIH_HIP(hipMemcpyAsync(OUT + off, out.p, sizeof(double) * (size_t)ms[i] * h->p, hipMemcpyDeviceToHost, h->stream));
        MIH_HIP(hipStreamSynchronize(h->stream));
        off += (size_t)ms[i] * h->p;
    }
    return MIH_OK;
}
#endif

__global__ void k_fill_random(double *r, int64_t n, uint64_t seed)
{
    int64_t i = blockIdx.x * (int64_t)blockDim.x + threadIdx.x;
    if (i >= n) return;
    uint32_t a = (uint32_t)i * 0x9E3779B1u ^ (uint32_t)seed;
    a ^= a >> 16; a *= 0x7feb352du; a ^= a >> 15; a *= 0x846ca68bu; a ^= a >> 16;
    uint32_t b = a * 0x85EBCA77u; b ^= b >> 13;
    r[i] = ((a & 0xFFFF) + (a >> 16) + (b & 0xFFFF) + (b >> 16)) * (1.0 / 65536.0) - 2.0;
}

__global__ void k_checksum(const double *x, int64_t p, double *out)
{
    __shared__ double red[256];
    double a = 0.0;
    for (int64_t i = threadIdx.x; i < p; i += 256) a += x[i];
    red[threadIdx.x] = a;
    __syncthreads();
    for (int k = 128; k > 0; k >>= 1) { if ((int)threadIdx.x < k) red[threadIdx.x] += red[threadIdx.x + k]; __syncthreads(); }
    if (threadIdx.x == 0) *out = red[0];
}

int mih_bench_xtv(const mih_mat *h, int digits, int m, int iters, int warmup, uint64_t seed, float *ms_per_pass, double *checksum)
{
    if (!h || iters < 1 || !ms_per_pass || m < 1) return MIH_BAD_ARG;
    MIH_HIP(hipSetDevice(h->device));
    XtvWork w;
    MIH_TRY(xtv_work_init(h, w, m, xtv_tune(digits), m > 1));
    DevBuf<double> r, out, cs;
    MIH_TRY(r.alloc((size_t)h->n * m));
    MIH_TRY(out.alloc((size_t)h->p * m));
    MIH_TRY(cs.alloc(1));
    hipStream_t s = h->stream;
    int rc = MIH_OK;
    hipLaunchKernelGGL(k_fill_random, dim3((unsigned)((h->n * m + 255) / 256)), dim3(256), 0, s, r.p, h->n * m, seed);
    for (int i = 0; i < warmup && !rc; ++i) rc = xtv_device(h, w, r.p, m, out.p, s);
    hipEvent_t e0, e1;
    (void)hipEventCreate(&e0); (void)hipEventCreate(&e1);
    (void)hipEventRecord(e0, s);
    for (int i = 0; i < iters && !rc; ++i) rc = xtv_device(h, w, r.p, m, out.p, s);
    (void)hipEventRecord(e1, s);
    hipError_t e = hipEventSynchronize(e1);
    float ms = 0.f;
    (void)hipEventElapsedTime(&ms, e0, e1);
    (void)hipEventDestroy(e0); (void)hipEventDestroy(e1);
    if (rc) return rc;
    if (e != hipSuccess) return hip_fail(e, "bench sync", __FILE__, __LINE__);
    *ms_per_pass = ms / iters;
    if (checksum) {
        hipLaunchKernelGGL(k_checksum, dim3(1), dim3(256), 0, s, out.p, h->p * m, cs.p);
        MIH_HIP(hipMemcpyAsync(checksum, cs.p, sizeof(double), hipMemcpyDeviceToHost, s));
        MIH_HIP(hipStreamSynchronize(s));
    }
    return MIH_OK;
}

}
```

Before: 56.33 iterations/s.

## Add five-genotypes-per-byte SNP image and a matching single-residual Xᵀr kernel

Builds a second copy of the genotype matrix that packs five 2-bit genotypes per byte in base 3, with missing genotypes mapped to zero, laid out by row slice for a new MFMA kernel that decodes bytes through an LDS lookup table. When the image exists and m=1, Xᵀr streams this denser image instead of the 2-bit one, cutting HBM bytes per iteration by about a fifth. It is built by default for matrices of 4 GiB or more when free memory allows, and is dropped when later allocations run out of memory. The cost is extra device memory, a table lookup per byte, and a digit layout changed to 40-row fragments. The reported GB/s figure now counts the smaller image.

```diff
diff --git a/include/mendeliht_hip.h b/include/mendeliht_hip.h
--- a/include/mendeliht_hip.h
+++ b/include/mendeliht_hip.h
@@ -62,6 +62,7 @@
 int mih_dosage_export(const mih_mat *h, int64_t col0, int64_t ncols, uint16_t *out);
 int mih_mat_destroy(mih_mat *h);
 int mih_mat_reserve(mih_mat *h, int64_t bytes);
+int mih_snp_pack(mih_mat *h, int mode);
 int mih_mat_dims(const mih_mat *h, int64_t *n, int64_t *p);
 int mih_snp_mu_sigma(const mih_mat *h, double *mu, double *sinv);
 int mih_snp_export_bed(const mih_mat *h, uint8_t *bed_cols_out);
diff --git a/mendeliht.jl_amd/api.py b/mendeliht.jl_amd/api.py
--- a/mendeliht.jl_amd/api.py
+++ b/mendeliht.jl_amd/api.py
@@ -136,6 +136,7 @@
         "mih_mat_destroy": [vp],
         "mih_mat_dims": [vp, C.POINTER(i64), C.POINTER(i64)],
         "mih_mat_reserve": [vp, i64],
+        "mih_snp_pack": [vp, C.c_int],
         "mih_snp_mu_sigma": [vp, vp, vp],
         "mih_snp_export_bed": [vp, vp],
         "mih_snp_naive_impute": [vp, vp],
@@ -190,7 +191,7 @@
             "mih_snp_create_synthetic_shard",
             "mih_dense_create", "mih_dense_create_synthetic", "mih_dense_create_f32",
             "mih_dosage_create", "mih_dosage_create_synthetic", "mih_dosage_export",
-            "mih_dosage_create_bgen", "mih_dosage_regrid", "mih_mat_destroy", "mih_mat_dims", "mih_mat_reserve",
+            "mih_dosage_create_bgen", "mih_dosage_regrid", "mih_mat_destroy", "mih_mat_dims", "mih_mat_reserve", "mih_snp_pack",
             "mih_snp_mu_sigma", "mih_snp_export_bed", "mih_snp_naive_impute", "mih_xtv", "mih_xtv_batched", "mih_xv_sparse",
             "mih_project_topk", "mih_project_group_sparse", "mih_fit_iht", "mih_cv_iht", "mih_cv_meanloss", "mih_cv_assignment", "mih_cv_iht_multi", "mih_fit_iht_path",
             "mih_fit_mv", "mih_cv_mv", "mih_bench_xtv", "mih_xtv_algorithmic_bytes", "mih_xtv_batched_fmt", "mih_abi_sizes",
@@ -436,6 +437,10 @@
         x = cls(None, center=center, scale=scale, impute=impute, device=device, _handle=h)
         x._reserve(reserve)
         return x
+
+    def pack(self, on=True):
+        _check(lib().mih_snp_pack(self._h, 1 if on else 0))
+        return self
 
     def mu_sigma(self):
         mu, s = np.empty(self.p), np.empty(self.p)
diff --git a/mendeliht.jl_amd/csrc/common.h b/mendeliht.jl_amd/csrc/common.h
--- a/mendeliht.jl_amd/csrc/common.h
+++ b/mendeliht.jl_amd/csrc/common.h
@@ -47,6 +47,18 @@
 
 inline int64_t round_up(int64_t a, int64_t b) { return (a + b - 1) / b * b; }
 
+std::recursive_mutex &pack5_mutex();
+bool pack5_drop_all();
+inline hipError_t lib_malloc(void **q, size_t bytes)
+{
+    hipError_t e = hipMalloc(q, bytes);
+    if (e == hipErrorOutOfMemory) {
+        (void)hipGetLastError();
+        if (pack5_drop_all()) e = hipMalloc(q, bytes);
+    }
+    return e;
+}
+
 struct DevPool {
     char *base = nullptr; size_t bytes = 0;
     std::mutex mu;
@@ -57,7 +69,7 @@
     bool init(size_t total)
     {
         total = (total + kGran - 1) / kGran * kGran;
-        if (hipMalloc((void **)&base, total) != hipSuccess) { (void)hipGetLastError(); base = nullptr; return false; }
+        if (lib_malloc((void **)&base, total) != hipSuccess) { (void)hipGetLastError(); base = nullptr; return false; }
         bytes = total; free_blocks[0] = total;
         return true;
     }
@@ -102,7 +114,7 @@
     if (DevPool *pl = current_pool()) {
         if (bytes >= (1ull << 20)) { if (void *r = pl->take(bytes)) { *q = r; *from = pl; return hipSuccess; } }
     }
-    return hipMalloc(q, bytes);
+    return lib_malloc(q, bytes);
 }
 
 struct Arena {
@@ -268,6 +280,9 @@
     int32_t   denom = 0;
     double   *du_mun = nullptr;
     double   *du_sc = nullptr;
+    uint8_t  *X5 = nullptr;
+    int       p5_splits = 0;
+    int64_t   p5_bps = 0, p5_sp = 0;
     hipStream_t stream = nullptr;
     mih::DevPool *pool = nullptr;
     std::shared_ptr<mih::DevPool> pool_owner;
@@ -311,6 +326,7 @@
     int lay16 = 0;
     int flat = 0;
     int nres = 0;
+    int pack5 = 0; int64_t p5_bps = 0, p5_sp = 0;
     const int32_t *gate = nullptr; int32_t gate_val = 0;
 };
 constexpr int kMaxFlatPasses = 16;
@@ -363,6 +379,11 @@
 int  xtv_work_init(const mih_mat *h, XtvWork &w, int m, const XtvTune &tune, bool batched = true);
 int  xtv_device(const mih_mat *h, XtvWork &w, const double *r_dev, int m, double *out_dev, hipStream_t s);
 void xtv_count_peels(const mih_mat *h, XtvWork &w, hipStream_t s);
+int  xtv_single_splits(const mih_mat *h);
+constexpr int kP5Rows = 160;
+inline int64_t pack5_steps(int64_t bps) { return (bps * 128 + kP5Rows - 1) / kP5Rows; }
+int  pack5_build(mih_mat *h);
+void pack5_drop(mih_mat *h);
 int  xtv_lockstep_width(const mih_mat *h, const XtvTune &tune);
 
 struct XvWork {
diff --git a/mendeliht.jl_amd/csrc/dosage.hip b/mendeliht.jl_amd/csrc/dosage.hip
--- a/mendeliht.jl_amd/csrc/dosage.hip
+++ b/mendeliht.jl_amd/csrc/dosage.hip
@@ -86,7 +86,7 @@
     h->kind = 1; h->device = device; h->n = n; h->p = p; h->center = h->scale = h->impute = 0;
     h->denom = denom;
     h->du_ld = (n + 7) / 8 * 8;
-    if (hipMalloc((void **)&h->Du, sizeof(uint16_t) * (size_t)h->du_ld * (size_t)p) != hipSuccess) {
+    if (lib_malloc((void **)&h->Du, sizeof(uint16_t) * (size_t)h->du_ld * (size_t)p) != hipSuccess) {
         set_error("hipMalloc for the dosage matrix (%lld x %lld u16) failed", (long long)n, (long long)p); (void)hipGetLastError(); return MIH_OOM;
     }
     for (double **a : {&h->mu, &h->sinv, &h->du_mun, &h->du_sc})
diff --git a/mendeliht.jl_amd/csrc/snp.hip b/mendeliht.jl_amd/csrc/snp.hip
--- a/mendeliht.jl_amd/csrc/snp.hip
+++ b/mendeliht.jl_amd/csrc/snp.hip
@@ -1,4 +1,5 @@
 #include "common.h"
+#include <algorithm>
 #include <memory>
 #include <cstdarg>
 #include <cmath>
@@ -303,13 +304,104 @@
     return MIH_OK;
 }
 
+__global__ void __launch_bounds__(256)
+k_pack5(const uint32_t *__restrict__ X, int64_t nbp, int splits, int64_t bps, int64_t sp, uint4 *__restrict__ X5)
+{
+    const int lane = threadIdx.x & 63, m = lane & 31, h = lane >> 5;
+    const int64_t stp = blockIdx.x * 4ll + (threadIdx.x >> 6), cg = blockIdx.y;
+    if (stp >= splits * sp) return;
+    const int64_t slice = stp / sp, t = stp - slice * sp;
+    const int64_t r0 = slice * bps * 128, rend = (slice + 1) * bps < nbp ? (slice + 1) * bps * 128 : nbp * 128;
+    const int64_t j = cg * 32 + m;
+    uint32_t out[4];
+    #pragma unroll
+    for (int f = 0; f < 4; ++f) {
+        uint32_t wd = 0;
+        #pragma unroll
+        for (int d = 0; d < 4; ++d) {
+            const int64_t row = r0 + t * kP5Rows + 40 * f + 20 * h + 5 * d;
+            uint32_t byte = 0, pw = 1;
+            #pragma unroll
+            for (int q = 0; q < 5; ++q) {
+                const int64_t i = row + q;
+                uint32_t g = 0;
+                if (i < rend) g = (X[xword(nbp, j, i >> 4)] >> (2 * (int)(i & 15))) & 3u;
+                byte += pw * (g < 3u ? g : 0u);
+                pw *= 3u;
+            }
+            wd |= byte << (8 * d);
+        }
+        out[f] = wd;
+    }
+    X5[((cg * splits + slice) * sp + t) * 64 + lane] = make_uint4(out[0], out[1], out[2], out[3]);
+}
+
+std::recursive_mutex &pack5_mutex() { static std::recursive_mutex mu; return mu; }
+static std::vector<mih_mat *> &pack5_live() { static std::vector<mih_mat *> v; return v; }
+
+void pack5_drop(mih_mat *h)
+{
+    std::lock_guard<std::recursive_mutex> g(pack5_mutex());
+    auto &v = pack5_live();
+    v.erase(std::remove(v.begin(), v.end(), h), v.end());
+    if (!h->X5) return;
+    uint8_t *q = h->X5;
+    h->X5 = nullptr; h->p5_splits = 0; h->p5_bps = h->p5_sp = 0;
+    int dev = 0;
+    (void)hipGetDevice(&dev);
+    (void)hipSetDevice(h->device);
+    (void)hipFree(q);
+    (void)hipSetDevice(dev);
+}
+
+bool pack5_drop_all()
+{
+    std::lock_guard<std::recursive_mutex> g(pack5_mutex());
+    const std::vector<mih_mat *> v = pack5_live();
+    for (mih_mat *h : v) pack5_drop(h);
+    return !v.empty();
+}
+
+int pack5_build(mih_mat *h)
+{
+    if (h->kind != 0 || !h->X) { set_error("the five-per-byte image belongs to a 2-bit matrix"); return MIH_BAD_ARG; }
+    std::lock_guard<std::recursive_mutex> g(pack5_mutex());
+    if (h->X5) return MIH_OK;
+    const int splits = xtv_single_splits(h);
+    const int64_t bps = (h->nbp + splits - 1) / splits, sp = pack5_steps(bps);
+    if (h->ncg > 65535) { set_error("the five-per-byte image is built for at most 2 097 120 columns"); return MIH_BAD_DIM; }
+    const size_t bytes = (size_t)h->ncg * (size_t)splits * (size_t)sp * 1024;
+    uint8_t *q = nullptr;
+    if (hipMalloc((void **)&q, bytes) != hipSuccess) {
+        (void)hipGetLastError();
+        set_error("no room for the five-per-byte image (%zu bytes)", bytes);
+        return MIH_OOM;
+    }
+    hipLaunchKernelGGL(k_pack5, dim3((unsigned)((splits * sp + 3) / 4), (unsigned)h->ncg), dim3(256), 0, h->stream,
+                       h->X, h->nbp, splits, bps, sp, reinterpret_cast<uint4 *>(q));
+    if (hipStreamSynchronize(h->stream) != hipSuccess) { (void)hipGetLastError(); (void)hipFree(q); set_error("building the five-per-byte image failed"); return MIH_HIP_ERROR; }
+    h->X5 = q; h->p5_splits = splits; h->p5_bps = bps; h->p5_sp = sp;
+    pack5_live().push_back(h);
+    return MIH_OK;
+}
+
+static void pack5_by_default(mih_mat *h)
+{
+    const size_t x_bytes = (size_t)h->ncg * (size_t)h->nbp * 1024;
+    if (h->kind != 0 || x_bytes < (size_t)(4ull << 30)) return;
+    size_t free_b = 0, total_b = 0;
+    if (hipMemGetInfo(&free_b, &total_b) != hipSuccess) { (void)hipGetLastError(); return; }
+    if (free_b < x_bytes) return;
+    (void)pack5_build(h);
+}
+
 static int alloc_snp(mih_mat *h)
 {
     h->ncg = (h->p + 31) / 32;
     h->nbp = (h->n + 127) / 128;
     h->n_pad = h->nbp * 128;
     size_t bytes = sizeof(uint4) * (size_t)h->ncg * (size_t)h->nbp * 64;
-    hipError_t e = hipMalloc((void **)&h->X, bytes);
+    hipError_t e = lib_malloc((void **)&h->X, bytes);
     if (e != hipSuccess) { set_error("hipMalloc of %zu bytes for the genotype matrix failed: %s", bytes, hipGetErrorString(e)); return MIH_OOM; }
     MIH_HIP(hipMalloc((void **)&h->mu, sizeof(double) * (size_t)h->p));
     MIH_HIP(hipMalloc((void **)&h->sinv, sizeof(double) * (size_t)h->p));
@@ -397,6 +489,9 @@
     const size_t want = asked_bytes ? asked_bytes : 4 * big + 64 * var;
     size_t free_b = 0, total_b = 0;
     if (hipMemGetInfo(&free_b, &total_b) != hipSuccess) { (void)hipGetLastError(); return; }
+    if (free_b < 4 * want && asked && pack5_drop_all()) {
+        if (hipMemGetInfo(&free_b, &total_b) != hipSuccess) { (void)hipGetLastError(); return; }
+    }
     if (free_b < 4 * want) return;
     std::shared_ptr<DevPool> pool(new DevPool());
     if (pool->init(want)) { h->pool_owner = pool; h->pool = pool.get(); }
@@ -512,6 +607,8 @@
     lap("statistics + missing lists");
     reserve_fit_memory(h);
     lap("reserve for the fits");
+    pack5_by_default(h);
+    lap("five-per-byte image");
     *out = h;
     return MIH_OK;
 }
@@ -553,6 +650,7 @@
         if (hipStreamSynchronize(h->stream) != hipSuccess) return fail(MIH_HIP_ERROR);
     }
     reserve_fit_memory(h);
+    pack5_by_default(h);
     *out = h;
     return MIH_OK;
 }
@@ -565,7 +663,7 @@
     mih_mat *h = new mih_mat();
     h->kind = 1; h->device = device; h->n = n; h->p = p; h->center = h->scale = h->impute = 0;
     auto fail = [&](int code) { mih_mat_destroy(h); return code; };
-    if (hipMalloc((void **)&h->D, sizeof(double) * (size_t)n * (size_t)p) != hipSuccess) { set_error("hipMalloc for dense matrix failed"); (void)hipGetLastError(); return fail(MIH_OOM); }
+    if (lib_malloc((void **)&h->D, sizeof(double) * (size_t)n * (size_t)p) != hipSuccess) { set_error("hipMalloc for dense matrix failed"); (void)hipGetLastError(); return fail(MIH_OOM); }
     if (hipMemcpy(h->D, x, sizeof(double) * (size_t)n * (size_t)p, hipMemcpyHostToDevice) != hipSuccess) return fail(MIH_HIP_ERROR);
     if (hipStreamCreate(&h->stream) != hipSuccess) return fail(MIH_HIP_ERROR);
     *out = h;
@@ -580,7 +678,7 @@
     mih_mat *h = new mih_mat();
     h->kind = 1; h->device = device; h->n = n; h->p = p; h->center = h->scale = h->impute = 0;
     auto fail = [&](int code) { mih_mat_destroy(h); return code; };
-    if (hipMalloc((void **)&h->Df, sizeof(float) * (size_t)n * (size_t)p) != hipSuccess) { set_error("hipMalloc for dense matrix failed"); (void)hipGetLastError(); return fail(MIH_OOM); }
+    if (lib_malloc((void **)&h->Df, sizeof(float) * (size_t)n * (size_t)p) != hipSuccess) { set_error("hipMalloc for dense matrix failed"); (void)hipGetLastError(); return fail(MIH_OOM); }
     if (hipMemcpy(h->Df, x, sizeof(float) * (size_t)n * (size_t)p, hipMemcpyHostToDevice) != hipSuccess) return fail(MIH_HIP_ERROR);
     if (hipStreamCreate(&h->stream) != hipSuccess) return fail(MIH_HIP_ERROR);
     *out = h;
@@ -595,7 +693,7 @@
     mih_mat *h = new mih_mat();
     h->kind = 1; h->device = device; h->n = n; h->p = p; h->center = h->scale = h->impute = 0;
     auto fail = [&](int code) { mih_mat_destroy(h); return code; };
-    if (hipMalloc((void **)&h->D, sizeof(double) * (size_t)n * (size_t)p) != hipSuccess) { set_error("hipMalloc for dense matrix failed"); (void)hipGetLastError(); return fail(MIH_OOM); }
+    if (lib_malloc((void **)&h->D, sizeof(double) * (size_t)n * (size_t)p) != hipSuccess) { set_error("hipMalloc for dense matrix failed"); (void)hipGetLastError(); return fail(MIH_OOM); }
     if (hipStreamCreate(&h->stream) != hipSuccess) return fail(MIH_HIP_ERROR);
     hipLaunchKernelGGL(k_synth_dense, dim3(8192), dim3(256), 0, h->stream, h->D, n * p, seed);
     if (hipStreamSynchronize(h->stream) != hipSuccess) return fail(MIH_HIP_ERROR);
@@ -609,6 +707,7 @@
     (void)hipSetDevice(h->device);
     for (hipStream_t ws : h->worker_streams) if (ws) { (void)hipStreamSynchronize(ws); (void)hipStreamDestroy(ws); }
     h->worker_streams.clear();
+    pack5_drop(h);
     if (h->X) (void)hipFree(h->X);
     if (h->mu) (void)hipFree(h->mu);
     if (h->sinv) (void)hipFree(h->sinv);
@@ -634,6 +733,16 @@
     reserve_fit_memory(h, true, (size_t)bytes);
     if (!h->pool) { set_error("the device has no room for a reserve of the asked size beside this matrix"); return MIH_OOM; }
     return MIH_OK;
+}
+
+int mih_snp_pack(mih_mat *h, int mode)
+{
+    if (!h) { set_error("null handle"); return MIH_BAD_ARG; }
+    if (h->kind != 0) { set_error("the five-per-byte image belongs to a 2-bit matrix"); return MIH_BAD_ARG; }
+    if (mode != 0 && mode != 1) { set_error("mode must be 0 (drop the image) or 1 (build it)"); return MIH_BAD_ARG; }
+    MIH_HIP(hipSetDevice(h->device));
+    if (mode == 0) { pack5_drop(h); return MIH_OK; }
+    return pack5_build(h);
 }
 
 int mih_mat_dims(const mih_mat *h, int64_t *n, int64_t *p)
diff --git a/mendeliht.jl_amd/csrc/xtv.hip b/mendeliht.jl_amd/csrc/xtv.hip
--- a/mendeliht.jl_amd/csrc/xtv.hip
+++ b/mendeliht.jl_amd/csrc/xtv.hip
@@ -151,15 +151,23 @@
     }
     __syncthreads();
     if (vs < m && blk < nblk) {
-        const int64_t i = blk * 64 + lane;
-        double x = (i < n) ? r[(int64_t)vs * n + i] : 0.0;
+        int64_t i = blk * 64 + lane;
+        bool have = i < n;
+        if (dm.pack5) {
+            const int64_t stp = blk >> 2, slice = stp / dm.p5_sp;
+            const int64_t r0 = slice * dm.p5_bps * 128, r1 = r0 + dm.p5_bps * 128;
+            i = r0 + (4 * (stp - slice * dm.p5_sp) + (blk & 3)) * 40 + lane;
+            have = lane < 40 && i < r1 && i < n;
+        }
+        double x = have ? r[(int64_t)vs * n + i] : 0.0;
         if (peel) {
             const double *pl = peel + (int64_t)vs * kPeelStride;
             if (pl[0] > 0.0 && fabs(x) > pl[1]) x = 0.0;
         }
         long long R = __double2ll_rn(x * (sh.spart ? s_scale : scal[4 * vs + 3]));
-        const int hh = lane >> 5, uu = (lane >> 4) & 1, ss = lane & 15;
-        const int el = 8 * (2 * uu + (ss & 1)) + (ss >> 1);
+        const int l40 = lane < 40 ? lane : 0;
+        const int hh = dm.pack5 ? l40 / 20 : lane >> 5, uu = (lane >> 4) & 1, ss = lane & 15;
+        const int el = dm.pack5 ? 8 * ((l40 % 20) / 5) + l40 % 5 : 8 * (2 * uu + (ss & 1)) + (ss >> 1);
         const int bit = (fp6 ? 6 : 4) * el, dwd = bit >> 5, sh = bit & 31;
         uint32_t *mine = &img[w][hh][0][0];
         const bool neg = R < 0;
@@ -730,6 +738,230 @@
     xtv_epilogue_lds<CT, NR>(acc, reinterpret_cast<float *>(lds) + wave * (32 * 36), lane, cg0, ncg, split, splits, dm, scal, partial);
 }
 
+constexpr int kP5Table = 256 * 128;
+template <int CT, int WAVES, int D, int MODE = 0, int PIPE = 0>
+__global__ void __launch_bounds__(WAVES * 64, 1)
+k_xtv_pack5(const uint8_t *__restrict__ X5, int64_t nbp, int64_t ncg, const uint4 *__restrict__ dig, int splits, DigitMode dm,
+            const double *__restrict__ scal, double *__restrict__ partial )
+{
+    constexpr int S = D + 1;
+    constexpr int DOS = WAVES * CT * 1024;
+    constexpr int DGT = 4096;
+    constexpr int STAGE = DOS + DGT;
+    constexpr int L1 = CT + 1, L0 = CT;
+    static_assert(WAVES >= 4, "four digit fragments a step, one per wave");
+    static_assert(!PIPE || CT % 2 == 0, "the look-ahead tile lands in A[0]");
+    static_assert(S * STAGE + kP5Table <= 160 * 1024, "LDS ring too large");
+    static_assert(D * L1 <= 63, "vmcnt range");
+    static_assert(S * STAGE >= WAVES * 32 * 36 * 4, "the epilogue buffers overlay the ring");
+    if (dm.gate && *dm.gate != dm.gate_val) return;
+    __shared__ uint4 lds[(S * STAGE + kP5Table) / 16];
+    const int lane = threadIdx.x & 63;
+    const int wave = __builtin_amdgcn_readfirstlane(threadIdx.x >> 6);
+    const int split = blockIdx.x % splits;
+    const int64_t grp = blockIdx.x / splits;
+    const int64_t cg0 = (grp * WAVES + wave) * CT;
+    const int64_t bps = dm.p5_bps, sp = dm.p5_sp;
+    const int64_t b0 = split * bps;
+    const int64_t b1 = (b0 + bps < nbp) ? b0 + bps : nbp;
+    const int nb = b0 < b1 ? (int)(((b1 - b0) * 128 + kP5Rows - 1) / kP5Rows) : 1;
+
+    f32x16 acc[CT][1];
+    #pragma unroll
+    for (int c = 0; c < CT; ++c)
+        #pragma unroll
+        for (int g = 0; g < 16; ++g) acc[c][0][g] = 0.f;
+    {
+        char *ldsb = reinterpret_cast<char *>(lds);
+        {
+            uint32_t *tab = reinterpret_cast<uint32_t *>(ldsb + S * STAGE);
+            for (int i = threadIdx.x; i < 256 * 32; i += WAVES * 64) {
+                uint32_t b = (uint32_t)i >> 5, w = 0;
+                #pragma unroll
+                for (int q = 0; q < 5; ++q) { w |= (b % 3u) << (4 * q); b /= 3u; }
+                tab[i] = w;
+            }
+        }
+        const char *xs[CT];
+        #pragma unroll
+        for (int c = 0; c < CT; ++c) {
+            const int64_t cg = cg0 + c < ncg ? cg0 + c : ncg - 1;
+            xs[c] = reinterpret_cast<const char *>(X5) + ((cg * splits + split) * sp) * 1024;
+        }
+        const bool dwave = wave < 4;
+        const char *dsrc = reinterpret_cast<const char *>(dig) + ((int64_t)split * sp) * 4096 + (wave & 3) * 1024;
+        const uint32_t voff = lane * 16;
+        const uint32_t lds0 = (uint32_t)(uintptr_t)lds;
+        const uint32_t mydos = wave * CT * 1024;
+        const uint32_t tab0 = S * STAGE + (lane & 31) * 4;
+
+        auto issue = [&](int ts, int st) {
+            const int tb = ts < nb ? ts : nb - 1;
+            const uint32_t base = lds0 + st * STAGE;
+            #pragma unroll
+            for (int c = 0; c < CT; ++c) glds16<true>(base + mydos + c * 1024, voff, xs[c] + (int64_t)tb * 1024);
+            if (dwave) glds16<false>(base + DOS + (wave & 3) * 1024, voff, dsrc + (int64_t)tb * 4096);
+        };
+        auto wait_step = [&]() { if (dwave) wait_vm_barrier<(D - 1) * L1>(); else wait_vm_barrier<(D - 1) * L0>(); };
+        auto lookup = [&](int st, int c, uint32_t (&a)[16]) {
+            const i32x4v raw = *reinterpret_cast<const i32x4v *>(ldsb + st * STAGE + mydos + c * 1024 + lane * 16);
+            #pragma unroll
+            for (int j = 0; j < 16; ++j) {
+                const uint32_t byte = ((uint32_t)raw[j >> 2] >> (8 * (j & 3))) & 255u;
+                if (MODE == 2) a[j] = byte;
+                else a[j] = *reinterpret_cast<const uint32_t *>(ldsb + ((byte << 7) + tab0));
+            }
+        };
+
+        #pragma unroll
+        for (int s = 0; s < D; ++s) issue(s, s);
+        wait_step();
+        int st = 0;
+        uint32_t A[2][16];
+        if (PIPE) lookup(0, 0, A[0]);
+        for (int t = 0; t < nb; ++t) {
+            const int st_next = st + 1 == S ? 0 : st + 1, st_ld = st == 0 ? S - 1 : st - 1;
+            issue(t + D, st_ld);
+            i32x8 B[4];
+            #pragma unroll
+            for (int f = 0; f < 4; ++f) {
+                const i32x4v lo = *reinterpret_cast<const i32x4v *>(ldsb + st * STAGE + DOS + f * 1024 + lane * 16);
+                B[f] = i32x8{lo[0], lo[1], lo[2], lo[3], 0, 0, 0, 0};
+            }
+            if (!PIPE) lookup(st, 0, A[0]);
+            #pragma unroll
+            for (int c = 0; c < CT; ++c) {
+                if (c + 1 < CT) lookup(st, c + 1, A[(c + 1) & 1]);
+                #pragma unroll
+                for (int f = 0; f < 4; ++f) {
+                    const i32x4v a = i32x4v{(int)A[c & 1][4 * f], (int)A[c & 1][4 * f + 1], (int)A[c & 1][4 * f + 2], (int)A[c & 1][4 * f + 3]};
+                    acc[c][0] = MODE == 1 ? fake4x(a, B[f], acc[c][0]) : mfma4x<false>(a, B[f], acc[c][0]);
+                }
+            }
+            if (PIPE) {
+                if (dwave) wait_vm<D * L1 - CT>(); else wait_vm<D * L0 - CT>();
+                lookup(st_next, 0, A[0]);
+            }
+            wait_step();
+            st = st_next;
+        }
+        asm volatile("s_waitcnt vmcnt(0) lgkmcnt(0)\n\ts_barrier" ::: "memory");
+    }
+    if (cg0 >= ncg) return;
+    xtv_epilogue_lds_s<CT, 1, 32>(acc, reinterpret_cast<float *>(lds) + wave * (32 * 36), lane, cg0, ncg, split, splits, dm, scal, partial);
+}
+
+template <int CT, int WAVES, int D, int OCC>
+__global__ void __launch_bounds__(WAVES * 64, OCC * WAVES / 4)
+k_xtv_pack5r(const uint8_t *__restrict__ X5, int64_t nbp, int64_t ncg, const uint4 *__restrict__ dig, int splits, DigitMode dm,
+             const double *__restrict__ scal, double *__restrict__ partial )
+{
+    constexpr int S = D + 1;
+    constexpr int STAGE = 4096;
+    constexpr int L1 = CT + 1, L0 = CT;
+    static_assert(WAVES >= 4, "four digit fragments a step, one per wave");
+    static_assert(OCC * (S * STAGE + kP5Table) <= 160 * 1024, "LDS of the workgroups that share a CU");
+    static_assert(D * L1 <= 63, "vmcnt range");
+    static_assert(S * STAGE + kP5Table >= WAVES * 32 * 36 * 4, "the epilogue buffers overlay the ring and the table");
+    if (dm.gate && *dm.gate != dm.gate_val) return;
+    __shared__ uint4 lds[(S * STAGE + kP5Table) / 16];
+    const int lane = threadIdx.x & 63;
+    const int wave = __builtin_amdgcn_readfirstlane(threadIdx.x >> 6);
+    const int split = blockIdx.x % splits;
+    const int64_t grp = blockIdx.x / splits;
+    const int64_t cg0 = (grp * WAVES + wave) * CT;
+    const int64_t bps = dm.p5_bps, sp = dm.p5_sp;
+    const int64_t b0 = split * bps;
+    const int64_t b1 = (b0 + bps < nbp) ? b0 + bps : nbp;
+    const int nb = b0 < b1 ? (int)(((b1 - b0) * 128 + kP5Rows - 1) / kP5Rows) : 1;
+
+    f32x16 acc[CT][1];
+    #pragma unroll
+    for (int c = 0; c < CT; ++c)
+        #pragma unroll
+        for (int g = 0; g < 16; ++g) acc[c][0][g] = 0.f;
+    {
+        char *ldsb = reinterpret_cast<char *>(lds);
+        {
+            uint32_t *tab = reinterpret_cast<uint32_t *>(ldsb + S * STAGE);
+            for (int i = threadIdx.x; i < 256 * 32; i += WAVES * 64) {
+                uint32_t b = (uint32_t)i >> 5, w = 0;
+                #pragma unroll
+                for (int q = 0; q < 5; ++q) { w |= (b % 3u) << (4 * q); b /= 3u; }
+                tab[i] = w;
+            }
+        }
+        const u32x4 *xs[CT];
+        #pragma unroll
+        for (int c = 0; c < CT; ++c) {
+            const int64_t cg = cg0 + c < ncg ? cg0 + c : ncg - 1;
+            xs[c] = reinterpret_cast<const u32x4 *>(X5 + ((cg * splits + split) * sp) * 1024) + lane;
+        }
+        const bool dwave = wave < 4;
+        const char *dsrc = reinterpret_cast<const char *>(dig) + ((int64_t)split * sp) * 4096 + (wave & 3) * 1024;
+        const uint32_t voff = lane * 16;
+        const uint32_t lds0 = (uint32_t)(uintptr_t)lds;
+        const uint32_t tab0 = S * STAGE + (lane & 31) * 4;
+
+        auto issue = [&](int ts, int st, u32x4 (&r)[CT]) {
+            const int tb = ts < nb ? ts : nb - 1;
+            #pragma unroll
+            for (int c = 0; c < CT; ++c) r[c] = __builtin_nontemporal_load(xs[c] + (int64_t)tb * 64);
+            asm volatile("" ::: "memory");
+            if (dwave) glds16<false>(lds0 + st * STAGE + (wave & 3) * 1024, voff, dsrc + (int64_t)tb * 4096);
+        };
+        auto wait_step = [&]() { if (dwave) wait_vm_barrier<(D - 1) * L1>(); else wait_vm_barrier<(D - 1) * L0>(); };
+        auto lookup = [&](const u32x4 &raw, uint32_t (&a)[16]) {
+            #pragma unroll
+            for (int j = 0; j < 16; ++j) {
+                const uint32_t byte = (raw[j >> 2] >> (8 * (j & 3))) & 255u;
+                a[j] = *reinterpret_cast<const uint32_t *>(ldsb + ((byte << 7) + tab0));
+            }
+        };
+
+        u32x4 R[D][CT];
+        #pragma unroll
+        for (int s = 0; s < D; ++s) issue(s, s, R[s]);
+        wait_step();
+        int st = 0;
+        for (int t0 = 0; t0 < nb; t0 += D) {
+            #pragma unroll
+            for (int u = 0; u < D; ++u) {
+                const int t = t0 + u;
+                if (t < nb) {
+                    const int st_next = st + 1 == S ? 0 : st + 1, st_ld = st == 0 ? S - 1 : st - 1;
+                    u32x4 cur[CT];
+                    #pragma unroll
+                    for (int c = 0; c < CT; ++c) cur[c] = R[u][c];
+                    issue(t + D, st_ld, R[u]);
+                    i32x8 B[4];
+                    #pragma unroll
+                    for (int f = 0; f < 4; ++f) {
+                        const i32x4v lo = *reinterpret_cast<const i32x4v *>(ldsb + st * STAGE + f * 1024 + lane * 16);
+                        B[f] = i32x8{lo[0], lo[1], lo[2], lo[3], 0, 0, 0, 0};
+                    }
+                    uint32_t A[2][16];
+                    lookup(cur[0], A[0]);
+                    #pragma unroll
+                    for (int c = 0; c < CT; ++c) {
+                        if (c + 1 < CT) lookup(cur[c + 1], A[(c + 1) & 1]);
+                        #pragma unroll
+                        for (int f = 0; f < 4; ++f) {
+                            const i32x4v a = i32x4v{(int)A[c & 1][4 * f], (int)A[c & 1][4 * f + 1], (int)A[c & 1][4 * f + 2], (int)A[c & 1][4 * f + 3]};
+                            acc[c][0] = mfma4x<false>(a, B[f], acc[c][0]);
+                        }
+                    }
+                    wait_step();
+                    st = st_next;
+                }
+            }
+        }
+        asm volatile("s_waitcnt vmcnt(0) lgkmcnt(0)\n\ts_barrier" ::: "memory");
+    }
+    if (cg0 >= ncg) return;
+    xtv_epilogue_lds_s<CT, 1, 32>(acc, reinterpret_cast<float *>(lds) + wave * (32 * 36), lane, cg0, ncg, split, splits, dm, scal, partial);
+}
+
 typedef float f32x4a __attribute__((ext_vector_type(4)));
 __device__ __forceinline__ f32x4a mfma16(i32x4v a, const i32x8 &b, f32x4a acc)
 {
@@ -1422,6 +1654,63 @@
     return s;
 }
 
+static int pass_splits(const mih_mat *h, const XtvTune &tn, const DigitMode &dm, int cap)
+{
+    int splits = probe_splits(tn);
+    if (splits <= 0) splits = auto_splits(h, tn);
+    const int64_t need = (h->n_pad + (1ll << dm.rows_log2) - 1) >> dm.rows_log2;
+    if (splits < need) splits = (int)need;
+    if (splits > h->nbp) splits = (int)h->nbp;
+    if (splits > cap) splits = cap;
+    return splits;
+}
+int xtv_single_splits(const mih_mat *h)
+{
+    DigitMode dm;
+    digit_mode(428, dm);
+    return pass_splits(h, XtvTune(), dm, kMaxSplits);
+}
+static int64_t pack5_frag_cap(const mih_mat *h) { return (h->nbp * 16) / 5 + 8 * kMaxSplits + 8; }
+
+static void dispatch_pack5(const XtvTune &tn, const mih_mat *h, const uint8_t *X5, const uint4 *dig, int splits, DigitMode dm, const double *scal,
+                           double *partial, hipStream_t s, char *name)
+{
+#define MIH_P5(C, W, DD, MODE, PIPE, TAG) { const int64_t groups = (h->ncg + W * C - 1) / (W * C); \
+        hipLaunchKernelGGL((k_xtv_pack5<C, W, DD, MODE, PIPE>), dim3((unsigned)(groups * splits)), dim3(W * 64), 0, s, \
+                           X5, h->nbp, h->ncg, dig, splits, dm, scal, partial); \
+        snprintf(name, 48, "k_xtv_pack5<%d,%d,%d%s>", C, W, DD, TAG); return; }
+#define MIH_P5R(C, W, DD, OCC) { const int64_t groups = (h->ncg + W * C - 1) / (W * C); \
+        hipLaunchKernelGGL((k_xtv_pack5r<C, W, DD, OCC>), dim3((unsigned)(groups * splits)), dim3(W * 64), 0, s, \
+                           X5, h->nbp, h->ncg, dig, splits, dm, scal, partial); \
+        snprintf(name, 48, "k_xtv_pack5r<%d,%d,%d,%d>", C, W, DD, OCC); return; }
+#ifdef MIH_PROBES
+    switch (tn.multi_variant) {
+    case 51: MIH_P5(2, 8, 5, 1, 0, ",probe1")
+    case 52: MIH_P5(2, 8, 5, 2, 0, ",probe2")
+    case 53: MIH_P5(2, 16, 2, 0, 0, "")
+    case 54: MIH_P5(2, 8, 5, 0, 0, "")
+    case 55: MIH_P5(4, 8, 2, 0, 0, "")
+    case 56: MIH_P5(2, 8, 5, 0, 1, ",pipe")
+    case 57: MIH_P5R(2, 8, 6, 2)
+    case 58: MIH_P5R(2, 8, 3, 2)
+    case 59: MIH_P5R(1, 8, 6, 2)
+    case 60: MIH_P5R(1, 8, 8, 2)
+    case 61: MIH_P5R(2, 4, 4, 3)
+    case 62: MIH_P5R(2, 8, 5, 2)
+    case 63: MIH_P5R(2, 8, 4, 1)
+    default: break;
+    }
+#endif
+    (void)tn;
+    MIH_P5R(2, 8, 4, 2)
+#undef MIH_P5
+#undef MIH_P5R
+}
+static bool pack5_tune_ok(const XtvTune &tn)
+{
+    return tn.variant < 0 && tn.slices == 0 && (tn.multi_variant == 0 || (tn.multi_variant >= 50 && tn.multi_variant <= 63));
+}
+
 static bool xtv_lay16(const DigitMode &dm, const XtvTune &tn)
 {
     return dm.base == 49 && tn.variant < 0 && (tn.multi_variant == 0 || (tn.multi_variant >= 40 && tn.multi_variant < 50));
@@ -1475,6 +1764,7 @@
         if (npass <= kMaxFlatPasses) { ops = (m * w.dm.slots + 31) / 32 + npass; rhs_cap = (size_t)m; }
     }
     w.ops_cap = ops; w.rhs_cap = rhs_cap;
+    if (w.dm.base == 4 && pack5_frag_cap(h) > nblk) nblk = pack5_frag_cap(h);
     const size_t lanes = (size_t)w.ops_cap * (size_t)nblk * 64;
     const size_t dwords = lanes * (w.dm.base == 49 ? 6 : 4);
     MIH_TRY(w.digits.alloc(dwords));
@@ -1543,15 +1833,11 @@
         return MIH_OK;
     }
     if (m > w.m_cap) { set_error("X'r workspace too small"); return MIH_BAD_ARG; }
-    int splits = probe_splits(tn);
-    if (splits <= 0) splits = auto_splits(h, tn);
     DigitMode dm = (w.use_alt && w.has_alt) ? w.dm_alt : w.dm;
     dm.lay16 = xtv_lay16(dm, tn);
     const int64_t need = (h->n_pad + (1ll << dm.rows_log2) - 1) >> dm.rows_log2;
     if (need > w.splits_cap) { set_error("n = %lld rows needs more than %d row slices for exact accumulation", (long long)h->n, w.splits_cap); return MIH_BAD_DIM; }
-    if (splits < need) splits = (int)need;
-    if (splits > h->nbp) splits = (int)h->nbp;
-    if (splits > w.splits_cap) splits = w.splits_cap;
+    const int splits = pass_splits(h, tn, dm, w.splits_cap);
     const int64_t nblk = h->nbp * 2, pstride = h->ncg * 32;
     const int per_op = dm.per_op;
     const int nops = (m + per_op - 1) / per_op;
@@ -1562,6 +1848,31 @@
     uint4 *dig_all = reinterpret_cast<uint4 *>(w.digits.p);
     uint2 *dig2_all = reinterpret_cast<uint2 *>(w.digits.p + (size_t)w.ops_cap * (size_t)nblk * 64 * 4);
     FlatPasses fp{};
+    if (m == 1 && dm.base == 4 && dm.per_op == 1 && pack5_tune_ok(tn)) {
+        std::lock_guard<std::recursive_mutex> g(pack5_mutex());
+        const int64_t nfrag = 4 * (int64_t)splits * h->p5_sp;
+        if (h->X5 && h->p5_splits == splits && nfrag * 64 * 4 <= (int64_t)w.digits.n) {
+            dm.pack5 = 1; dm.p5_bps = h->p5_bps; dm.p5_sp = h->p5_sp;
+            hipLaunchKernelGGL(k_digits, dim3((unsigned)((nfrag + 3) / 4), 1u), dim3(256), 0, s, r_dev, h->n, nfrag, m, dm,
+                               w.scal.p, dig_all, dig2_all, fp, w.stats_done ? w.shook : XtvStatsHook(), w.peel.p);
+            PassRecord rec;
+            const bool prof = prof_begin(h, s, rec);
+            char name[48] = {0};
+            dispatch_pack5(tn, h, h->X5, dig_all, splits, dm, w.scal.p, w.partial.p, s, name);
+            if (prof) {
+                rec.residuals = 1; rec.operands = 1; rec.stream_tag = w.stream_tag;
+                memcpy(rec.kernel, name, sizeof(rec.kernel));
+                prof_end(h, s, rec);
+            }
+            const bool hooked = w.hook.cur != nullptr;
+            hipLaunchKernelGGL(k_xtv_finalize, dim3((unsigned)((h->p + 255) / 256 + (hooked ? w.hook.blocks : 0))), dim3(256), 0, s,
+                               w.partial.p, splits, pstride, h->p, 1, w.scal.p, r_dev, h->n, h->mu, h->sinv, h->miss_ptr, h->miss_row,
+                               h->center, h->scale, h->impute && h->total_missing > 0, out_dev, w.gate, w.gate_val,
+                               hooked ? w.hook : XtvSupportHook(), w.peel.p, h->X, h->nbp);
+            MIH_HIP(hipGetLastError());
+            return MIH_OK;
+        }
+    }
     if (xtv_flat(dm, tn)) {
         const int cap = xtv_pass_residuals(dm, tn), npass = (m + cap - 1) / cap;
         if (npass <= kMaxFlatPasses) {
@@ -1713,8 +2024,12 @@
 int mih_xtv_algorithmic_bytes(const mih_mat *h, int m, double *bytes)
 {
     if (!h || !bytes || m < 1) return MIH_BAD_ARG;
-    if (h->kind == 0)
-        *bytes = (double)h->p * (double)((h->n + 3) / 4) + 8.0 * m * ((double)h->n + (double)h->p) + 16.0 * (double)h->p;
+    if (h->kind == 0) {
+        bool img;
+        { std::lock_guard<std::recursive_mutex> g(pack5_mutex()); img = h->X5 != nullptr; }
+        const double col = (m == 1 && img) ? (double)((h->n + 4) / 5) : (double)((h->n + 3) / 4);
+        *bytes = (double)h->p * col + 8.0 * m * ((double)h->n + (double)h->p) + 16.0 * (double)h->p;
+    }
     else
         *bytes = (h->Du ? 2.0 : h->Df ? 4.0 : 8.0) * (double)h->n * (double)h->p + 8.0 * m * ((double)h->n + (double)h->p);
     return MIH_OK;
```

Result: no change. 56.73 iterations/s (median of 6 runs) (+0.7%).
